# mavmap/mavmap

Hardware: AMD Instinct MI355X
Metric: global-BA LM iterations/sec (higher is better)
Workload: dtype f64; 1 GPU; C3: 500 images / 200000 points / 2000000 obs global BA, PINHOLE+OPENCV, 2 shared cameras; images=500, points=200000, observations=2000000, parallelism=single GPU, options=max_iter 200, ftol 1e-6, gtol 1e-10, ptol 1e-8, Cauchy a=1, refine intrinsics

## Files before the change

### mavmap_amd/csrc/internal.h

```cpp
#ifndef MAVBA_INTERNAL_H_
#define MAVBA_INTERNAL_H_

#include <hip/hip_runtime.h>
#include <stdint.h>

#include <utility>
#include <vector>
#include <functional>

namespace mavba {

constexpr int kPoseRec = 24;
constexpr int kIntrRec = 36;

constexpr int kImgRec = 81;
constexpr int kCamRec = 54;
constexpr int kSweepAcc = 135;

struct SweepChunk { int image; int begin; int end; };

enum { BLK_PP = 0, BLK_IP = 1, BLK_II = 2 };

struct SchurBlock {
  int kind;
  int row_ent, col_ent;
  int chunk_begin, chunk_end;
};
struct SchurChunk { int begin; int end; int slot; };
struct PartialReduce { int kind, src_begin, src_end, dst; };
struct PartialRide { int n = 0; const PartialReduce* tasks = nullptr; double* pp = nullptr; double* ip = nullptr; double* ii = nullptr; };
void launch_partial_reduce(hipStream_t st, int num_tasks, const PartialReduce* tasks, double* part_pp, double* part_ip,
                           double* part_ii);

constexpr int kClImagesMax = 16, kClCamsMax = 3;
constexpr int kClCamRow0 = 6 * kClImagesMax, kClHRow = kClCamRow0 + 9 * kClCamsMax, kClRows = (kClHRow + 16) / 16 * 16;
constexpr int kClTabPP = 0, kClTabIP = kClImagesMax * (kClImagesMax + 1) / 2, kClTabII = kClTabIP + kClCamsMax * kClImagesMax,
              kClTab = kClTabII + kClCamsMax * (kClCamsMax + 1) / 2;
constexpr int kClBatch = 32;
constexpr int kTailObs = 16;
constexpr int kClMaxBatches = 64;
struct SchurCluster { int p0, p1; };

#if defined(__HIPCC__)
__host__ __device__
#endif
inline unsigned image_set_mix(unsigned x) {
  x ^= x >> 16; x *= 0x7feb352du; x ^= x >> 15; x *= 0x846ca68bu; x ^= x >> 16;
  return x;
}

constexpr int kRowsBatch = 16;
constexpr int kRowsMaxPoints = 256;
constexpr int kRowsClasses = 3;
constexpr int kRowsClassNT[kRowsClasses] = {5, 6, 8};
struct SchurRowsCluster { int p0, p1, ni, nc, emit_off, emit_n[2], flags; };
constexpr int kRowsUnplaced = 1;
#if defined(__HIPCC__)
__host__ __device__
#endif
inline int rows_cam_off(int flags, int lc) { return lc <= 0 ? 0 : lc >= 3 ? (flags >> 24) & 255 : (flags >> (8 * lc)) & 255; }
#if defined(__HIPCC__)
__host__ __device__
#endif
inline int rows_cam_rows(int flags) { return (flags >> 24) & 255; }
inline int rows_pack_flags(bool unplaced, const int* k, int nc) {
  int off[4] = {0, 0, 0, 0};
  for (int c = 0; c < 3; ++c) off[c + 1] = off[c] + (c < nc ? k[c] : 0);
  return (unplaced ? kRowsUnplaced : 0) | off[1] << 8 | off[2] << 16 | off[3] << 24;
}
constexpr unsigned kRowsEmitZero = 8191u;
constexpr unsigned rows_emit_entry(int src, int o, int tab_index) { return (unsigned)src | (unsigned)o << 13 | (unsigned)tab_index << 20; }
constexpr int kRowsListsCam = kClImagesMax, kRowsListsCams = 2 * kClImagesMax, kRowsLists = 2 * kClImagesMax + kClCamsMax + 1;
constexpr int kRowsPassSplit = 96;
#if defined(__HIPCC__)
__host__ __device__
#endif
inline int rows_class_of_rows(int rows) { return rows <= 16 * kRowsClassNT[0] ? 0 : rows <= 16 * kRowsClassNT[1] ? 1 : 2; }
#if defined(__HIPCC__)
__host__ __device__
#endif
inline int rows_count(int ni, int cam_rows) { return 6 * ni + cam_rows + 1; }

enum {
  SC_COST = 0,
  SC_XNORM2,
  SC_GRAD_MAX,
  SC_NEW_COST,
  SC_STEP_NORM2,
  SC_MODEL_CHANGE,
  SC_CAND_XNORM2,
  SC_FAIL,
  SC_FAIL_FRONT,
  SC_CAND_END,
  SC_EVAL_COUNT = SC_GRAD_MAX + 1,
  SC_CAND_BEGIN = SC_NEW_COST,
  SC_CAND_COUNT = SC_CAND_END - SC_CAND_BEGIN,
  SC_COUNT = 16
};

enum { LM_REJECTED = 0, LM_ACCEPTED = 1, LM_INVALID = 2, LM_TERM_PTOL = 3, LM_TERM_FTOL = 4, LM_TERM_GTOL = 5 };
struct LmSpec {
  const double* dec;
  const double* scal;
  double radius, decrease_factor;
  double ptol, ftol, min_rel_dec, max_radius, abs_gtol;
  int pending_eval;
};
struct LmDecision {
  int code;
  double radius, decrease_factor;
  double rel, step_norm, cost_change;
};
#if defined(__HIPCC__)
__host__ __device__
#endif
inline LmSpec lm_spec_off() { LmSpec s{}; s.dec = nullptr; s.scal = nullptr; return s; }

struct SweepArgs {
  int N, Nstride, NI, NC, KMAX;
  const double2* uv; const int* obs_img; const int* obs_pt;
  const double* camrec; const double* intr; const int* img_cam; const int* cam_model;
  const double* points;
  const unsigned char* pt_active;
  double loss_b, loss_inv_b;
  double* R; double* Jp; double* Jc; double* Jk;
  double* cost_partial;
};
int jacobian_sweep_grid(int N);
void launch_cam_prepare(hipStream_t st, int NI, const double* poses, double* camrec);
void launch_jacobian_sweep(hipStream_t st, const SweepArgs& a);
void launch_cost_only(hipStream_t st, const SweepArgs& a);
void launch_raw_residual_norm(hipStream_t st, const SweepArgs& a, double* out_norm);

void launch_point_reduce(hipStream_t st, int NP, int NPs, int Nstride, int KMAX, const int* pt_start,
                         const int* q_start, const int* q_cam, const int* obs_img, const int* img_cam,
                         const double* R, const double* Jp, const double* Jk, double* Cu, double* gu,
                         double* Wk );

constexpr int kFrontObs = 256, kFrontPts = 64, kFrontQ = 96, kFrontMaxGrid = 65536;
struct FrontTile { int p0, p1, o0, o1, q0, q1; };
struct FrontArgs {
  SweepArgs sw;
  int num_tiles, NPs;
  const FrontTile* tiles;
  const int* pt_start; const int* q_start; const int* q_cam; const int* q_pt;
  const unsigned char* pt_free;
  const double* scale_cam; const double* scale_pt;
  double radius, dmin, dmax;
  double* Cu; double* gu; double* Gi; double* h;
  double* Epose; double* Eintr;
  double* fail;
  long long* trace;
  LmSpec spec;
};
int point_front_grid(int num_tiles);
void launch_point_front(hipStream_t st, const FrontArgs& a, int kmax_intr, bool entries);

struct CamSweepArgs {
  int NI, NC;
  const SweepChunk* chunks; int num_chunks;
  const double2* im_uv; const int* im_pt;
  const double* camrec; const double* intr; const int* img_cam; const int* cam_model;
  const double* points; const unsigned char* pt_active; double loss_b, loss_inv_b;
  double* partial;
  LmSpec spec;
};
void launch_camera_sweep(hipStream_t st, const CamSweepArgs& a, int kmax, bool any_intr_free);
void launch_rot_prior(hipStream_t st, int n, const int* prior_img, const double* prior_R0, double w,
                      const double* poses, double* res, double* jac, double* cost_partial, const LmSpec& spec = lm_spec_off());

void launch_scales(hipStream_t st, int NI, int NC, int NP, int NPs, int jacobi,
                   const unsigned char* pose_free, const unsigned char* intr_free,
                   const unsigned char* pt_free, const double* img_rec, const double* cam_rec,
                   const double* Cu, double* scale_cam, double* scale_pt);

constexpr int kStateNormsCamBlocks = 64;

void launch_factor_entries_pose(hipStream_t st, int N, int Nstride, int NPs, const int* obs_img, const int* obs_pt,
                                const unsigned char* pt_free, const double* Jc, const double* Jp, const double* scale_cam,
                                const double* scale_pt, double* Gi, double* h, double* Epose, const int* pt_start,
                                const double* Cu, const double* gu, double radius, double dmin, double dmax, double* fail);
void launch_entries_intr(hipStream_t st, int Q, int NI, int NPs, const int* q_pt, const int* q_cam,
                         const double* Wk, const double* scale_cam, const double* scale_pt,
                         const double* Gi, const double* h, double* Eintr);

void launch_schur_chunks(hipStream_t st, int kind, int num_chunks, const SchurChunk* chunks,
                         const int2* terms, const double* Epose, const double* Eintr,
                         double* partial);
#if defined(__HIPCC__)
__host__ __device__
#endif
constexpr int schur_partial_stride(int kind) { return kind == BLK_PP ? 42 : kind == BLK_IP ? 54 : 90; }
void launch_schur_rows(hipStream_t st, const FrontArgs& a, int kmax_intr, bool generic, int num_clusters,
                       const SchurRowsCluster* clusters, const int* tab, const int* cl_lists, const unsigned short* obs_meta,
                       const unsigned long long* lanemap, const unsigned* emit_map, double* part_pp, double* part_ip, double* part_ii,
                       const struct CamSweepArgs* with_sweep = nullptr );
void rows_emit_map(int ni, int nc, int flags, std::vector<unsigned>& pass0, std::vector<unsigned>& pass1);
constexpr unsigned long long kRowsLanesIdentity = 0xFEDCBA9876543210ull;
void launch_schur_clusters(hipStream_t st, int num_clusters, const SchurCluster* clusters, const int* tab,
                           const int* pt_start, const int* q_start, const unsigned short* obs_meta,
                           const unsigned short* q_meta, const unsigned char* pt_clustered, const double* Epose,
                           const double* Eintr, const double* h, int NPs, double* part_pp, double* part_ip,
                           double* part_ii);
void launch_schur_finalize(hipStream_t st, int num_blocks, const SchurBlock* blocks,
                           const double* part_pp, const double* part_ip, const double* part_ii,
                           int NI, int NC, const int* slot, int nb, bool add_base, double radius, double dmin,
                           double dmax, const int* img_cam, const double* img_rec,
                           const double* cam_rec, const double* scale_cam, const int* off_img, const int* off_cam,
                           double* S);
void launch_tiles_copy(hipStream_t st, int num_tiles, const int* tiles, const int* slot, int nb, double* M, double* buf, bool to_buf);
void launch_fix_diag(hipStream_t st, int n_mat, const int* slot, bool add_one, const int* col_var,
                     const double* scale_cam, double* S);

int backsub_points_grid(int NP);
void launch_backsub_points_jvp(hipStream_t st, int NP, int NPs, int NI, double radius, double dmin, double dmax,
                               const SweepArgs& a, const int* pt_start, const double* delta_cam,
                               const unsigned char* pt_free, const double* Gi, const double* h, const double* Cu,
                               const double* gu, const double* scale_pt, double* cand_points, double* delta_points,
                               double* partial , const double* cand_camrec = nullptr, const double* cand_intr = nullptr,
                               double* cost_partial = nullptr);
struct BsTile { int p0, np, o0, no; };
constexpr int kBsTileObs = 64, kBsTilePts = 64;
std::vector<BsTile> build_backsub_tiles(const int* pt_start, int NP);
int backsub_tiles_grid(int num_tiles);
void launch_backsub_points_tiles(hipStream_t st, int num_tiles, const BsTile* tiles, int NPs, int NI, double radius, double dmin,
                                 double dmax, const SweepArgs& a, const int* pt_start, const double* delta_cam,
                                 const unsigned char* pt_free, const double* Gi, const double* h, const double* Cu,
                                 const double* gu, const double* scale_pt, double* cand_points, double* delta_points,
                                 double* partial , const double* cand_camrec, const double* cand_intr,
                                 double* cost_partial);
struct CamUpdateArgs {
  int NI, NC, cam_part; double radius, dmin, dmax;
  const double* scale_cam; const double* img_rec; const double* cam_rec; const double* poses; const double* intr;
  double* cand_poses; double* cand_intr; double* delta_cam; double* partial3 ; double* cand_camrec;
};
int update_cameras_groups(int NI);
void launch_update_cameras(hipStream_t st, const CamUpdateArgs& u, const double* y);

struct ReduceTask { const double* src; int rows, stride, is_max; const double* src2; int rows2; double* out; };
struct ReduceTasks { ReduceTask t[6]; };
void launch_reduce_tasks(hipStream_t st, const ReduceTasks& tasks, int n, const LmSpec& spec = lm_spec_off());
constexpr int kLmPubDoubles = SC_COUNT + 8;
void launch_lm_snapshot(hipStream_t st, const LmSpec& spec, double* dec, double* host_pub, double seq, double* fail_slots );
void launch_lm_decide_cases(hipStream_t st, int n, const double* in, double* out);
void launch_lm_tail(hipStream_t st, const ReduceTasks& tasks, int n, const LmSpec& spec, double* dec, double* host_pub, double seq, double* fail_slots);
void state_norms_grid(int NI, int NC, int NP, int* gp, int* gc);
struct EvalTailArgs {
  int NI, NC, NP, NPs, with_cams, cam_part, gp, gc, num_tasks;
  int first_group = 0;
  const int* img_chunk_start; const double* cam_partial; const int* prior_start; const double* prior_res; const double* prior_jac;
  const int* cam_img_start; const int* cam_imgs; double* img_rec; double* cam_rec; double* img_intr_tmp;
  const unsigned char* pose_free; const unsigned char* intr_free; const unsigned char* pt_free;
  const double* poses; const double* intr; const double* points; const double* gu; double* norm_partial;
  ReduceTasks T; LmSpec spec;
  PartialRide ride;
};
void launch_camera_reduce(hipStream_t st, const EvalTailArgs& a);
void launch_state_norms(hipStream_t st, const EvalTailArgs& a);
void launch_eval_small(hipStream_t st, const EvalTailArgs& a);
void launch_eval_head_tail(hipStream_t st, const EvalTailArgs& a);

void launch_points_to_caller(hipStream_t st, int NP, int width, const int* orig, const double* in, double* out);
void launch_point_errors(hipStream_t st, int NP, const int* pt_start, const double* rnorm,
                         const int* pt_count, double* perr);

hipError_t device_alloc(void** p, size_t bytes);
void device_free(void* p);
hipError_t copy_h2d_staged(void* dst, const void* src, size_t bytes, hipStream_t st);
hipError_t copy_d2h_staged_sync(void* dst, const void* src, size_t bytes, hipStream_t st);
void release_staged(hipStream_t st);
bool upload_batch_begin(hipStream_t st);
hipError_t upload_batch_end(bool emit);
hipError_t zero_async(void* p, size_t bytes, hipStream_t st);
void upload_batch_debug_arena(size_t bytes);
int host_threads();
void host_run(int T, const std::function<void(int)>& body);

struct CholFront {
  int k;
  int na;
  int act_off;
  int factor_next;
  int sh_begin;
  long long sh_off;
};
struct CholStep { int kind, front_off, nf, nf0, max_na, merge_begin, init_off, tasks; };
struct CholMerge { int sh_begin; long long sh_off; };
struct CholNode { int begin, end, parent; };
enum { CHOL_TASK_TILE = 0, CHOL_TASK_PRE_DIAG = 1, CHOL_TASK_PRE_SUB = 2, CHOL_TASK_CHAIN = 3 };
struct CholTask { int kind, i, j, ub, ue; };
struct CholStructure {
  int nb = 0, nseg = 1;
  std::vector<CholNode> nodes;
  std::vector<int> seg_of_tile;
  std::vector<int> seg_first;
  std::vector<CholFront> fronts;
  std::vector<CholMerge> merges;
  std::vector<CholStep> steps;
  std::vector<int> init_tiles;
  int num_leaf_init = 0;
  int chain_steps = 0;
  int num_fronts_max = 0;
  long long envelope_tiles = 0;
  double factor_flops = 0.0;
  size_t shadow_doubles = 0;
  int* d_ints = nullptr;
  int *d_rows = nullptr, *d_seg_of_tile = nullptr, *d_seg_first = nullptr, *d_init = nullptr;
  unsigned* d_flags = nullptr;
  CholFront* d_fronts = nullptr;
  CholMerge* d_merges = nullptr;
  mutable double* d_shadow = nullptr;
  std::vector<int> tile_slot;
  int* d_tile_slot = nullptr;
  long long num_tiles = 0;
  size_t store_doubles() const { return (size_t)std::max<long long>(num_tiles, 1) * 4096; }
  int active_tiles = 0;
  bool persist_ok = false;
  double predicted_forward_us = 0.0;
  int persist_grid = 0;
  int persist_chain_wgs = 0;
  long long persist_tiles = 0;
  long long persist_updates = 0;
  CholTask* d_tasks = nullptr;
  int* d_pints = nullptr;
  int *d_wg_begin = nullptr, *d_upd = nullptr, *d_tile_id = nullptr, *d_chain_info = nullptr;
  unsigned* d_pflags = nullptr;
  double* d_pre = nullptr;
  unsigned long long* d_trace = nullptr;
  std::vector<CholTask> h_tasks;
  std::vector<int> h_wg_begin, h_upd, h_chain_info;
  bool host_only = false;
  int host_only_cus = 256;
  double lpp_estimate_us = 0.0;
  mutable unsigned epoch = 0;
  CholStructure() {}
  CholStructure(const CholStructure&) = delete;
  CholStructure& operator=(const CholStructure&) = delete;
  ~CholStructure();
  void release();
  hipError_t build(int nb, const std::vector<std::pair<int, int>>& tile_pairs, const std::vector<CholNode>& tree,
                   hipStream_t st);
  hipError_t build_dense(int nb);
  hipError_t build_persistent(const std::vector<std::vector<int>>& col_rows, const std::vector<int>& col_step,
                              const std::vector<int>& height, hipStream_t st);
};
bool dense_spd_solve_is_small(int n_pad, const CholStructure& cs);
bool dense_spd_solve_device(hipStream_t st, double* M, int n_pad, double* y, double* fail,
                            double* diag_ws, double* L, const CholStructure& cs,
                            const int* y_scatter = nullptr, double* y_nat = nullptr, bool allow_persistent = true,
                            hipEvent_t after_factor = nullptr ,
                            const CamUpdateArgs* upd = nullptr);

}
#endif
```

### mavmap_amd/csrc/kernels.hip

```cpp
#include "internal.h"
#include <cstdlib>
#include <type_traits>
#include "ba_math.h"
#include "dev_reduce.h"
#include "lm_decide.h"
#include "lm_bodies.h"
#include "sweep_body.h"
#include "launch_dispatch.h"

namespace mavba {

__global__ void k_cam_prepare(int NI, const double* __restrict__ poses, double* __restrict__ camrec) {
  const int i = blockIdx.x * blockDim.x + threadIdx.x;
  if (i >= NI) return;
  double rec[9];
  cam_prepare(poses + 6 * i, rec);
#pragma unroll
  for (int k = 0; k < 9; ++k) camrec[9 * i + k] = rec[k];
}
void launch_cam_prepare(hipStream_t st, int NI, const double* poses, double* camrec) {
  if (NI <= 0) return;
  hipLaunchKernelGGL(k_cam_prepare, dim3((NI + 127) / 128), dim3(128), 0, st, NI, poses, camrec);
}

// ... 370 lines not shown
    const int np = T.p1 - T.p0;
    const int o0 = T.o0, o1 = T.o1;
    const int q0 = T.q0, nq = KMAX > 0 ? T.q1 - T.q0 : 0;
    int im = im_n, lp = 0, pt0 = pt_n;
    double2 m0 = m_n;
    bool act = act_n;
    const bool own_free = own_free_n;
    const double own_sp[3] = {own_sp_n[0], own_sp_n[1], own_sp_n[2]};
    for (int j = tid; j <= np; j += 256) s_pb[j] = a.pt_start[T.p0 + j];
    for (int i = tid; i < np * 9; i += 256) s_sum[i] = 0.0;
    if constexpr (KMAX > 0) {
      for (int q = tid; q < nq; q += 256) { s_qcam[q] = a.q_cam[q0 + q]; s_qpt[q] = a.q_pt[q0 + q] - T.p0; }
      for (int i = tid; i < nq * SH::K3; i += 256) s_q[i] = 0.0;
    }
    const bool single = o1 - o0 <= kFrontObs;
    double jc[12], jp[6];
    auto eval_obs = [&](int imv, int pt, double2 m, double (&rr)[2], double (&jk)[18], int& cam) -> double {
      im = imv;
      lp = pt - T.p0;
      cam = w.img_cam[imv];
      const int model = w.cam_model[cam];
      double rec[9], kin[9], X[3];
#pragma unroll
      for (int k = 0; k < 9; ++k) rec[k] = w.camrec[9 * imv + k];
#pragma unroll
      for (int k = 0; k < 9; ++k) kin[k] = w.intr[9 * cam + k];
      X[0] = w.points[3 * (long long)pt]; X[1] = w.points[3 * (long long)pt + 1]; X[2] = w.points[3 * (long long)pt + 2];
      double r[2], Jc[12], Jp[6], Jk[18];
      obs_jacobian(model, rec, kin, X, m.x, m.y, r, Jc, Jp, Jk);
      double wgt, half_rho;
      cauchy_weight(r[0] * r[0] + r[1] * r[1], w.loss_b, w.loss_inv_b, wgt, half_rho);
      if constexpr (MASK) { if (!w.pt_active[pt]) { wgt = 0.0; half_rho = 0.0; } }
      rr[0] = wgt * r[0]; rr[1] = wgt * r[1];
#pragma unroll
      for (int e = 0; e < 12; ++e) jc[e] = wgt * Jc[e];
#pragma unroll
      for (int e = 0; e < 6; ++e) jp[e] = wgt * Jp[e];
#pragma unroll
      for (int e = 0; e < 18; ++e) jk[e] = wgt * Jk[e];
      return half_rho;
    };
    for (int base = o0; base < o1; base += kFrontObs) {
      const int o = base + tid;
      if (base != o0) {
        act = o < o1;
        if (act) { im = w.obs_img[o]; pt0 = w.obs_pt[o]; m0 = w.uv[o]; }
      }
      double prod[SH::NROWS];
      int cam = -1;
      if (act) {
        double rr[2], jk[18];
        cost += eval_obs(im, pt0, m0, rr, jk, cam);
        prod[0] = jp[0] * jp[0] + jp[3] * jp[3]; prod[1] = jp[0] * jp[1] + jp[3] * jp[4]; prod[2] = jp[0] * jp[2] + jp[3] * jp[5];
        prod[3] = jp[1] * jp[1] + jp[4] * jp[4]; prod[4] = jp[1] * jp[2] + jp[4] * jp[5]; prod[5] = jp[2] * jp[2] + jp[5] * jp[5];
        prod[6] = jp[0] * rr[0] + jp[3] * rr[1]; prod[7] = jp[1] * rr[0] + jp[4] * rr[1]; prod[8] = jp[2] * rr[0] + jp[5] * rr[1];
#pragma unroll
        for (int k = 0; k < KMAX; ++k)
#pragma unroll
          for (int t = 0; t < 3; ++t) prod[9 + 3 * k + t] = jk[k] * jp[t] + jk[9 + k] * jp[3 + t];
      }
      auto round = [&](auto rc) {
        constexpr int R = decltype(rc)::value;
        constexpr int lo = R * SH::NR, hi = (lo + SH::NR < SH::NROWS) ? lo + SH::NR : SH::NROWS;
        constexpr int PR = R == 0 ? 9 : 0;
        constexpr int wlo = (lo > 9 ? lo : 9) - 9, WR = hi - 9 - wlo;
        if (R > 0) lds_barrier();
        if (act) {
          if (R == 0) s_cam[tid] = cam;
#pragma unroll
          for (int v = lo; v < hi; ++v) s_park[(v - lo) * kFrPitch + tid] = prod[v];
        }
        lds_barrier();
        const int nit = np * PR + nq * WR;
        for (int it = tid; it < nit; it += 256) {
          const bool is_pt = it < np * PR;
          int j, slot, c = -1;
          const double* row;
          double* dst;
          if (is_pt) {
            j = it / 9;
            slot = it - 9 * j;
            row = s_park + slot * kFrPitch - base;
            dst = s_sum + it;
          } else {
            const int t2 = it - np * PR;
            const int wr = WR > 0 ? WR : 1;
            const int q = t2 / wr, vv = wlo + (t2 - q * wr);
            j = s_qpt[q]; c = s_qcam[q];
            row = s_park + (vv + 9 - lo) * kFrPitch - base;
            dst = s_q + q * SH::K3 + vv;
          }
          const int b = max(s_pb[j], base), e = min(s_pb[j + 1], base + kFrontObs);
          const int* camv = s_cam - base;
          double acc = *dst;
          for (int i0 = b; i0 < e; i0 += 4) {
            const int i1 = min(i0 + 1, e - 1), i2 = min(i0 + 2, e - 1), i3 = min(i0 + 3, e - 1);
            double x0 = row[i0], x1 = row[i1], x2 = row[i2], x3 = row[i3];
            if (WR > 0 && !is_pt) {
              x0 = camv[i0] == c ? x0 : 0.0; x1 = camv[i1] == c ? x1 : 0.0; x2 = camv[i2] == c ? x2 : 0.0; x3 = camv[i3] == c ? x3 : 0.0;
            }
            acc += x0;
            acc += i0 + 1 < e ? x1 : 0.0;
            acc += i0 + 2 < e ? x2 : 0.0;
            acc += i0 + 3 < e ? x3 : 0.0;
          }
          *dst = acc;
        }
      };
      round(std::integral_constant<int, 0>{});
      if constexpr (SH::ROUNDS > 1) round(std::integral_constant<int, 1>{});
      lds_barrier();
    }
    if (tile + 1 < t_end) request_tile(tile + 1);
    if (tid < np) {
      const int p = T.p0 + tid;
      double C6[6], g3[3];
#pragma unroll
      for (int k = 0; k < 6; ++k) C6[k] = s_sum[tid * 9 + k];
#pragma unroll
      for (int k = 0; k < 3; ++k) g3[k] = s_sum[tid * 9 + 6 + k];
#pragma unroll
      for (int k = 0; k < 6; ++k) a.Cu[(size_t)k * NPs + p] = C6[k];
#pragma unroll
      for (int k = 0; k < 3; ++k) a.gu[(size_t)k * NPs + p] = g3[k];
      if constexpr (ENTRIES) {
        double G[6] = {0, 0, 0, 0, 0, 0}, hh[3] = {0, 0, 0}, sp[3] = {0, 0, 0};
        if (own_free) {
#pragma unroll
          for (int k = 0; k < 3; ++k) sp[k] = own_sp[k];
          double C[6];
          C[0] = sp[0] * sp[0] * C6[0]; C[1] = sp[0] * sp[1] * C6[1]; C[2] = sp[0] * sp[2] * C6[2];
          C[3] = sp[1] * sp[1] * C6[3]; C[4] = sp[1] * sp[2] * C6[4]; C[5] = sp[2] * sp[2] * C6[5];
          const double inv_radius = 1.0 / a.radius;
          C[0] = __builtin_fma(clampd(C[0], a.dmin, a.dmax), inv_radius, C[0]);
          C[3] = __builtin_fma(clampd(C[3], a.dmin, a.dmax), inv_radius, C[3]);
          C[5] = __builtin_fma(clampd(C[5], a.dmin, a.dmax), inv_radius, C[5]);
          bool fin = chol3_inv_fast(C, G);
          const double gs[3] = {sp[0] * g3[0], sp[1] * g3[1], sp[2] * g3[2]};
          gi_mul(G, gs, hh);
#pragma unroll
          for (int k = 0; k < 6; ++k) fin = fin && isfinite(G[k]);
          if (!fin) atomicAdd(a.fail, 1.0);
        }
        if (s_pb[tid + 1] > s_pb[tid]) {
#pragma unroll
          for (int k = 0; k < 6; ++k) a.Gi[(size_t)k * NPs + p] = G[k];
#pragma unroll
          for (int k = 0; k < 3; ++k) a.h[(size_t)k * NPs + p] = hh[k];
        }
#pragma unroll
        for (int k = 0; k < 6; ++k) s_g[tid * 12 + k] = G[k];
#pragma unroll
        for (int k = 0; k < 3; ++k) { s_g[tid * 12 + 6 + k] = hh[k]; s_g[tid * 12 + 9 + k] = sp[k]; }
      }
    }
    if constexpr (ENTRIES) {
      lds_barrier();
      if constexpr (KMAX > 0) {
        for (int it = tid; it < nq * 9; it += 256) {
          const int q = it / 9, k = it - 9 * q;
          const double* g = s_g + s_qpt[q] * 12;
          double w0 = 0.0, w1 = 0.0, w2 = 0.0;
          if (k < KMAX) {
            const double sk = a.scale_cam[6 * w.NI + 9 * s_qcam[q] + k];
            const double* W = s_q + q * SH::K3 + 3 * k;
            w0 = W[0] * sk * g[9]; w1 = W[1] * sk * g[10]; w2 = W[2] * sk * g[11];
          }
          const double u0 = w0 * g[0];
          const double u1 = w0 * g[1] + w1 * g[2];
          const double u2 = w0 * g[3] + w1 * g[4] + w2 * g[5];
          double* out = a.Eintr + (size_t)(q0 + q) * kIntrRec;
          out[3 * k] = u0; out[3 * k + 1] = u1; out[3 * k + 2] = u2;
          out[27 + k] = u0 * g[6] + u1 * g[7] + u2 * g[8];
        }
        lds_barrier();
      }
      for (int base = o0; base < o1; base += kFrontObs) {
        const int o = base + tid;
        if (!single) {
          act = o < o1;
          if (act) { double rr[2], jk[18]; int cam; (void)eval_obs(w.obs_img[o], w.obs_pt[o], w.uv[o], rr, jk, cam); }
        }
        double rec[kPoseRec];
#pragma unroll
        for (int k = 0; k < kPoseRec; ++k) rec[k] = 0.0;
        if (act && a.pt_free[T.p0 + lp]) {
          const double* g = s_g + lp * 12;
          double jps[6];
#pragma unroll
          for (int row = 0; row < 2; ++row)
#pragma unroll
            for (int k = 0; k < 3; ++k) jps[row * 3 + k] = jp[row * 3 + k] * g[9 + k];
#pragma unroll
          for (int e = 0; e < 6; ++e) {
            const double sc = a.scale_cam[6 * im + e];
            const double j0 = jc[e] * sc, j1 = jc[6 + e] * sc;
            const double w0 = j0 * jps[0] + j1 * jps[3], w1 = j0 * jps[1] + j1 * jps[4], w2 = j0 * jps[2] + j1 * jps[5];
            const double u0 = w0 * g[0];
            const double u1 = w0 * g[1] + w1 * g[2];
            const double u2 = w0 * g[3] + w1 * g[4] + w2 * g[5];
            rec[3 * e] = u0; rec[3 * e + 1] = u1; rec[3 * e + 2] = u2;
            rec[18 + e] = u0 * g[6] + u1 * g[7] + u2 * g[8];
          }
        }
        const long long lim = (long long)o1 * kPoseRec;
        constexpr int kStage = SH::A >= 256 * 25 ? 256 : 128;
#pragma unroll
        for (int part = 0; part < 256 / kStage; ++part) {
          if (tid / kStage == part) {
#pragma unroll
            for (int k = 0; k < kPoseRec; ++k) s_rec[(tid % kStage) * 25 + k] = rec[k];
          }
          lds_barrier();
          const long long gbase = ((long long)base + part * kStage) * kPoseRec;
#pragma unroll 4
          for (int i = tid; i < kStage * kPoseRec; i += 256) {
            const int t = i / kPoseRec, k = i - t * kPoseRec;
            if (gbase + i < lim) a.Epose[gbase + i] = s_rec[t * 25 + k];
          }
          lds_barrier();
        }
      }
    } else {
      lds_barrier();
    }
  }
  const double tot = block_sum_256(cost, s_red);
  if (tid == 0) w.cost_partial[blockIdx.x] = tot;
}

int point_front_grid(int num_tiles) {
  static const int cap = [] { const char* e = std::getenv("MAVBA_FRONT_GRID"); const int v = e ? std::atoi(e) : 0; return v > 0 && v < kFrontMaxGrid ? v : kFrontMaxGrid; }();
  return num_tiles < 1 ? 0 : (num_tiles > cap ? cap : num_tiles);
}
void launch_point_front(hipStream_t st, const FrontArgs& a, int kmax_intr, bool entries) {
  const int grid = point_front_grid(a.num_tiles);
  if (grid <= 0) return;
  const bool mask = a.sw.pt_active != nullptr;
  int dev = 0;
  (void)hipGetDevice(&dev);
  with_width_or_none(kmax_intr, [&](auto k) {
    with_bool(entries, [&](auto e) {
      with_bool(mask, [&](auto m) {
        const auto kernel = &k_point_front<decltype(k)::value, decltype(e)::value, decltype(m)::value>;
        constexpr size_t bytes = FrontShape<decltype(k)::value>::BYTES;
        static bool configured[64] = {};
        if (dev >= 0 && dev < 64 && !configured[dev]) {
          (void)hipFuncSetAttribute(reinterpret_cast<const void*>(kernel), hipFuncAttributeMaxDynamicSharedMemorySize, (int)bytes);
          configured[dev] = true;
        }
        hipLaunchKernelGGL(kernel, dim3(grid), dim3(256), bytes, st, a);
      });
    });
  });
}

__global__ void __launch_bounds__(256) k_camera_sweep(CamSweepArgs a) {
  if (!lm_spec_go(a.spec, nullptr)) return;
  __shared__ double s_red[4 * kSweepAcc];
  camera_sweep_body(a, blockIdx.x, s_red);
}

template <int K>
__global__ void __launch_bounds__(256, 2) k_camera_sweep_gram(CamSweepArgs a) {
  if (!lm_spec_go(a.spec, nullptr)) return;
  __shared__ __attribute__((aligned(16))) double s_rows[kCsLdsDoubles];
  camera_sweep_gram_body<K>(a, blockIdx.x, s_rows);
}
void launch_camera_sweep(hipStream_t st, const CamSweepArgs& a, int kmax, bool any_intr_free) {
  if (a.num_chunks <= 0) return;
  const dim3 g(a.num_chunks), b(256);
  if (!any_intr_free) hipLaunchKernelGGL(k_camera_sweep, g, b, 0, st, a);
  else with_width(kmax, [&](auto k) { hipLaunchKernelGGL((k_camera_sweep_gram<decltype(k)::value>), g, b, 0, st, a); });
}

__global__ void k_rot_prior(int n, const int* __restrict__ prior_img, const double* __restrict__ R0,
                            double w, const double* __restrict__ poses, double* __restrict__ res,
                            double* __restrict__ jac, double* __restrict__ cost_partial, LmSpec spec) {
  if (!lm_spec_go(spec, nullptr)) return;
  const int q = blockIdx.x * blockDim.x + threadIdx.x;
  if (q >= n) return;
  double r, j[3];
  rot_prior_eval(poses + 6 * prior_img[q], R0 + 9 * q, w, r, j);
  res[q] = r; jac[3 * q] = j[0]; jac[3 * q + 1] = j[1]; jac[3 * q + 2] = j[2];
  cost_partial[q] = 0.5 * r * r;
}
void launch_rot_prior(hipStream_t st, int n, const int* prior_img, const double* prior_R0, double w,
                      const double* poses, double* res, double* jac, double* cost_partial, const LmSpec& spec) {
  if (n <= 0) return;
  hipLaunchKernelGGL(k_rot_prior, dim3((n + 127) / 128), dim3(128), 0, st, n, prior_img, prior_R0, w, poses, res, jac, cost_partial, spec);
}

__device__ void partial_reduce_task(const PartialReduce T, int lane, double* part_pp, double* part_ip, double* part_ii);
__global__ void __launch_bounds__(64) k_camera_reduce_img(
    int NI, const int* __restrict__ img_chunk_start, const double* __restrict__ partial,
    const int* __restrict__ prior_start, const double* __restrict__ prior_res,
    const double* __restrict__ prior_jac, double* __restrict__ img_rec, double* __restrict__ img_intr_tmp, LmSpec spec, PartialRide ride) {
  if (!lm_spec_go(spec, nullptr)) return;
  if ((int)blockIdx.x >= NI) { partial_reduce_task(ride.tasks[blockIdx.x - NI], threadIdx.x, ride.pp, ride.ip, ride.ii); return; }
  camera_reduce_img_body(blockIdx.x, threadIdx.x, img_chunk_start, partial, prior_start, prior_res, prior_jac, img_rec, img_intr_tmp);
}
__global__ void __launch_bounds__(1024) k_camera_reduce_cam(
    const int* __restrict__ cam_img_start, const int* __restrict__ cam_imgs,
    const double* __restrict__ img_intr_tmp, double* __restrict__ cam_rec, LmSpec spec) {
  __shared__ double s_part[16][64];
  if (!lm_spec_go(spec, nullptr)) return;
  const int c = blockIdx.x;
  const int e = threadIdx.x & 63, part = threadIdx.x >> 6;
  double s = 0.0;
  if (e < kCamRec) {
    const int t1 = cam_img_start[c + 1];
    for (int t = cam_img_start[c] + part; t < t1; t += 64) {
      const int i0 = cam_imgs[t], i1 = cam_imgs[min(t + 16, t1 - 1)], i2 = cam_imgs[min(t + 32, t1 - 1)], i3 = cam_imgs[min(t + 48, t1 - 1)];
      const double x0 = img_intr_tmp[(size_t)i0 * kCamRec + e], x1 = img_intr_tmp[(size_t)i1 * kCamRec + e];
      const double x2 = img_intr_tmp[(size_t)i2 * kCamRec + e], x3 = img_intr_tmp[(size_t)i3 * kCamRec + e];
      s += x0;
      if (t + 16 < t1) s += x1;
      if (t + 32 < t1) s += x2;
      if (t + 48 < t1) s += x3;
    }
  }
  s_part[part][e] = s;
  __syncthreads();
  if (part == 0 && e < kCamRec) {
    double tot = 0.0;
#pragma unroll
    for (int k = 0; k < 16; ++k) tot += s_part[k][e];
    cam_rec[(size_t)c * kCamRec + e] = tot;
  }
}
void launch_camera_reduce(hipStream_t st, const EvalTailArgs& a) {
  if (a.NI > 0 || a.ride.n > 0)
    hipLaunchKernelGGL(k_camera_reduce_img, dim3(a.NI + a.ride.n), dim3(64), 0, st, a.NI, a.img_chunk_start, a.cam_partial,
                       a.prior_start, a.prior_res, a.prior_jac, a.img_rec, a.img_intr_tmp, a.spec, a.ride);
  if (a.NC > 0 && a.with_cams)
    hipLaunchKernelGGL(k_camera_reduce_cam, dim3(a.NC), dim3(1024), 0, st, a.cam_img_start, a.cam_imgs, a.img_intr_tmp, a.cam_rec, a.spec);
}

__global__ void k_scales(int NI, int NC, int NP, int NPs, int jacobi,
                         const unsigned char* __restrict__ pose_free,
                         const unsigned char* __restrict__ intr_free,
                         const unsigned char* __restrict__ pt_free, const double* __restrict__ img_rec,
                         const double* __restrict__ cam_rec, const double* __restrict__ Cu,
                         double* __restrict__ scale_cam, double* __restrict__ scale_pt) {
  const int t = blockIdx.x * blockDim.x + threadIdx.x;
  const int ncam = 6 * NI + 9 * NC;
  if (t < ncam) {
    double n2; bool fr;
    if (t < 6 * NI) {
      const int i = t / 6, e = t % 6;
      n2 = img_rec[(size_t)i * kImgRec + sym_idx(e, e, 6)];
      fr = pose_free[t] != 0;
    } else {
      const int c = (t - 6 * NI) / 9, k = (t - 6 * NI) % 9;
      n2 = cam_rec[(size_t)c * kCamRec + sym_idx(k, k, 9)];
      fr = intr_free[9 * c + k] != 0;
    }
    scale_cam[t] = fr ? (jacobi ? 1.0 / (1.0 + sqrt(n2)) : 1.0) : 0.0;
  }
  if (t < NP) {
    const bool fr = pt_free[t] != 0;
    const int d[3] = {0, 3, 5};
#pragma unroll
    for (int k = 0; k < 3; ++k)
      scale_pt[k * NPs + t] = fr ? (jacobi ? 1.0 / (1.0 + sqrt(Cu[d[k] * NPs + t])) : 1.0) : 0.0;
  }
}
void launch_scales(hipStream_t st, int NI, int NC, int NP, int NPs, int jacobi,
                   const unsigned char* pose_free, const unsigned char* intr_free,
                   const unsigned char* pt_free, const double* img_rec, const double* cam_rec,
                   const double* Cu, double* scale_cam, double* scale_pt) {
  const int n = max(6 * NI + 9 * NC, NP);
  if (n <= 0) return;
  hipLaunchKernelGGL(k_scales, dim3((n + 255) / 256), dim3(256), 0, st, NI, NC, NP, NPs, jacobi, pose_free,
                     intr_free, pt_free, img_rec, cam_rec, Cu, scale_cam, scale_pt);
}

__global__ void __launch_bounds__(256) k_state_norms(
    int NI, int NC, int NP, int NPs, int gp, int cam_part, const unsigned char* __restrict__ pose_free,
    const unsigned char* __restrict__ intr_free, const unsigned char* __restrict__ pt_free,
    const double* __restrict__ poses, const double* __restrict__ intr, const double* __restrict__ points,
    const double* __restrict__ img_rec, const double* __restrict__ cam_rec, const double* __restrict__ gu,
    double* __restrict__ partial, LmSpec spec) {
  __shared__ double s_red[4];
  if (!lm_spec_go(spec, nullptr)) return;
  state_norms_body(blockIdx.x, gp, gridDim.x - gp, NI, NC, NP, NPs, cam_part, pose_free, intr_free, pt_free, poses, intr, points,
                   img_rec, cam_rec, gu, partial, s_red);
}
void state_norms_grid(int NI, int NC, int NP, int* gp, int* gc) {
  *gp = std::min(512, (NP + 255) / 256);
  *gc = std::max(1, std::min(kStateNormsCamBlocks, (6 * NI + 9 * NC + 255) / 256));
}
void launch_state_norms(hipStream_t st, const EvalTailArgs& a) {
  hipLaunchKernelGGL(k_state_norms, dim3(a.gp + a.gc), dim3(256), 0, st, a.NI, a.NC, a.NP, a.NPs, a.gp, a.cam_part, a.pose_free,
                     a.intr_free, a.pt_free, a.poses, a.intr, a.points, a.img_rec, a.cam_rec, a.gu, a.norm_partial, a.spec);
}


__global__ void __launch_bounds__(256) k_entries_pose(
    int N, int Nstride, int NPs, const int* __restrict__ obs_img, const int* __restrict__ obs_pt,
    const unsigned char* __restrict__ pt_free, const double* __restrict__ Jc, const double* __restrict__ Jp,
    const double* __restrict__ scale_cam, const double* __restrict__ scale_pt, double* __restrict__ Gi,
    double* __restrict__ h, double* __restrict__ Epose, const int* __restrict__ pt_start, const double* __restrict__ Cu,
    const double* __restrict__ gu, double radius, double dmin, double dmax, double* __restrict__ fail) {
  __shared__ double s_rec[256 * 25];
  const long long S = Nstride;
  const long long o = (long long)blockIdx.x * 256 + threadIdx.x;
  double rec[kPoseRec];
#pragma unroll
  for (int k = 0; k < kPoseRec; ++k) rec[k] = 0.0;
  if (o < N) {
    const int p = obs_pt[o];
    const bool fr = pt_free[p] != 0;
    if (!fr && o == pt_start[p]) {
#pragma unroll
      for (int k = 0; k < 6; ++k) Gi[k * NPs + p] = 0.0;
#pragma unroll
      for (int k = 0; k < 3; ++k) h[k * NPs + p] = 0.0;
    }
    if (fr) {
      const int im = obs_img[o];
      double sp[3], G[6], hh[3], jp[6];
#pragma unroll
      for (int k = 0; k < 3; ++k) sp[k] = scale_pt[k * NPs + p];
      double C[6];
      C[0] = sp[0] * sp[0] * Cu[p];           C[1] = sp[0] * sp[1] * Cu[NPs + p];     C[2] = sp[0] * sp[2] * Cu[2 * NPs + p];
      C[3] = sp[1] * sp[1] * Cu[3 * NPs + p]; C[4] = sp[1] * sp[2] * Cu[4 * NPs + p]; C[5] = sp[2] * sp[2] * Cu[5 * NPs + p];
      C[0] += clampd(C[0], dmin, dmax) / radius;
      C[3] += clampd(C[3], dmin, dmax) / radius;
      C[5] += clampd(C[5], dmin, dmax) / radius;
      const bool ok = chol3_inv(C, G);
      const double gs[3] = {sp[0] * gu[p], sp[1] * gu[NPs + p], sp[2] * gu[2 * NPs + p]};
      gi_mul(G, gs, hh);
      if (o == pt_start[p]) {
        bool fin = ok;
#pragma unroll
        for (int k = 0; k < 6; ++k) fin = fin && isfinite(G[k]);
        if (!fin) atomicAdd(fail, 1.0);
#pragma unroll
        for (int k = 0; k < 6; ++k) Gi[k * NPs + p] = G[k];
#pragma unroll
        for (int k = 0; k < 3; ++k) h[k * NPs + p] = hh[k];
      }
#pragma unroll
      for (int row = 0; row < 2; ++row)
#pragma unroll
        for (int k = 0; k < 3; ++k) jp[row * 3 + k] = Jp[(row * 3 + k) * S + o] * sp[k];
#pragma unroll
      for (int e = 0; e < 6; ++e) {
        const double sc = scale_cam[6 * im + e];
        const double j0 = Jc[e * S + o] * sc, j1 = Jc[(6 + e) * S + o] * sc;
        const double w0 = j0 * jp[0] + j1 * jp[3], w1 = j0 * jp[1] + j1 * jp[4], w2 = j0 * jp[2] + j1 * jp[5];
        const double u0 = w0 * G[0];
        const double u1 = w0 * G[1] + w1 * G[2];
        const double u2 = w0 * G[3] + w1 * G[4] + w2 * G[5];
        rec[3 * e] = u0; rec[3 * e + 1] = u1; rec[3 * e + 2] = u2;
        rec[18 + e] = u0 * hh[0] + u1 * hh[1] + u2 * hh[2];
      }
    }
  }
#pragma unroll
  for (int k = 0; k < kPoseRec; ++k) s_rec[threadIdx.x * 25 + k] = rec[k];
  __syncthreads();
  const long long base = (long long)blockIdx.x * 256 * kPoseRec;
  const long long lim = (long long)N * kPoseRec;
  for (int i = threadIdx.x; i < 256 * kPoseRec; i += 256) {
    const int t = i / kPoseRec, k = i - t * kPoseRec;
    if (base + i < lim) Epose[base + i] = s_rec[t * 25 + k];
  }
}
void launch_factor_entries_pose(hipStream_t st, int N, int Nstride, int NPs, const int* obs_img, const int* obs_pt,
                                const unsigned char* pt_free, const double* Jc, const double* Jp, const double* scale_cam,
                                const double* scale_pt, double* Gi, double* h, double* Epose, const int* pt_start,
                                const double* Cu, const double* gu, double radius, double dmin, double dmax, double* fail) {
  if (N <= 0) return;
  hipLaunchKernelGGL(k_entries_pose, dim3((N + 255) / 256), dim3(256), 0, st, N, Nstride, NPs, obs_img, obs_pt,
                     pt_free, Jc, Jp, scale_cam, scale_pt, Gi, h, Epose, pt_start, Cu, gu, radius, dmin, dmax, fail);
}

__global__ void __launch_bounds__(256) k_entries_intr(
    int Q, int NI, int NPs, const int* __restrict__ q_pt, const int* __restrict__ q_cam,
    const double* __restrict__ Wk, const double* __restrict__ scale_cam, const double* __restrict__ scale_pt,
    const double* __restrict__ Gi, const double* __restrict__ h, double* __restrict__ Eintr) {
  const long long t = (long long)blockIdx.x * 256 + threadIdx.x;
  const int q = (int)(t / 9), k = (int)(t - 9ll * q);
  if (q >= Q) return;
  const int p = q_pt[q], c = q_cam[q];
  const double* W = Wk + (size_t)q * 27 + 3 * k;
  const double sk = scale_cam[6 * NI + 9 * c + k];
  const double w0 = W[0] * sk * scale_pt[p], w1 = W[1] * sk * scale_pt[NPs + p], w2 = W[2] * sk * scale_pt[2 * NPs + p];
  const double u0 = w0 * Gi[p];
  const double u1 = w0 * Gi[NPs + p] + w1 * Gi[2 * NPs + p];
  const double u2 = w0 * Gi[3 * (size_t)NPs + p] + w1 * Gi[4 * (size_t)NPs + p] + w2 * Gi[5 * (size_t)NPs + p];
  double* out = Eintr + (size_t)q * kIntrRec;
  out[3 * k] = u0; out[3 * k + 1] = u1; out[3 * k + 2] = u2;
  out[27 + k] = u0 * h[p] + u1 * h[NPs + p] + u2 * h[2 * NPs + p];
}
void launch_entries_intr(hipStream_t st, int Q, int NI, int NPs, const int* q_pt, const int* q_cam,
                         const double* Wk, const double* scale_cam, const double* scale_pt,
                         const double* Gi, const double* h, double* Eintr) {
  if (Q <= 0) return;
  hipLaunchKernelGGL(k_entries_intr, dim3((unsigned)((9ll * Q + 255) / 256)), dim3(256), 0, st, Q, NI, NPs, q_pt, q_cam, Wk, scale_cam,
                     scale_pt, Gi, h, Eintr);
}

template <int RX, int RY, int SX, int SY, bool DIAG>
__global__ void __launch_bounds__(256) k_schur_chunks(int num_chunks, const SchurChunk* __restrict__ chunks,
                                                      const int2* __restrict__ terms,
                                                      const double* __restrict__ EX,
                                                      const double* __restrict__ EY,
                                                      double* __restrict__ partial) {
  const int wv = threadIdx.x >> 6, lane = threadIdx.x & 63;
  const int per_xcd = (gridDim.x + 7) >> 3;
  const int wg = (blockIdx.x & 7) * per_xcd + (blockIdx.x >> 3);
  const int cid = wg * 4 + wv;
  if (cid >= num_chunks) return;
  const SchurChunk ch = chunks[cid];
  constexpr int NA = RX * RY;
  constexpr int PS = NA + (DIAG ? RX : 0);
  double acc[NA], ev[RX];
#pragma unroll
  for (int i = 0; i < NA; ++i) acc[i] = 0.0;
#pragma unroll
  for (int i = 0; i < RX; ++i) ev[i] = 0.0;
  for (int t = ch.begin + lane; t < ch.end; t += 64) {
    const int2 xy = terms[t];
    const double* px = EX + (size_t)xy.x * SX;
    const double* py = EY + (size_t)xy.y * SY;
    double ux[RX * 3], uy[RY * 3];
#pragma unroll
    for (int i = 0; i < RX * 3; i += 2) {
      if (i + 1 < RX * 3) { const double2 v = *reinterpret_cast<const double2*>(px + i); ux[i] = v.x; ux[i + 1] = v.y; }
      else ux[i] = px[i];
    }
#pragma unroll
    for (int i = 0; i < RY * 3; i += 2) {
      if (i + 1 < RY * 3) { const double2 v = *reinterpret_cast<const double2*>(py + i); uy[i] = v.x; uy[i + 1] = v.y; }
      else uy[i] = py[i];
    }
#pragma unroll
    for (int r = 0; r < RX; ++r)
#pragma unroll
      for (int c = 0; c < RY; ++c)
        acc[r * RY + c] += ux[3 * r] * uy[3 * c] + ux[3 * r + 1] * uy[3 * c + 1] + ux[3 * r + 2] * uy[3 * c + 2];
    if (DIAG && xy.x == xy.y) {
#pragma unroll
      for (int r = 0; r < RX; ++r) ev[r] += px[RX * 3 + r];
    }
  }
  double* out = partial + (size_t)ch.slot * PS;
#pragma unroll
  for (int i = 0; i < NA; ++i) { const double v = wave_sum(acc[i]); if (lane == 0) out[i] = v; }
  if (DIAG) {
#pragma unroll
    for (int r = 0; r < RX; ++r) { const double v = wave_sum(ev[r]); if (lane == 0) out[NA + r] = v; }
  }
}

namespace {
typedef double cl_d4 __attribute__((ext_vector_type(4)));
constexpr int kClK = 3 * kClBatch, kClPitch = kClK + 2;
constexpr int kClThreads = 512, kClWaves = kClThreads / 64;
struct ClShape {
  static constexpr int images = kClImagesMax, cam_row0 = kClCamRow0, hrow = kClHRow, rows = kClRows;
  static constexpr int NT = rows / 16, tiles = NT * (NT + 1) / 2, acc = (tiles + kClWaves - 1) / kClWaves;
  static constexpr int tab_ip = kClTabIP, tab_ii = kClTabII, tab = kClTab;
};
constexpr bool kClPipelined = kClBatch >= 32;
template <int NT>
constexpr bool cluster_row_used(int W, int row) {
  int t = 0;
  for (int i = 0; i < NT; ++i)
    for (int j = 0; j <= i; ++j) {
      if (t % kClWaves == W && (i == row || j == row)) return true;
      ++t;
    }
  return false;
}
template <class SH, int W>
__device__ __forceinline__ void cluster_mfma(const double* __restrict__ E, int lane, cl_d4 (&acc)[SH::acc]) {
  constexpr int NT = SH::NT;
  const int li = lane & 15, lk = lane >> 4;
  const double* base = E + li * kClPitch + lk;
  auto load = [&](double (&x)[NT], int kk) {
#pragma unroll
    for (int i = 0; i < NT; ++i)
      if (cluster_row_used<NT>(W, i)) x[i] = base[16 * i * kClPitch + kk];
  };
  auto mma = [&](const double (&x)[NT]) {
    int t = 0;
#pragma unroll
    for (int i = 0; i < NT; ++i)
#pragma unroll
      for (int j = 0; j <= i; ++j) {
        if (t % kClWaves == W) acc[t / kClWaves] = __builtin_amdgcn_mfma_f64_16x16x4f64(x[i], x[j], acc[t / kClWaves], 0, 0, 0);
        ++t;
      }
  };
  if constexpr (!kClPipelined) {
    double a[NT];
#pragma unroll 1
    for (int kk = 0; kk < kClK; kk += 4) { load(a, kk); mma(a); }
  } else {
    static_assert(kClK % 8 == 0, "two k-steps per trip");
    double a[NT], b[NT];
    load(a, 0);
#pragma unroll 1
    for (int kk = 0; kk < kClK; kk += 8) {
      load(b, kk + 4);
      __builtin_amdgcn_sched_barrier(0);
      mma(a);
      __builtin_amdgcn_sched_barrier(0);
      if (kk + 8 < kClK) load(a, kk + 8);
      __builtin_amdgcn_sched_barrier(0);
      mma(b);
      __builtin_amdgcn_sched_barrier(0);
    }
  }
}
template <class SH>
__device__ __forceinline__ void cluster_store(int R, int C, double v, const int* __restrict__ tab,
                                              double* __restrict__ part_pp, double* __restrict__ part_ip,
                                              double* __restrict__ part_ii) {
  constexpr int P0 = SH::cam_row0, H = SH::hrow;
  if (R < P0) {
    const int la = R / 6, r = R - 6 * la, lb = C / 6, c = C - 6 * lb;
    if (la == lb && r < c) return;
    const int slot = tab[la * (la + 1) / 2 + lb];
    if (slot >= 0) part_pp[(size_t)slot * 42 + r * 6 + c] = v;
  } else if (R < H) {
    const int lc = (R - P0) / 9, r = (R - P0) - 9 * lc;
    if (C < P0) {
      const int la = C / 6, c = C - 6 * la;
      const int slot = tab[SH::tab_ip + lc * SH::images + la];
      if (slot >= 0) part_ip[(size_t)slot * 54 + r * 6 + c] = v;
    } else {
      const int lc2 = (C - P0) / 9, c = (C - P0) - 9 * lc2;
      if (lc == lc2 && r < c) return;
      const int slot = tab[SH::tab_ii + lc * (lc + 1) / 2 + lc2];
      if (slot >= 0) part_ii[(size_t)slot * 90 + r * 9 + c] = v;
    }
  } else if (R == H) {
    if (C < P0) {
      const int la = C / 6, r = C - 6 * la;
      const int slot = tab[la * (la + 1) / 2 + la];
      if (slot >= 0) part_pp[(size_t)slot * 42 + 36 + r] = v;
    } else if (C < H) {
      const int lc = (C - P0) / 9, r = (C - P0) - 9 * lc;
      const int slot = tab[SH::tab_ii + lc * (lc + 1) / 2 + lc];
      if (slot >= 0) part_ii[(size_t)slot * 90 + 81 + r] = v;
    }
  }
}
template <class SH, int W>
__device__ __forceinline__ void cluster_emit(int lane, const cl_d4 (&acc)[SH::acc], const int* __restrict__ tab,
                                             double* __restrict__ part_pp, double* __restrict__ part_ip,
                                             double* __restrict__ part_ii) {
  const int li = lane & 15, lk = lane >> 4;
  int t = 0;
#pragma unroll
  for (int i = 0; i < SH::NT; ++i)
#pragma unroll
    for (int j = 0; j <= i; ++j) {
      if (t % kClWaves == W) {
#pragma unroll
        for (int r = 0; r < 4; ++r) {
          const int R = 16 * i + lk + 4 * r, C = 16 * j + li;
          if (R >= C) cluster_store<SH>(R, C, acc[t / kClWaves][r], tab, part_pp, part_ip, part_ii);
        }
      }
      ++t;
    }
}
}

namespace {
constexpr int kClChunk = (kClImagesMax * kClBatch * 2 / 3 * 9 + kClThreads - 1) / kClThreads, kClQChunk = (2 * kClBatch * 14 + kClThreads - 1) / kClThreads + 1;
template <int REC, int USED, int NU>
struct ClusterRegs { double2 v[NU]; unsigned meta[NU]; };
template <int REC, int USED, int NU>
struct ClusterPlan {
  static constexpr int D2 = (USED + 1) / 2;
  int src[NU];
  int rec_no[NU];
  unsigned dst[NU];
  __device__ __forceinline__ void init(int tid) {
#pragma unroll
    for (int u = 0; u < NU; ++u) {
      const int f = u * kClThreads + tid, oo = f / D2, e2 = (f - oo * D2) * 2;
      rec_no[u] = oo;
      src[u] = oo * REC + e2;
      dst[u] = (unsigned)((e2 / 3) * kClPitch + e2 % 3) | (e2 % 3 == 2 ? 0x8000u : 0u) | (e2 + 1 < USED ? 0x4000u : 0u);
    }
  }
};
template <int REC, int USED, int NU>
__device__ __forceinline__ void cluster_fetch(ClusterRegs<REC, USED, NU>& R, const ClusterPlan<REC, USED, NU>& P, int first,
                                              int count, const unsigned short* __restrict__ rec_meta,
                                              const double* __restrict__ rec) {
  if (count <= 0) return;
  const double* base = rec + (size_t)first * REC;
  const unsigned short* mbase = rec_meta + first;
  const int last = count - 1;
#pragma unroll
  for (int u = 0; u < NU; ++u) {
    const int over = max(P.rec_no[u] - last, 0);
    R.v[u] = *reinterpret_cast<const double2*>(base + (P.src[u] - over * REC));
    R.meta[u] = mbase[P.rec_no[u] - over];
  }
}
template <int REC, int USED, int NU>
__device__ __forceinline__ void cluster_scatter(const ClusterRegs<REC, USED, NU>& R, const ClusterPlan<REC, USED, NU>& P,
                                                double* __restrict__ E, int row0, int row_step, int count) {
#pragma unroll
  for (int u = 0; u < NU; ++u)
    if (P.rec_no[u] < count && R.meta[u] != 0xFFFFu) {
      const int at = (row0 + row_step * (int)(R.meta[u] >> 8)) * kClPitch + 3 * (int)(R.meta[u] & 255u) + (int)(P.dst[u] & 0x3FFFu);
      E[at] = R.v[u].x;
      if (P.dst[u] & 0x4000u) E[at + ((P.dst[u] & 0x8000u) ? kClPitch - 2 : 1)] = R.v[u].y;
    }
}
template <int REC, int USED, int NU>
__device__ __forceinline__ void cluster_fetch_any(ClusterRegs<REC, USED, NU>& R, int tid, int u0, int first, int count,
                                                  const unsigned short* __restrict__ rec_meta, const double* __restrict__ rec) {
  constexpr int D2 = (USED + 1) / 2;
  const int ntot = count * D2;
#pragma unroll
  for (int u = 0; u < NU; ++u) {
    const int f = (u0 + u) * kClThreads + tid;
    R.meta[u] = 0xFFFFu;
    if (f < ntot) {
      const int oo = f / D2, e2 = (f - oo * D2) * 2, o = first + oo;
      R.v[u] = *reinterpret_cast<const double2*>(rec + (size_t)o * REC + e2);
      R.meta[u] = rec_meta[o];
    }
  }
}
template <int REC, int USED, int NU>
__device__ __forceinline__ void cluster_scatter_any(const ClusterRegs<REC, USED, NU>& R, double* __restrict__ E, int tid, int u0,
                                                    int row0, int row_step) {
  constexpr int D2 = (USED + 1) / 2;
#pragma unroll
  for (int u = 0; u < NU; ++u)
    if (R.meta[u] != 0xFFFFu) {
      const int f = (u0 + u) * kClThreads + tid, e2 = (f % D2) * 2;
      const int at = (row0 + row_step * (int)(R.meta[u] >> 8) + e2 / 3) * kClPitch + 3 * (int)(R.meta[u] & 255u) + e2 % 3;
      E[at] = R.v[u].x;
      if (e2 + 1 < USED) E[at + ((e2 % 3 == 2) ? kClPitch - 2 : 1)] = R.v[u].y;
    }
}
template <int REC, int USED, int NU>
__device__ __forceinline__ void cluster_overflow(double* __restrict__ E, int tid, int first, int count, int row0,
                                                 int row_step, const unsigned short* __restrict__ rec_meta,
                                                 const double* __restrict__ rec) {
  const int u_end = (count * ((USED + 1) / 2) + kClThreads - 1) / kClThreads;
  for (int uc = NU; uc < u_end; uc += NU) {
    ClusterRegs<REC, USED, NU> R;
    cluster_fetch_any(R, tid, uc, first, count, rec_meta, rec);
    cluster_scatter_any(R, E, tid, uc, row0, row_step);
  }
}
}

__global__ void __launch_bounds__(kClThreads, kClPipelined ? 1 : 2) k_schur_clusters(
    const SchurCluster* __restrict__ clusters, const int* __restrict__ tabs, const int* __restrict__ pt_start,
    const int* __restrict__ q_start, const unsigned short* __restrict__ obs_meta,
    const unsigned short* __restrict__ q_meta, const unsigned char* __restrict__ pt_clustered,
    const double* __restrict__ Epose, const double* __restrict__ Eintr, const double* __restrict__ h, int NPs,
    double* __restrict__ part_pp, double* __restrict__ part_ip, double* __restrict__ part_ii) {
  using SH = ClShape;
  __shared__ __attribute__((aligned(16))) double E[SH::rows * kClPitch];
  __shared__ int s_bounds[2][kClMaxBatches + 1];
  __shared__ int s_tab[SH::tab];
  const int tid = threadIdx.x, wv = tid >> 6, lane = tid & 63;
  const SchurCluster cl = clusters[blockIdx.x];
  const int nbatch = (cl.p1 - cl.p0 + kClBatch - 1) / kClBatch;
  for (int i = tid; i <= nbatch; i += kClThreads) {
    const int p = min(cl.p0 + i * kClBatch, cl.p1);
    s_bounds[0][i] = pt_start[p];
    s_bounds[1][i] = q_start[p];
  }
  for (int i = tid; i < SH::tab; i += kClThreads) s_tab[i] = tabs[(size_t)blockIdx.x * SH::tab + i];
  cl_d4 acc[SH::acc];
#pragma unroll
  for (int i = 0; i < SH::acc; ++i) acc[i] = (cl_d4){0.0, 0.0, 0.0, 0.0};
  __syncthreads();
  ClusterRegs<kPoseRec, 18, kClChunk> RP;
  ClusterRegs<kIntrRec, 27, kClQChunk> RQ;
  ClusterPlan<kPoseRec, 18, kClChunk> PP;
  ClusterPlan<kIntrRec, 27, kClQChunk> PQ;
  PP.init(tid);
  PQ.init(tid);
  double hv = 0.0;
  unsigned char hon = 0;
  auto fetch = [&](int bi) {
    const int b0 = cl.p0 + bi * kClBatch, b1 = min(b0 + kClBatch, cl.p1);
    cluster_fetch(RP, PP, s_bounds[0][bi], s_bounds[0][bi + 1] - s_bounds[0][bi], obs_meta, Epose);
    cluster_fetch(RQ, PQ, s_bounds[1][bi], s_bounds[1][bi + 1] - s_bounds[1][bi], q_meta, Eintr);
    hon = 0;
    if (tid < (b1 - b0) * 3) {
      const int pp = tid / 3, t = tid - 3 * pp;
      hon = pt_clustered[b0 + pp];
      hv = h[(size_t)t * NPs + b0 + pp];
    }
  };
  if constexpr (kClPipelined) fetch(0);
  for (int bi = 0; bi < nbatch; ++bi) {
    if constexpr (!kClPipelined) fetch(bi);
    for (int i = tid; i < SH::rows * kClPitch / 2; i += kClThreads) reinterpret_cast<double2*>(E)[i] = make_double2(0.0, 0.0);
    __syncthreads();
    cluster_scatter(RP, PP, E, 0, 6, s_bounds[0][bi + 1] - s_bounds[0][bi]);
    cluster_scatter(RQ, PQ, E, SH::cam_row0, 9, s_bounds[1][bi + 1] - s_bounds[1][bi]);
    if (hon) E[SH::hrow * kClPitch + tid] = hv;
    cluster_overflow<kPoseRec, 18, kClChunk>(E, tid, s_bounds[0][bi], s_bounds[0][bi + 1] - s_bounds[0][bi], 0, 6, obs_meta, Epose);
    cluster_overflow<kIntrRec, 27, kClQChunk>(E, tid, s_bounds[1][bi], s_bounds[1][bi + 1] - s_bounds[1][bi], SH::cam_row0, 9, q_meta, Eintr);
    __syncthreads();
    if constexpr (kClPipelined) {
      if (bi + 1 < nbatch) fetch(bi + 1);
      __builtin_amdgcn_sched_barrier(0);
    }
    switch (wv) {
      case 0: cluster_mfma<SH, 0>(E, lane, acc); break;
      case 1: cluster_mfma<SH, 1>(E, lane, acc); break;
      case 2: cluster_mfma<SH, 2>(E, lane, acc); break;
      case 3: cluster_mfma<SH, 3>(E, lane, acc); break;
      case 4: cluster_mfma<SH, 4>(E, lane, acc); break;
      case 5: cluster_mfma<SH, 5>(E, lane, acc); break;
      case 6: cluster_mfma<SH, 6>(E, lane, acc); break;
      default: cluster_mfma<SH, 7>(E, lane, acc); break;
    }
    __syncthreads();
  }
  const int* tab = s_tab;
  switch (wv) {
    case 0: cluster_emit<SH, 0>(lane, acc, tab, part_pp, part_ip, part_ii); break;
    case 1: cluster_emit<SH, 1>(lane, acc, tab, part_pp, part_ip, part_ii); break;
    case 2: cluster_emit<SH, 2>(lane, acc, tab, part_pp, part_ip, part_ii); break;
    case 3: cluster_emit<SH, 3>(lane, acc, tab, part_pp, part_ip, part_ii); break;
    case 4: cluster_emit<SH, 4>(lane, acc, tab, part_pp, part_ip, part_ii); break;
    case 5: cluster_emit<SH, 5>(lane, acc, tab, part_pp, part_ip, part_ii); break;
    case 6: cluster_emit<SH, 6>(lane, acc, tab, part_pp, part_ip, part_ii); break;
    default: cluster_emit<SH, 7>(lane, acc, tab, part_pp, part_ip, part_ii); break;
  }
}
void launch_schur_clusters(hipStream_t st, int num_clusters, const SchurCluster* clusters, const int* tab,
                           const int* pt_start, const int* q_start, const unsigned short* obs_meta,
                           const unsigned short* q_meta, const unsigned char* pt_clustered, const double* Epose,
                           const double* Eintr, const double* h, int NPs, double* part_pp, double* part_ip,
                           double* part_ii) {
  if (num_clusters <= 0) return;
  hipLaunchKernelGGL(k_schur_clusters, dim3(num_clusters), dim3(kClThreads), 0, st, clusters, tab, pt_start, q_start, obs_meta,
                     q_meta, pt_clustered, Epose, Eintr, h, NPs, part_pp, part_ip, part_ii);
}

void launch_schur_chunks(hipStream_t st, int kind, int num_chunks, const SchurChunk* chunks,
                         const int2* terms, const double* Epose, const double* Eintr, double* partial) {
  if (num_chunks <= 0) return;
  const dim3 g((((num_chunks + 3) / 4) + 7) / 8 * 8), b(256);
  if (kind == BLK_PP)
    hipLaunchKernelGGL((k_schur_chunks<6, 6, kPoseRec, kPoseRec, true>), g, b, 0, st, num_chunks, chunks, terms, Epose, Epose, partial);
  else if (kind == BLK_IP)
    hipLaunchKernelGGL((k_schur_chunks<9, 6, kIntrRec, kPoseRec, false>), g, b, 0, st, num_chunks, chunks, terms, Eintr, Epose, partial);
  else
    hipLaunchKernelGGL((k_schur_chunks<9, 9, kIntrRec, kIntrRec, true>), g, b, 0, st, num_chunks, chunks, terms, Eintr, Eintr, partial);
}

__device__ __forceinline__ double strided_sum16(const double* __restrict__ part, int PS, int idx, int begin, int end) {
  double s[16];
#pragma unroll
  for (int u = 0; u < 16; ++u) s[u] = 0.0;
  for (int c = begin; c < end; c += 16) {
    double x[16];
#pragma unroll
    for (int u = 0; u < 16; ++u) x[u] = part[(size_t)min(c + u, end - 1) * PS + idx];
#pragma unroll
    for (int u = 0; u < 16; ++u) s[u] += (c + u < end) ? x[u] : 0.0;
  }
  return (((s[0] + s[1]) + (s[2] + s[3])) + ((s[4] + s[5]) + (s[6] + s[7]))) + (((s[8] + s[9]) + (s[10] + s[11])) + ((s[12] + s[13]) + (s[14] + s[15])));
}
__device__ void partial_reduce_task(const PartialReduce T, int lane, double* part_pp, double* part_ip, double* part_ii) {
  double* part = T.kind == BLK_PP ? part_pp : T.kind == BLK_IP ? part_ip : part_ii;
  const int PS = schur_partial_stride(T.kind);
  for (int idx = lane; idx < PS; idx += 64) part[(size_t)T.dst * PS + idx] = strided_sum16(part, PS, idx, T.src_begin, T.src_end);
}
__global__ void __launch_bounds__(256) k_partial_reduce(int num_tasks, const PartialReduce* __restrict__ tasks,
                                                        double* __restrict__ part_pp, double* __restrict__ part_ip,
                                                        double* __restrict__ part_ii) {
  const int task = blockIdx.x * 4 + (threadIdx.x >> 6), lane = threadIdx.x & 63;
  if (task >= num_tasks) return;
  partial_reduce_task(tasks[task], lane, part_pp, part_ip, part_ii);
}
void launch_partial_reduce(hipStream_t st, int num_tasks, const PartialReduce* tasks, double* part_pp, double* part_ip,
                           double* part_ii) {
  if (num_tasks <= 0) return;
  hipLaunchKernelGGL(k_partial_reduce, dim3((num_tasks + 3) / 4), dim3(256), 0, st, num_tasks, tasks, part_pp, part_ip, part_ii);
}

__global__ void __launch_bounds__(256) k_schur_finalize(
    int num_blocks, const SchurBlock* __restrict__ blocks, const double* __restrict__ part_pp,
    const double* __restrict__ part_ip, const double* __restrict__ part_ii, int NI, int NC, const int* __restrict__ slot, int nb,
    int add_base, double radius, double dmin, double dmax, const int* __restrict__ img_cam,
    const double* __restrict__ img_rec, const double* __restrict__ cam_rec,
    const double* __restrict__ scale_cam, const int* __restrict__ off_img, const int* __restrict__ off_cam,
    double* __restrict__ S) {
  const int wv = threadIdx.x >> 6, lane = threadIdx.x & 63;
  const int bid = blockIdx.x * 4 + wv;
  if (bid >= num_blocks) return;
  const SchurBlock B = blocks[bid];
  const int RX = B.kind == BLK_PP ? 6 : 9, RY = B.kind == BLK_II ? 9 : 6;
  const int NA = RX * RY;
  const bool diag_kind = B.kind != BLK_IP;
  const int PS = NA + (diag_kind ? RX : 0);
  const double* part = B.kind == BLK_PP ? part_pp : B.kind == BLK_IP ? part_ip : part_ii;
  const int row0 = B.kind == BLK_PP ? 6 * B.row_ent : 6 * NI + 9 * B.row_ent;
  const int col0 = B.kind == BLK_II ? 6 * NI + 9 * B.col_ent : 6 * B.col_ent;
  const int prow0 = B.kind == BLK_PP ? off_img[B.row_ent] : off_cam[B.row_ent];
  const int pcol0 = B.kind == BLK_II ? off_cam[B.col_ent] : off_img[B.col_ent];
  const bool is_diag = diag_kind && B.row_ent == B.col_ent;
  auto apply = [&](int idx, double s) {
    if (idx < NA) {
      const int r = idx / RY, c = idx - r * RY;
      const int gr = row0 + r, gc = col0 + c;
      double base = 0.0;
      if (add_base) {
        const double sr = scale_cam[gr], sc = scale_cam[gc];
        if (B.kind == BLK_PP && is_diag) {
          const int x = r < c ? r : c, y = r < c ? c : r;
          base = sr * sc * img_rec[(size_t)B.row_ent * kImgRec + sym_idx(x, y, 6)];
          if (r == c && sr != 0.0) base += clampd(base, dmin, dmax) / radius;
        } else if (B.kind == BLK_IP && img_cam[B.col_ent] == B.row_ent) {
          base = sr * sc * img_rec[(size_t)B.col_ent * kImgRec + 27 + c * 9 + r];
        } else if (B.kind == BLK_II && is_diag) {
          const int x = r < c ? r : c, y = r < c ? c : r;
          base = sr * sc * cam_rec[(size_t)B.row_ent * kCamRec + sym_idx(x, y, 9)];
          if (r == c && sr != 0.0) base += clampd(base, dmin, dmax) / radius;
        }
      }
      double val = base - s;
      if (is_diag && r == c && scale_cam[gr] == 0.0) val = add_base ? 1.0 : 0.0;
      if (!is_diag || r >= c) {
        const int R = prow0 + r, C = pcol0 + c;
        if ((R >> 6) >= (C >> 6)) S[((size_t)slot[(R >> 6) * nb + (C >> 6)] << 12) + (R & 63) * 64 + (C & 63)] = val;
        if ((C >> 6) >= (R >> 6)) S[((size_t)slot[(C >> 6) * nb + (R >> 6)] << 12) + (C & 63) * 64 + (R & 63)] = val;
      }
    } else if (is_diag) {
      const int r = idx - NA;
      const int gr = row0 + r;
      double base = 0.0;
      if (add_base) {
        const double g = B.kind == BLK_PP ? img_rec[(size_t)B.row_ent * kImgRec + 21 + r]
                                          : cam_rec[(size_t)B.row_ent * kCamRec + 45 + r];
        base = scale_cam[gr] * g;
      }
      const int C = prow0 + r;
      S[((size_t)slot[nb * nb + (C >> 6)] << 12) + (C & 63)] = base - s;
    }
  };
  for (int idx = lane; idx < PS; idx += 64) apply(idx, strided_sum16(part, PS, idx, B.chunk_begin, B.chunk_end));
}
void launch_schur_finalize(hipStream_t st, int num_blocks, const SchurBlock* blocks,
                           const double* part_pp, const double* part_ip, const double* part_ii,
                           int NI, int NC, const int* slot, int nb, bool add_base, double radius, double dmin,
                           double dmax, const int* img_cam, const double* img_rec,
                           const double* cam_rec, const double* scale_cam, const int* off_img, const int* off_cam,
                           double* S) {
  if (num_blocks <= 0) return;
  hipLaunchKernelGGL(k_schur_finalize, dim3((num_blocks + 3) / 4), dim3(256), 0, st, num_blocks, blocks, part_pp,
                     part_ip, part_ii, NI, NC, slot, nb, add_base ? 1 : 0, radius, dmin, dmax, img_cam, img_rec, cam_rec,
                     scale_cam, off_img, off_cam, S);
}
__global__ void __launch_bounds__(256) k_tiles_copy(int num_tiles, const int* __restrict__ tiles, const int* __restrict__ slot, int nb,
                                                    double* __restrict__ M, double* __restrict__ buf, int to_buf) {
  const int t = blockIdx.x;
  if (t < num_tiles) {
    double2* a = reinterpret_cast<double2*>(M + ((size_t)tiles[t] << 12));
    double2* b = reinterpret_cast<double2*>(buf + ((size_t)t << 12));
    for (int e = threadIdx.x; e < 2048; e += 256) { if (to_buf) b[e] = a[e]; else a[e] = b[e]; }
  } else {
    double* rhs = buf + ((size_t)num_tiles << 12);
    for (int c = (t - num_tiles) * 256 + threadIdx.x; c < nb * 64; c += (gridDim.x - num_tiles) * 256) {
      double* a = M + ((size_t)slot[nb * nb + (c >> 6)] << 12) + (c & 63);
      if (to_buf) rhs[c] = *a; else *a = rhs[c];
    }
  }
}
void launch_tiles_copy(hipStream_t st, int num_tiles, const int* tiles, const int* slot, int nb, double* M, double* buf, bool to_buf) {
  const int extra = std::max(1, std::min(16, (nb * 64 + 1023) / 1024));
  hipLaunchKernelGGL(k_tiles_copy, dim3(num_tiles + extra), dim3(256), 0, st, num_tiles, tiles, slot, nb, M, buf, to_buf ? 1 : 0);
}

__global__ void k_fix_diag(int n_mat, const int* __restrict__ slot, int add_one, const int* __restrict__ col_var,
                           const double* __restrict__ scale_cam, double* __restrict__ S) {
  const int t = blockIdx.x * blockDim.x + threadIdx.x;
  if (t >= n_mat) return;
  const int j = col_var[t];
  if (j < 0 || scale_cam[j] == 0.0) S[((size_t)slot[(t >> 6) * (n_mat >> 6) + (t >> 6)] << 12) + (t & 63) * 65] = add_one ? 1.0 : 0.0;
}
void launch_fix_diag(hipStream_t st, int n_mat, const int* slot, bool add_one, const int* col_var, const double* scale_cam, double* S) {
  hipLaunchKernelGGL(k_fix_diag, dim3((n_mat + 255) / 256), dim3(256), 0, st, n_mat, slot, add_one ? 1 : 0, col_var, scale_cam, S);
}

constexpr int kBsCamsLds = 16;
__global__ void __launch_bounds__(256) k_backsub_points_packed(
    int NP, int NPs, int NI, int NC, int N, int ppb, int nblocks, double radius, double dmin, double dmax, double loss_b, double loss_inv_b,
    const int* __restrict__ pt_start, const int* __restrict__ obs_img, const int* __restrict__ obs_pt,
    const double2* __restrict__ uv, const int* __restrict__ img_cam, const int* __restrict__ cam_model,
    const double* __restrict__ camrec, const double* __restrict__ intr, const double* __restrict__ delta_cam,
    const unsigned char* __restrict__ pt_free, const double* __restrict__ Gi, const double* __restrict__ h,
    const double* __restrict__ Cu, const double* __restrict__ gu, const double* __restrict__ scale_pt,
    const double* __restrict__ points, double* __restrict__ cand_points, double* __restrict__ delta_points,
    double* __restrict__ partial, const double* __restrict__ cand_camrec, const double* __restrict__ cand_intr,
    const unsigned char* __restrict__ pt_active, double* __restrict__ cost_partial) {
  __shared__ double s_t[3][256];
  __shared__ double s_new[3][128];
  __shared__ double s_red[4];
  __shared__ double s_kin[kBsCamsLds][9], s_dk[kBsCamsLds][9];
  __shared__ int s_model[kBsCamsLds];
  const int tid = threadIdx.x;
  const bool cams_lds = NC <= kBsCamsLds;
  double a_step = 0.0, a_model = 0.0, a_x2 = 0.0, a_cost = 0.0;
  const int G = (int)gridDim.x;
  struct Obs { int pt, im; double2 m; };
  auto load_obs = [&](int o) {
    Obs r{0, 0, make_double2(0.0, 0.0)};
    if (N <= 0) return r;
    const int oc = min(o, N - 1);
    r.pt = obs_pt[oc]; r.im = obs_img[oc]; r.m = uv[oc];
    return r;
  };
  auto obs_term = [&](const Obs& q, bool valid, double (&t)[3]) {
    t[0] = t[1] = t[2] = 0.0;
    if (!valid || !pt_free[q.pt]) return;
    const int cam = img_cam[q.im];
    const double X[3] = {points[3 * (size_t)q.pt], points[3 * (size_t)q.pt + 1], points[3 * (size_t)q.pt + 2]};
    double rec[9], kin[9], dc[6], dk[9];
#pragma unroll
    for (int k = 0; k < 9; ++k) rec[k] = camrec[9 * q.im + k];
#pragma unroll
    for (int k = 0; k < 6; ++k) dc[k] = delta_cam[6 * q.im + k];
    int model;
    if (cams_lds) {
      model = s_model[cam];
#pragma unroll
      for (int k = 0; k < 9; ++k) { kin[k] = s_kin[cam][k]; dk[k] = s_dk[cam][k]; }
    } else {
      model = cam_model[cam];
#pragma unroll
      for (int k = 0; k < 9; ++k) { kin[k] = intr[9 * cam + k]; dk[k] = delta_cam[6 * NI + 9 * cam + k]; }
    }
    double r[2], tt[3];
#ifndef MAVBA_BS_SKIP
#define MAVBA_BS_SKIP 0
#endif
    if (MAVBA_BS_SKIP & 1) { r[0] = rec[0] + kin[0] + dc[0] + dk[0]; r[1] = X[0] + q.m.x; tt[0] = rec[3]; tt[1] = X[1]; tt[2] = q.m.y; }
    else
    obs_backsub_term(model, rec, kin, X, q.m.x, q.m.y, dc, dk, r, tt);
    double w, half_rho;
    cauchy_weight(r[0] * r[0] + r[1] * r[1], loss_b, loss_inv_b, w, half_rho);
    const double w2 = w * w;
    t[0] = w2 * tt[0]; t[1] = w2 * tt[1]; t[2] = w2 * tt[2];
  };
  int o0 = 0, o1 = 0, o0n = 0, o1n = 0;
  Obs cur{0, 0, make_double2(0.0, 0.0)};
  if ((int)blockIdx.x < nblocks) {
    const int b0 = (int)blockIdx.x;
    o0 = pt_start[b0 * ppb]; o1 = pt_start[min(b0 * ppb + ppb, NP)];
    if (b0 + G < nblocks) { o0n = pt_start[(b0 + G) * ppb]; o1n = pt_start[min((b0 + G) * ppb + ppb, NP)]; }
    cur = load_obs(o0 + tid);
  }
  if (cams_lds) {
    for (int e = tid; e < 9 * NC; e += 256) { s_kin[e / 9][e % 9] = intr[e]; s_dk[e / 9][e % 9] = delta_cam[6 * NI + e]; }
    for (int c = tid; c < NC; c += 256) s_model[c] = cam_model[c];
    __syncthreads();
  }
  for (int blk = blockIdx.x; blk < nblocks; blk += G) {
    const int p0 = blk * ppb, p1 = min(p0 + ppb, NP);
    const int p = p0 + tid;
    const bool owner = p < p1;
    int o0nn = 0, o1nn = 0;
    Obs nxt = cur;
    if (blk + G < nblocks) {
      nxt = load_obs(o0n + tid);
      if (blk + 2 * G < nblocks) { o0nn = pt_start[(blk + 2 * G) * ppb]; o1nn = pt_start[min((blk + 2 * G) * ppb + ppb, NP)]; }
    }
    int mb = 0, me = 0;
    bool fr = false;
    double G[6] = {0, 0, 0, 0, 0, 0}, sp[3] = {0, 0, 0}, hh[3] = {0, 0, 0}, cu[3] = {0, 0, 0}, gg[3] = {0, 0, 0}, Xo[3] = {0, 0, 0};
    if (owner) {
      mb = pt_start[p]; me = pt_start[p + 1];
      fr = pt_free[p] != 0;
#pragma unroll
      for (int k = 0; k < 3; ++k) Xo[k] = points[3 * (size_t)p + k];
      if (fr) {
        const int dg[3] = {0, 3, 5};
#pragma unroll
        for (int k = 0; k < 6; ++k) G[k] = Gi[k * NPs + p];
#pragma unroll
        for (int k = 0; k < 3; ++k) { sp[k] = scale_pt[k * NPs + p]; hh[k] = h[k * NPs + p]; cu[k] = Cu[dg[k] * NPs + p]; gg[k] = gu[k * NPs + p]; }
      }
    }
    double T[3] = {0.0, 0.0, 0.0};
    for (int base = o0; base < o1; base += 256) {
      const int o = base + tid;
      const Obs q = base == o0 ? cur : load_obs(o);
      double t[3];
      obs_term(q, o < o1, t);
      s_t[0][tid] = t[0]; s_t[1][tid] = t[1]; s_t[2][tid] = t[2];
      __syncthreads();
      if (owner) {
        const int b = max(mb, base), e = (MAVBA_BS_SKIP & 2) ? min(me, max(mb, base) + 1) : min(me, base + 256);
        for (int i = b; i < e; ++i) { T[0] += s_t[0][i - base]; T[1] += s_t[1][i - base]; T[2] += s_t[2][i - base]; }
      }
      __syncthreads();
    }
    if (owner) {
      double d[3] = {0, 0, 0};
      if (fr) {
        const double q0 = -sp[0] * T[0], q1 = -sp[1] * T[1], q2 = -sp[2] * T[2];
        const double z[3] = {q0 * G[0], q0 * G[1] + q1 * G[2], q0 * G[3] + q1 * G[4] + q2 * G[5]};
        const double tt[3] = {hh[0] - z[0], hh[1] - z[1], hh[2] - z[2]};
        double yp[3];
        git_mul(G, tt, yp);
#pragma unroll
        for (int k = 0; k < 3; ++k) {
          const double s = sp[k];
          const double D2 = clampd(s * s * cu[k], dmin, dmax) / radius;
          const double gs = s * gg[k];
          a_model += 0.5 * yp[k] * (gs + D2 * yp[k]);
          d[k] = -yp[k] * s;
          a_step += d[k] * d[k];
        }
      }
#pragma unroll
      for (int k = 0; k < 3; ++k) {
        const double xn = Xo[k] + d[k];
        cand_points[3 * (size_t)p + k] = xn;
        delta_points[3 * (size_t)p + k] = d[k];
        if (fr) a_x2 += xn * xn;
        if (cost_partial) s_new[k][tid] = xn;
      }
    }
    if (cost_partial) {
      __syncthreads();
      for (int base = o0; base < o1; base += 256) {
        const int o = base + tid;
        if (o < o1) {
          const int pt = obs_pt[o], im = obs_img[o];
          const double2 m = uv[o];
          const int cam = img_cam[im];
          double rec[9], kin[9], r[2];
#pragma unroll
          for (int k = 0; k < 9; ++k) rec[k] = cand_camrec[9 * im + k];
#pragma unroll
          for (int k = 0; k < 9; ++k) kin[k] = cand_intr[9 * cam + k];
          const double Xn[3] = {s_new[0][pt - p0], s_new[1][pt - p0], s_new[2][pt - p0]};
          obs_residual(cam_model[cam], rec, kin, Xn, m.x, m.y, r);
          double w, half_rho;
          cauchy_weight(r[0] * r[0] + r[1] * r[1], loss_b, loss_inv_b, w, half_rho);
          if (pt_active && !pt_active[pt]) half_rho = 0.0;
          a_cost += half_rho;
        }
      }
      __syncthreads();
    }
    o0 = o0n; o1 = o1n; o0n = o0nn; o1n = o1nn; cur = nxt;
  }
  const double s0 = block_sum_256(a_step, s_red);
  const double s1 = block_sum_256(a_model, s_red);
  const double s2 = block_sum_256(a_x2, s_red);
  if (threadIdx.x == 0) { partial[3 * blockIdx.x] = s0; partial[3 * blockIdx.x + 1] = s1; partial[3 * blockIdx.x + 2] = s2; }
  if (cost_partial) {
    const double s3 = block_sum_256(a_cost, s_red);
    if (threadIdx.x == 0) cost_partial[blockIdx.x] = s3;
  }
}
int backsub_points_grid(int NP) {
  int gp = (NP + 15) / 16;
  if (gp > 1024) gp = 1024;
  return gp < 1 ? 1 : gp;
}
void launch_backsub_points_jvp(hipStream_t st, int NP, int NPs, int NI, double radius, double dmin, double dmax,
                               const SweepArgs& a, const int* pt_start, const double* delta_cam,
                               const unsigned char* pt_free, const double* Gi, const double* h, const double* Cu,
                               const double* gu, const double* scale_pt, double* cand_points, double* delta_points,
                               double* partial, const double* cand_camrec, const double* cand_intr, double* cost_partial) {
  const int gp = backsub_points_grid(NP);
  const double track = NP > 0 ? (double)a.N / NP : 1.0;
  const int ppb = std::max(1, std::min(128, (int)(224.0 / std::max(track, 1.0))));
  const int nblocks = (NP + ppb - 1) / ppb;
  hipLaunchKernelGGL(k_backsub_points_packed, dim3(gp), dim3(256), 0, st, NP, NPs, NI, a.NC, a.N, ppb, nblocks, radius, dmin, dmax, a.loss_b,
                     a.loss_inv_b, pt_start, a.obs_img, a.obs_pt, a.uv, a.img_cam, a.cam_model, a.camrec, a.intr, delta_cam, pt_free,
                     Gi, h, Cu, gu, scale_pt, a.points, cand_points, delta_points, partial, cand_camrec, cand_intr, a.pt_active,
                     cost_partial);
}

__device__ __forceinline__ void wave_lds_sync() {
  __builtin_amdgcn_fence(__ATOMIC_RELEASE, "wavefront");
  __builtin_amdgcn_wave_barrier();
  __builtin_amdgcn_fence(__ATOMIC_ACQUIRE, "wavefront");
}
template <bool COST>
__global__ void __launch_bounds__(256) k_backsub_points_tiles(
    int num_tiles, const BsTile* __restrict__ tiles, int NPs, int NI, int NC, int N, double radius, double dmin, double dmax,
    double loss_b, double loss_inv_b, const int* __restrict__ pt_start, const int* __restrict__ obs_img,
    const int* __restrict__ obs_pt, const double2* __restrict__ uv, const int* __restrict__ img_cam,
    const int* __restrict__ cam_model, const double* __restrict__ camrec, const double* __restrict__ intr,
    const double* __restrict__ delta_cam, const unsigned char* __restrict__ pt_free, const double* __restrict__ Gi,
    const double* __restrict__ h, const double* __restrict__ Cu, const double* __restrict__ gu,
    const double* __restrict__ scale_pt, const double* __restrict__ points, double* __restrict__ cand_points,
    double* __restrict__ delta_points, double* __restrict__ partial, const double* __restrict__ cand_camrec,
    const double* __restrict__ cand_intr, const unsigned char* __restrict__ pt_active, double* __restrict__ cost_partial) {
  __shared__ double s_t[4][3][kBsTileObs];
  __shared__ double s_new[4][3][kBsTilePts];
  __shared__ double s_red[4];
  __shared__ double s_acc[4][256];
  __shared__ double s_kin[kBsCamsLds][9], s_dk[kBsCamsLds][9], s_ckin[kBsCamsLds][9];
  __shared__ int s_model[kBsCamsLds];
  const int tid = threadIdx.x, lane = tid & 63;
  const int wv = __builtin_amdgcn_readfirstlane(tid >> 6);
  const bool cams_lds = NC <= kBsCamsLds;
  const int stride = 4 * (int)gridDim.x;
  s_acc[0][tid] = 0.0; s_acc[1][tid] = 0.0; s_acc[2][tid] = 0.0; s_acc[3][tid] = 0.0;
  struct Obs { int pt, im; double2 m; };
  auto load_obs = [&](int o) {
    Obs r{0, 0, make_double2(0.0, 0.0)};
    if (N <= 0) return r;
    const int oc = min(o, N - 1);
    r.pt = obs_pt[oc]; r.im = obs_img[oc]; r.m = uv[oc];
    return r;
  };
  auto load_tile = [&](int t) {
    const int4 v = *reinterpret_cast<const int4*>(tiles + t);
    return BsTile{v.x, v.y, v.z, v.w};
  };
  auto obs_term = [&](const Obs& q, bool valid, double (&t)[3]) {
    t[0] = t[1] = t[2] = 0.0;
    if (!valid || !pt_free[q.pt]) return;
    const int cam = img_cam[q.im];
    const double X[3] = {points[3 * (size_t)q.pt], points[3 * (size_t)q.pt + 1], points[3 * (size_t)q.pt + 2]};
    double rec[9], kin[9], dc[6], dk[9];
#pragma unroll
    for (int k = 0; k < 9; ++k) rec[k] = camrec[9 * q.im + k];
#pragma unroll
    for (int k = 0; k < 6; ++k) dc[k] = delta_cam[6 * q.im + k];
    int model;
    if (cams_lds) {
      model = s_model[cam];
#pragma unroll
      for (int k = 0; k < 9; ++k) { kin[k] = s_kin[cam][k]; dk[k] = s_dk[cam][k]; }
    } else {
      model = cam_model[cam];
#pragma unroll
      for (int k = 0; k < 9; ++k) { kin[k] = intr[9 * cam + k]; dk[k] = delta_cam[6 * NI + 9 * cam + k]; }
    }
    double r[2], tt[3];
    obs_backsub_term(model, rec, kin, X, q.m.x, q.m.y, dc, dk, r, tt);
    double w, half_rho;
    cauchy_weight(r[0] * r[0] + r[1] * r[1], loss_b, loss_inv_b, w, half_rho);
    const double w2 = w * w;
    t[0] = w2 * tt[0]; t[1] = w2 * tt[1]; t[2] = w2 * tt[2];
  };
  int t = 4 * (int)blockIdx.x + wv;
  BsTile T{0, 0, 0, 0}, Tn{0, 0, 0, 0};
  Obs cur{0, 0, make_double2(0.0, 0.0)};
  if (t < num_tiles) {
    T = load_tile(t);
    if (t + stride < num_tiles) Tn = load_tile(t + stride);
    cur = load_obs(T.o0 + lane);
  }
  if (cams_lds) {
    for (int e = tid; e < 9 * NC; e += 256) {
      s_kin[e / 9][e % 9] = intr[e]; s_dk[e / 9][e % 9] = delta_cam[6 * NI + e];
      if constexpr (COST) s_ckin[e / 9][e % 9] = cand_intr[e];
    }
    for (int c = tid; c < NC; c += 256) s_model[c] = cam_model[c];
    __syncthreads();
  }
  for (; t < num_tiles; t += stride) {
    Obs nxt = cur;
    BsTile Tnn{0, 0, 0, 0};
    if (t + stride < num_tiles) {
      nxt = load_obs(Tn.o0 + lane);
      if (t + 2 * stride < num_tiles) Tnn = load_tile(t + 2 * stride);
    }
    const int p = T.p0 + lane;
    const bool owner = lane < T.np;
    int mb = 0, me = 0;
    if (owner) { mb = pt_start[p] - T.o0; me = pt_start[p + 1] - T.o0; }
    double Ts[3] = {0.0, 0.0, 0.0};
    for (int base = 0; base < T.no; base += kBsTileObs) {
      const Obs q = base == 0 ? cur : load_obs(T.o0 + base + lane);
      double tt[3];
      obs_term(q, base + lane < T.no, tt);
      s_t[wv][0][lane] = tt[0]; s_t[wv][1][lane] = tt[1]; s_t[wv][2][lane] = tt[2];
      wave_lds_sync();
      if (owner) {
        const int b = max(mb, base), e = min(me, base + kBsTileObs);
        for (int i = b; i < e; ++i) { Ts[0] += s_t[wv][0][i - base]; Ts[1] += s_t[wv][1][i - base]; Ts[2] += s_t[wv][2][i - base]; }
      }
      wave_lds_sync();
    }
    if (owner) {
      const bool fr = pt_free[p] != 0;
      double a_step = 0.0, a_model = 0.0, a_x2 = 0.0;
      double d[3] = {0, 0, 0}, Xo[3];
#pragma unroll
      for (int k = 0; k < 3; ++k) Xo[k] = points[3 * (size_t)p + k];
      if (fr) {
        const int dg[3] = {0, 3, 5};
        double G[6], sp[3], hh[3], cu[3], gg[3];
#pragma unroll
        for (int k = 0; k < 6; ++k) G[k] = Gi[k * NPs + p];
#pragma unroll
        for (int k = 0; k < 3; ++k) { sp[k] = scale_pt[k * NPs + p]; hh[k] = h[k * NPs + p]; cu[k] = Cu[dg[k] * NPs + p]; gg[k] = gu[k * NPs + p]; }
        const double q0 = -sp[0] * Ts[0], q1 = -sp[1] * Ts[1], q2 = -sp[2] * Ts[2];
        const double z[3] = {q0 * G[0], q0 * G[1] + q1 * G[2], q0 * G[3] + q1 * G[4] + q2 * G[5]};
        const double tt[3] = {hh[0] - z[0], hh[1] - z[1], hh[2] - z[2]};
        double yp[3];
        git_mul(G, tt, yp);
#pragma unroll
        for (int k = 0; k < 3; ++k) {
          const double s = sp[k];
          const double D2 = clampd(s * s * cu[k], dmin, dmax) / radius;
          const double gs = s * gg[k];
          a_model += 0.5 * yp[k] * (gs + D2 * yp[k]);
          d[k] = -yp[k] * s;
          a_step += d[k] * d[k];
        }
      }
#pragma unroll
      for (int k = 0; k < 3; ++k) {
        const double xn = Xo[k] + d[k];
        cand_points[3 * (size_t)p + k] = xn;
        delta_points[3 * (size_t)p + k] = d[k];
        if (fr) a_x2 += xn * xn;
        if constexpr (COST) s_new[wv][k][lane] = xn;
      }
      if (fr) { s_acc[0][tid] += a_step; s_acc[1][tid] += a_model; s_acc[2][tid] += a_x2; }
    }
    if constexpr (COST) {
      wave_lds_sync();
      for (int base = 0; base < T.no; base += kBsTileObs) {
        const Obs q = T.no <= kBsTileObs ? cur : load_obs(T.o0 + base + lane);
        if (base + lane < T.no) {
          const int cam = img_cam[q.im];
          double rec[9], kin[9], r[2];
#pragma unroll
          for (int k = 0; k < 9; ++k) rec[k] = cand_camrec[9 * q.im + k];
          int model;
          if (cams_lds) {
            model = s_model[cam];
#pragma unroll
            for (int k = 0; k < 9; ++k) kin[k] = s_ckin[cam][k];
          } else {
            model = cam_model[cam];
#pragma unroll
            for (int k = 0; k < 9; ++k) kin[k] = cand_intr[9 * cam + k];
          }
          const int j = q.pt - T.p0;
          const double Xn[3] = {s_new[wv][0][j], s_new[wv][1][j], s_new[wv][2][j]};
          obs_residual(model, rec, kin, Xn, q.m.x, q.m.y, r);
          double w, half_rho;
          cauchy_weight(r[0] * r[0] + r[1] * r[1], loss_b, loss_inv_b, w, half_rho);
          if (pt_active && !pt_active[q.pt]) half_rho = 0.0;
          s_acc[3][tid] += half_rho;
        }
      }
      wave_lds_sync();
    }
    T = Tn; Tn = Tnn; cur = nxt;
  }
  const double s0 = block_sum_256(s_acc[0][tid], s_red);
  const double s1 = block_sum_256(s_acc[1][tid], s_red);
  const double s2 = block_sum_256(s_acc[2][tid], s_red);
  if (tid == 0) { partial[3 * blockIdx.x] = s0; partial[3 * blockIdx.x + 1] = s1; partial[3 * blockIdx.x + 2] = s2; }
  if constexpr (COST) {
    const double s3 = block_sum_256(s_acc[3][tid], s_red);
    if (tid == 0) cost_partial[blockIdx.x] = s3;
  }
}
int backsub_tiles_grid(int num_tiles) { return std::max(1, std::min(768, (num_tiles + 3) / 4)); }
void launch_backsub_points_tiles(hipStream_t st, int num_tiles, const BsTile* tiles, int NPs, int NI, double radius, double dmin,
                                 double dmax, const SweepArgs& a, const int* pt_start, const double* delta_cam,
                                 const unsigned char* pt_free, const double* Gi, const double* h, const double* Cu,
                                 const double* gu, const double* scale_pt, double* cand_points, double* delta_points,
                                 double* partial, const double* cand_camrec, const double* cand_intr, double* cost_partial) {
  with_bool(cost_partial != nullptr, [&](auto cost) {
    hipLaunchKernelGGL((k_backsub_points_tiles<decltype(cost)::value>), dim3(backsub_tiles_grid(num_tiles)), dim3(256), 0, st, num_tiles,
                       tiles, NPs, NI, a.NC, a.N, radius, dmin, dmax, a.loss_b, a.loss_inv_b, pt_start, a.obs_img, a.obs_pt, a.uv, a.img_cam,
                       a.cam_model, a.camrec, a.intr, delta_cam, pt_free, Gi, h, Cu, gu, scale_pt, a.points, cand_points, delta_points,
                       partial, cand_camrec, cand_intr, a.pt_active, cost_partial);
  });
}

int update_cameras_groups(int NI) { return std::max(1, (NI + kUpdImagesPerGroup - 1) / kUpdImagesPerGroup); }
__global__ void __launch_bounds__(256) k_update_cameras(
    int NI, int NC, int cam_part, double radius, double dmin, double dmax, const double* __restrict__ y,
    const double* __restrict__ scale_cam, const double* __restrict__ img_rec, const double* __restrict__ cam_rec,
    const double* __restrict__ poses, const double* __restrict__ intr, double* cand_poses,
    double* __restrict__ cand_intr, double* __restrict__ delta_cam, double* __restrict__ partial3,
    double* __restrict__ cand_camrec) {
  __shared__ double s_red[4];
  update_cameras_body(blockIdx.x, NI, NC, cam_part, radius, dmin, dmax, y, scale_cam, img_rec, cam_rec, poses, intr, cand_poses, cand_intr,
                      delta_cam, partial3, cand_camrec, s_red);
}
void launch_update_cameras(hipStream_t st, const CamUpdateArgs& u, const double* y) {
  hipLaunchKernelGGL(k_update_cameras, dim3(update_cameras_groups(u.NI)), dim3(256), 0, st, u.NI, u.NC, u.cam_part, u.radius, u.dmin,
                     u.dmax, y, u.scale_cam, u.img_rec, u.cam_rec, u.poses, u.intr, u.cand_poses, u.cand_intr, u.delta_cam, u.partial3,
                     u.cand_camrec);
}

__global__ void __launch_bounds__(256) k_reduce_tasks(ReduceTasks T, LmSpec spec) {
  __shared__ double s_red[4];
  if (!lm_spec_go(spec, nullptr)) return;
  reduce_task_body(T.t[blockIdx.x], s_red);
}
__global__ void __launch_bounds__(64) k_lm_snapshot(LmSpec spec, double* dec, double* host_pub, double seq, double* fail_slots) {
  lm_snapshot_body(threadIdx.x, spec, dec, host_pub, seq, fail_slots);
}
__global__ void __launch_bounds__(1024) k_lm_tail(ReduceTasks T, int n, LmSpec spec, double* dec, double* host_pub, double seq, double* fail_slots) {
  __shared__ double s_t[4][2][4];
  reduce_tasks_grouped(T, n, s_t);
  if (threadIdx.x < 64) lm_snapshot_body(threadIdx.x, spec, dec, host_pub, seq, fail_slots);
}
__global__ void __launch_bounds__(1024) k_eval_small(EvalTailArgs a) {
  if (!lm_spec_go(a.spec, nullptr)) return;
  eval_tail_body<true>(a);
}
void launch_eval_small(hipStream_t st, const EvalTailArgs& a) { hipLaunchKernelGGL(k_eval_small, dim3(1), dim3(1024), 0, st, a); }
__global__ void __launch_bounds__(256) k_eval_head(EvalTailArgs a, int img_blocks) {
  __shared__ double s_red[4];
  if (!lm_spec_go(a.spec, nullptr)) return;
  if ((int)blockIdx.x < img_blocks) {
    const int i = 4 * blockIdx.x + (threadIdx.x >> 6);
    if (i < a.NI) camera_reduce_img_body(i, threadIdx.x & 63, a.img_chunk_start, a.cam_partial, a.prior_start, a.prior_res, a.prior_jac, a.img_rec, a.img_intr_tmp);
    return;
  }
  if ((int)blockIdx.x >= img_blocks + a.gp) {
    const int task = 4 * ((int)blockIdx.x - img_blocks - a.gp) + (threadIdx.x >> 6);
    if (task < a.ride.n) partial_reduce_task(a.ride.tasks[task], threadIdx.x & 63, a.ride.pp, a.ride.ip, a.ride.ii);
    return;
  }
  state_norms_body(blockIdx.x - img_blocks, a.gp, a.gc, a.NI, a.NC, a.NP, a.NPs, a.cam_part, a.pose_free, a.intr_free, a.pt_free, a.poses, a.intr,
                   a.points, a.img_rec, a.cam_rec, a.gu, a.norm_partial, s_red);
}
__global__ void __launch_bounds__(1024) k_eval_tail(EvalTailArgs a) {
  if (!lm_spec_go(a.spec, nullptr)) return;
  eval_tail_body<false>(a);
}
void launch_eval_head_tail(hipStream_t st, const EvalTailArgs& a) {
  const int img_blocks = (a.NI + 3) / 4;
  hipLaunchKernelGGL(k_eval_head, dim3(img_blocks + a.gp + (a.ride.n + 3) / 4), dim3(256), 0, st, a, img_blocks);
  EvalTailArgs b = a;
  b.first_group = a.gp;
  hipLaunchKernelGGL(k_eval_tail, dim3(1), dim3(1024), 0, st, b);
}
void launch_lm_tail(hipStream_t st, const ReduceTasks& T, int n, const LmSpec& spec, double* dec, double* host_pub, double seq, double* fail_slots) {
  if (n > 4) {
    launch_reduce_tasks(st, T, n);
    launch_lm_snapshot(st, spec, dec, host_pub, seq, fail_slots);
    return;
  }
  hipLaunchKernelGGL(k_lm_tail, dim3(1), dim3(1024), 0, st, T, n, spec, dec, host_pub, seq, fail_slots);
}
__global__ void k_lm_decide_cases(int n, const double* __restrict__ in, double* __restrict__ out) {
  const int c = blockIdx.x * blockDim.x + threadIdx.x;
  if (c >= n) return;
  const double* q = in + (size_t)c * (SC_COUNT + 8);
  LmSpec sp = lm_spec_off();
  sp.radius = q[SC_COUNT]; sp.decrease_factor = q[SC_COUNT + 1]; sp.ptol = q[SC_COUNT + 2]; sp.ftol = q[SC_COUNT + 3];
  sp.min_rel_dec = q[SC_COUNT + 4]; sp.max_radius = q[SC_COUNT + 5]; sp.abs_gtol = q[SC_COUNT + 6]; sp.pending_eval = q[SC_COUNT + 7] != 0.0;
  const LmDecision d = lm_decide(q, sp);
  double* o = out + (size_t)c * 6;
  o[0] = (double)d.code; o[1] = d.radius; o[2] = d.decrease_factor; o[3] = d.rel; o[4] = d.step_norm; o[5] = d.cost_change;
}
void launch_lm_decide_cases(hipStream_t st, int n, const double* in, double* out) {
  if (n > 0) hipLaunchKernelGGL(k_lm_decide_cases, dim3((n + 255) / 256), dim3(256), 0, st, n, in, out);
}
void launch_lm_snapshot(hipStream_t st, const LmSpec& spec, double* dec, double* host_pub, double seq, double* fail_slots) {
  hipLaunchKernelGGL(k_lm_snapshot, dim3(1), dim3(64), 0, st, spec, dec, host_pub, seq, fail_slots);
}
void launch_reduce_tasks(hipStream_t st, const ReduceTasks& T, int n, const LmSpec& spec) {
  if (n > 0) hipLaunchKernelGGL(k_reduce_tasks, dim3(n), dim3(256), 0, st, T, spec);
}

__global__ void k_points_to_caller(int NP, int width, const int* __restrict__ orig, const double* __restrict__ in, double* __restrict__ out) {
  const int t = blockIdx.x * blockDim.x + threadIdx.x;
  if (t >= NP * width) return;
  const int q = t / width, e = t - q * width;
  out[(size_t)orig[q] * width + e] = in[t];
}
void launch_points_to_caller(hipStream_t st, int NP, int width, const int* orig, const double* in, double* out) {
  if (NP <= 0) return;
  hipLaunchKernelGGL(k_points_to_caller, dim3((NP * width + 255) / 256), dim3(256), 0, st, NP, width, orig, in, out);
}

__global__ void k_point_errors(int NP, const int* __restrict__ pt_start, const double* __restrict__ rnorm,
                               const int* __restrict__ pt_count, double* __restrict__ perr) {
  const int p = blockIdx.x * blockDim.x + threadIdx.x;
  if (p >= NP) return;
  const double cnt = (double)pt_count[p];
  double s = 0.0;
  for (int o = pt_start[p]; o < pt_start[p + 1]; ++o) s += rnorm[o] / cnt;
  perr[p] = s;
}
void launch_point_errors(hipStream_t st, int NP, const int* pt_start, const double* rnorm,
                         const int* pt_count, double* perr) {
  if (NP <= 0) return;
  hipLaunchKernelGGL(k_point_errors, dim3((NP + 255) / 256), dim3(256), 0, st, NP, pt_start, rnorm, pt_count, perr);
}

}
```

### mavmap_amd/csrc/lm_bodies.h

```cpp
#ifndef MAVBA_LM_BODIES_H_
#define MAVBA_LM_BODIES_H_
#include "internal.h"
#include "ba_math.h"
#include "dev_reduce.h"
#include "lm_decide.h"

namespace mavba {

__device__ __forceinline__ void camera_reduce_img_elem(int i, int e, const int* img_chunk_start, const double* partial,
                                                        const int* prior_start, const double* prior_res, const double* prior_jac,
                                                        double* img_rec, double* img_intr_tmp) {
  const int c0 = img_chunk_start[i], c1 = img_chunk_start[i + 1];
  double s = 0.0;
  int c = c0;
  for (; c + 4 <= c1; c += 4) {
    const double x0 = partial[(size_t)c * kSweepAcc + e], x1 = partial[(size_t)(c + 1) * kSweepAcc + e];
    const double x2 = partial[(size_t)(c + 2) * kSweepAcc + e], x3 = partial[(size_t)(c + 3) * kSweepAcc + e];
    s += x0; s += x1; s += x2; s += x3;
  }
  for (; c < c1; ++c) s += partial[(size_t)c * kSweepAcc + e];
  if (e < 27 && prior_start) {
    for (int q = prior_start[i]; q < prior_start[i + 1]; ++q) {
      const double* j = prior_jac + 3 * q;
      if (e < 21) {
        int x = 0, rem = e;
        while (rem >= 6 - x) { rem -= 6 - x; ++x; }
        const int y = x + rem;
        if (y < 3) s += j[x] * j[y];
      } else if (e - 21 < 3) {
        s += j[e - 21] * prior_res[q];
      }
    }
  }
  if (e < kImgRec) img_rec[(size_t)i * kImgRec + e] = s;
  else img_intr_tmp[(size_t)i * kCamRec + (e - kImgRec)] = s;
}
__device__ __forceinline__ void camera_reduce_img_body(int i, int lane, const int* img_chunk_start, const double* partial,
                                                       const int* prior_start, const double* prior_res, const double* prior_jac,
                                                       double* img_rec, double* img_intr_tmp) {
  for (int e = lane; e < kSweepAcc; e += 64)
    camera_reduce_img_elem(i, e, img_chunk_start, partial, prior_start, prior_res, prior_jac, img_rec, img_intr_tmp);
}

__device__ __forceinline__ double camera_reduce_cam_part(int c, int part, int e, const int* cam_img_start, const int* cam_imgs,
                                                         const double* img_intr_tmp) {
  double s = 0.0;
  const int t1 = cam_img_start[c + 1];
  for (int t = cam_img_start[c] + part; t < t1; t += 16) s += img_intr_tmp[(size_t)cam_imgs[t] * kCamRec + e];
  return s;
}

__device__ __forceinline__ void state_norms_local(int vb, int lt, int gp, int gc, int NI, int NC, int NP, int NPs, int cam_part,
                                                  const unsigned char* pose_free, const unsigned char* intr_free,
                                                  const unsigned char* pt_free, const double* poses, const double* intr,
                                                  const double* points, const double* img_rec, const double* cam_rec,
                                                  const double* gu, double& gmax, double& x2) {
  gmax = 0.0; x2 = 0.0;
  if (vb < gp) {
    for (int p = vb * 256 + lt; p < NP; p += gp * 256) {
      if (!pt_free[p]) continue;
#pragma unroll
      for (int k = 0; k < 3; ++k) {
        gmax = fmax(gmax, fabs(gu[k * NPs + p]));
        const double x = points[3 * (size_t)p + k];
        x2 += x * x;
      }
    }
  } else {
    const int ncam = 6 * NI + 9 * NC;
    for (int t = (vb - gp) * 256 + lt; t < ncam; t += gc * 256) {
      double g, x; bool fr;
      if (t < 6 * NI) {
        fr = pose_free[t] != 0; g = img_rec[(size_t)(t / 6) * kImgRec + 21 + t % 6]; x = poses[t];
      } else {
        const int c = (t - 6 * NI) / 9, k = (t - 6 * NI) % 9;
        fr = intr_free[9 * c + k] != 0; g = cam_rec[(size_t)c * kCamRec + 45 + k]; x = intr[9 * c + k];
      }
      if (!fr) continue;
      gmax = fmax(gmax, fabs(g));
      if (cam_part) x2 += x * x;
    }
  }
}
__device__ __forceinline__ void state_norms_body(int vb, int gp, int gc, int NI, int NC, int NP, int NPs, int cam_part,
                                                 const unsigned char* pose_free, const unsigned char* intr_free,
                                                 const unsigned char* pt_free, const double* poses, const double* intr,
                                                 const double* points, const double* img_rec, const double* cam_rec,
                                                 const double* gu, double* partial, double* s_red) {
  double gmax, x2;
  state_norms_local(vb, threadIdx.x, gp, gc, NI, NC, NP, NPs, cam_part, pose_free, intr_free, pt_free, poses, intr, points, img_rec, cam_rec,
                    gu, gmax, x2);
  const double m = block_max_256(gmax, s_red);
  const double s = block_sum_256(x2, s_red);
  if (threadIdx.x == 0) { partial[2 * vb] = m; partial[2 * vb + 1] = s; }
}

__device__ __forceinline__ double group4_sum(const double* w) { return (w[0] + w[1]) + (w[2] + w[3]); }
__device__ __forceinline__ double group4_max(const double* w) { return fmax(fmax(w[0], w[1]), fmax(w[2], w[3])); }

__device__ __forceinline__ void reduce_task_body(const ReduceTask& t, double* s_red) {
  double v = 0.0;
  for (int r = threadIdx.x; r < t.rows; r += 256) {
    const double x = t.src[(size_t)r * t.stride];
    v = t.is_max ? fmax(v, x) : v + x;
  }
  double total = t.is_max ? block_max_256(v, s_red) : block_sum_256(v, s_red);
  if (t.rows2 > 0) {
    __syncthreads();
    double w = 0.0;
    for (int r = threadIdx.x; r < t.rows2; r += 256) w += t.src2[r];
    total += block_sum_256(w, s_red);
  }
  if (threadIdx.x == 0) *t.out = total;
}

__device__ __forceinline__ void reduce_tasks_grouped(const ReduceTasks& T, int n, double (*s_t)[2][4]) {
  const int tid = threadIdx.x, g = tid >> 8, lt = tid & 255, wv = (tid >> 6) & 3, lane = tid & 63;
  if (g < n) {
    const ReduceTask t = T.t[g];
    double v = 0.0;
    for (int r = lt; r < t.rows; r += 256) {
      const double x = t.src[(size_t)r * t.stride];
      v = t.is_max ? fmax(v, x) : v + x;
    }
    const double red = t.is_max ? wave_max(v) : wave_sum(v);
    double w = 0.0;
    for (int r = lt; r < t.rows2; r += 256) w += t.src2[r];
    const double red2 = wave_sum(w);
    if (lane == 0) { s_t[g][0][wv] = red; s_t[g][1][wv] = red2; }
  }
  __syncthreads();
  if (tid < n) {
    const ReduceTask t = T.t[tid];
    double total = t.is_max ? group4_max(s_t[tid][0]) : group4_sum(s_t[tid][0]);
    if (t.rows2 > 0) total += group4_sum(s_t[tid][1]);
    *t.out = total;
  }
  __syncthreads();
}

template <bool IMAGES>
__device__ __forceinline__ void eval_tail_body(const EvalTailArgs& a) {
  __shared__ double s_part[16][64];
  __shared__ double s_w[kStateNormsCamBlocks][2][4];
  __shared__ double s_t[4][2][4];
  const int tid = threadIdx.x, g = tid >> 8, lt = tid & 255, wv = (tid >> 6) & 3, lane = tid & 63;
  if constexpr (IMAGES) {
    for (int q = tid; q < a.NI * kSweepAcc; q += 1024)
      camera_reduce_img_elem(q / kSweepAcc, q % kSweepAcc, a.img_chunk_start, a.cam_partial, a.prior_start, a.prior_res, a.prior_jac, a.img_rec,
                             a.img_intr_tmp);
    __syncthreads();
  }
  if (a.with_cams) {
    for (int c = 0; c < a.NC; ++c) {
      if (lane < kCamRec) s_part[tid >> 6][lane] = camera_reduce_cam_part(c, tid >> 6, lane, a.cam_img_start, a.cam_imgs, a.img_intr_tmp);
      __syncthreads();
      if (tid < kCamRec) {
        double tot = 0.0;
#pragma unroll
        for (int k = 0; k < 16; ++k) tot += s_part[k][tid];
        a.cam_rec[(size_t)c * kCamRec + tid] = tot;
      }
      __syncthreads();
    }
  }
  const int nvb = a.gp + a.gc;
  for (int vb0 = a.first_group; vb0 < nvb; vb0 += 4) {
    const int vb = vb0 + g;
    if (vb < nvb) {
      double gmax, x2;
      state_norms_local(vb, lt, a.gp, a.gc, a.NI, a.NC, a.NP, a.NPs, a.cam_part, a.pose_free, a.intr_free, a.pt_free, a.poses, a.intr, a.points,
                        a.img_rec, a.cam_rec, a.gu, gmax, x2);
      const double m = wave_max(gmax), sum = wave_sum(x2);
      if (lane == 0) { s_w[vb - a.first_group][0][wv] = m; s_w[vb - a.first_group][1][wv] = sum; }
    }
  }
  __syncthreads();
  if (tid < nvb - a.first_group) {
    a.norm_partial[2 * (a.first_group + tid)] = group4_max(s_w[tid][0]);
    a.norm_partial[2 * (a.first_group + tid) + 1] = group4_sum(s_w[tid][1]);
  }
  __syncthreads();
  reduce_tasks_grouped(a.T, a.num_tasks, s_t);
}

constexpr int kUpdImagesPerGroup = 42;
__device__ __forceinline__ void update_cameras_body(int vb, int NI, int NC, int cam_part, double radius, double dmin, double dmax,
                                                    const double* y, const double* scale_cam, const double* img_rec,
                                                    const double* cam_rec, const double* poses, const double* intr,
                                                    double* cand_poses, double* cand_intr, double* delta_cam, double* partial3,
                                                    double* cand_camrec, double* s_red) {
  const int i0 = vb * kUpdImagesPerGroup, i1 = min(i0 + kUpdImagesPerGroup, NI);
  double a_step = 0.0, a_model = 0.0, a_x2 = 0.0;
  auto one = [&](int t) {
    const double s = scale_cam[t];
    double n2, g, x;
    if (t < 6 * NI) {
      const int i = t / 6, e = t % 6;
      n2 = img_rec[(size_t)i * kImgRec + sym_idx(e, e, 6)]; g = img_rec[(size_t)i * kImgRec + 21 + e]; x = poses[t];
    } else {
      const int c = (t - 6 * NI) / 9, k = (t - 6 * NI) % 9;
      n2 = cam_rec[(size_t)c * kCamRec + sym_idx(k, k, 9)]; g = cam_rec[(size_t)c * kCamRec + 45 + k]; x = intr[9 * c + k];
    }
    double d = 0.0;
    if (s != 0.0) {
      const double yy = y[t];
      const double D2 = clampd(s * s * n2, dmin, dmax) / radius;
      d = -yy * s;
      if (cam_part) { a_model += 0.5 * yy * (s * g + D2 * yy); a_step += d * d; }
    }
    const double xn = x + d;
    if (s != 0.0 && cam_part) a_x2 += xn * xn;
    delta_cam[t] = d;
    if (t < 6 * NI) cand_poses[t] = xn; else cand_intr[t - 6 * NI] = xn;
  };
  for (int t = 6 * i0 + threadIdx.x; t < 6 * i1; t += 256) one(t);
  if (vb == 0)
    for (int t = 6 * NI + threadIdx.x; t < 6 * NI + 9 * NC; t += 256) one(t);
  const double s0 = block_sum_256(a_step, s_red);
  const double s1 = block_sum_256(a_model, s_red);
  const double s2 = block_sum_256(a_x2, s_red);
  if (threadIdx.x == 0) { partial3[3 * vb] = s0; partial3[3 * vb + 1] = s1; partial3[3 * vb + 2] = s2; }
  if (cand_camrec) {
    __syncthreads();
    for (int i = i0 + threadIdx.x; i < i1; i += 256) {
      double rec[9];
      cam_prepare(cand_poses + 6 * i, rec);
#pragma unroll
      for (int k = 0; k < 9; ++k) cand_camrec[9 * i + k] = rec[k];
    }
  }
}

__device__ __forceinline__ void lm_snapshot_body(int lane, const LmSpec& spec, double* dec, double* host_pub, double seq, double* fail_slots) {
  const LmDecision d = lm_decide(spec.scal, spec);
  if (lane == 0) { dec[0] = (double)d.code; dec[1] = d.radius; }
  volatile double* out = host_pub;
  double v = 0.0;
  if (lane < SC_COUNT) v = spec.scal[lane];
  else if (lane == SC_COUNT) v = (double)d.code;
  else if (lane == SC_COUNT + 1) v = d.radius;
  else if (lane == SC_COUNT + 2) v = d.decrease_factor;
  else if (lane == SC_COUNT + 3) v = d.rel;
  else if (lane == SC_COUNT + 4) v = d.step_norm;
  else if (lane == SC_COUNT + 5) v = d.cost_change;
  if (lane < SC_COUNT + 6) out[lane] = v;
  __threadfence_system();
  __builtin_amdgcn_wave_barrier();
  if (lane == 0) out[SC_COUNT + 7] = seq;
  if (lane < 2 && fail_slots) fail_slots[lane] = 0.0;
}

}
#endif
```

### mavmap_amd/csrc/session.h

```cpp
#ifndef MAVBA_SESSION_H_
#define MAVBA_SESSION_H_
#include <algorithm>
#include <chrono>
#include <cmath>
#include <cstdio>
#include <cstdlib>
#include <cstring>
#include <condition_variable>
#include <functional>
#include <limits>
#include <map>
#include <memory>
#include <mutex>
#include <shared_mutex>
#include <stdexcept>
#include <string>
#include <thread>
#include <unordered_map>
#include <vector>

#include "../../include/mavba.h"
#include "../../include/mavba_triangulate.h"
#include "../../include/mavba_backsub_tiles.h"
#include "../../include/mavba_absolute_pose.h"
// ... 127 lines not shown

template <typename T>
struct PinnedBuf {
  T* p = nullptr;
  size_t n = 0;
  bool pinned = true;
  explicit PinnedBuf(size_t count) : n(count) {
    void* q = nullptr;
    const size_t bytes = std::max<size_t>(count, 1) * sizeof(T);
    if (pinned_alloc(&q, bytes) != hipSuccess) {
      (void)hipGetLastError();
      pinned = false;
      q = host_scratch_alloc(bytes);
    }
    p = static_cast<T*>(q);
  }
  PinnedBuf(const PinnedBuf&) = delete;
  PinnedBuf& operator=(const PinnedBuf&) = delete;
  ~PinnedBuf() { if (pinned) pinned_free(p); else host_scratch_free(p, std::max<size_t>(n, 1) * sizeof(T)); }
  T& operator[](size_t i) { return p[i]; }
  const T& operator[](size_t i) const { return p[i]; }
  T* data() { return p; }
};

template <typename KeyFn, typename EmitFn>
static void counting_sort_parallel(long long n, int nkeys, KeyFn key, std::vector<int>& start, EmitFn emit) {
  int T = n >= 200000 ? host_threads() : 1;
  while (T > 1 && (size_t)T * nkeys > ((size_t)64 << 20)) T /= 2;
  HostBuf<int> hist_store((size_t)T * nkeys);
  std::vector<int*> hist(T);
  for (int t = 0; t < T; ++t) hist[t] = hist_store.data() + (size_t)t * nkeys;
  auto run = [&](const std::function<void(int)>& body) { host_run(T, body); };
  run([&](int t) {
    std::memset(hist[t], 0, (size_t)nkeys * sizeof(int));
    for (long long i = n * t / T; i < n * (t + 1) / T; ++i) hist[t][key(i)]++;
  });
  start.assign((size_t)nkeys + 1, 0);
  std::vector<long long> range_sum((size_t)T + 1, 0);
  run([&](int r) {
    long long sum = 0;
    for (long long k = (long long)nkeys * r / T; k < (long long)nkeys * (r + 1) / T; ++k) {
      int within = 0;
      for (int t = 0; t < T; ++t) { const int c = hist[t][k]; hist[t][k] = within; within += c; }
      start[k] = within;
      sum += within;
    }
    range_sum[r + 1] = sum;
  });
  for (int r = 0; r < T; ++r) range_sum[r + 1] += range_sum[r];
  run([&](int r) {
    int pos = (int)range_sum[r];
    for (long long k = (long long)nkeys * r / T; k < (long long)nkeys * (r + 1) / T; ++k) {
      const int tot = start[k];
      start[k] = pos;
      for (int t = 0; t < T; ++t) hist[t][k] += pos;
      pos += tot;
    }
  });
  start[nkeys] = (int)range_sum[T];
  run([&](int t) {
    for (long long i = n * t / T; i < n * (t + 1) / T; ++i) emit(i, hist[t][key(i)]++);
  });
}

static inline int model_k(int m) { return m == MAVBA_MODEL_PINHOLE ? 4 : m == MAVBA_MODEL_OPENCV ? 8 : 9; }
static inline int round_up(int x, int m) { return (x + m - 1) / m * m; }
static inline double now_s() {
  return std::chrono::duration<double>(std::chrono::steady_clock::now().time_since_epoch()).count();
}

struct KernelTimer { std::string name; long long launches = 0; double total_ms = 0.0; };

template <typename F>
static void parallel_ranges(long long n, F&& body, long long min_parallel = 200000) {
  int T = (int)std::min<long long>(host_threads(), std::max<long long>(n, 1));
  if (n < min_parallel) T = 1;
  if (T == 1) { body(0ll, n); return; }
  host_run(T, [&](int t) { body(n * t / T, n * (t + 1) / T); });
}

}

using namespace mavba;

struct mavba_session {
  mavba_options opt;
  int device = 0;
  hipStream_t st = nullptr;
  int NI = 0, NC = 0, NP = 0, N = 0, Nstride = 32, NPs = 32, KMAX = 4, n_full = 0, n_pad = 64, Q = 0;
  long long NO_all = 0;
  bool any_intr_free = false;
  std::vector<double> h_poses0, h_intr0, h_points0;
  std::vector<int> h_cam_model, h_img_cam, h_pt_start, h_oimg;
  std::vector<long long> perm;
  std::vector<int> h_pt_count_all;
  std::vector<double> h_dropped_rnorm;
  std::vector<double> h_dropped_cost;
  double fixed_cost_priors = 0.0;
  int num_priors_all = 0;
  std::vector<unsigned char> h_pt_removed;
  DevBuf<unsigned char> d_pt_active;
  std::vector<int> h_pt_orig;
  std::vector<unsigned char> h_pose_const, h_intr_const_in, h_pt_const_in;
  std::vector<unsigned char> h_img_used, h_cam_used, h_pt_used;
  std::vector<unsigned char> h_prior_on_img;
  std::vector<unsigned char> h_pose_free, h_intr_free, h_pt_free;
  double fixed_cost = 0.0;
  long long num_residuals = 0, num_residuals_reduced = 0, num_parameters_reduced = 0;
  int num_priors = 0;
  double prior_weight = 0.0;
  double setup_seconds = 0.0, solve_seconds = 0.0;

  DevBuf<double2> d_uv, d_im_uv;
  DevBuf<int> d_obs_img, d_obs_pt, d_pt_start, d_im_pt, d_img_cam, d_cam_model, d_img_chunk_start,
      d_cam_img_start, d_cam_imgs, d_prior_img, d_prior_start, d_q_pt, d_q_cam, d_q_start, d_pt_count;
  DevBuf<FrontTile> d_front_tiles;
  int num_front_tiles = 0;
  DevBuf<FrontTile> d_tail_tiles;
  int num_tail_tiles = 0, tail_begin = 0;
  bool front_ok = false;
  bool fused_ok = false;
  int eval_rows = 0;
  bool front_valid = false;
  double front_radius = 0.0;
  bool fail_slot_clean = false;
  bool planes_ready = false;
  DevBuf<BsTile> d_bs_tiles;
  int num_bs_tiles = 0;
  int backsub_blocks = -1;
  void read_backsub_switch();
  bool backsub_on_tiles() const { return backsub_blocks < 0 ? !small_window() : backsub_blocks == 0; }
  int backsub_rows() const { return backsub_on_tiles() ? backsub_tiles_grid(num_bs_tiles) : backsub_points_grid(NP); }
  DevBuf<SweepChunk> d_sweep_chunks;
  int num_sweep_chunks = 0;
  DevBuf<unsigned char> d_pose_free, d_intr_free, d_pt_free;
  DevBuf<double> d_prior_R0;
  DevBuf<SchurBlock> d_blocks;
  DevBuf<SchurChunk> d_chunks[3];
  DevBuf<SchurCluster> d_clusters;
  DevBuf<SchurRowsCluster> d_rows_clusters;
  DevBuf<int> d_rows_lists;
  DevBuf<unsigned> d_rows_emit;
  DevBuf<unsigned long long> d_rows_lanes;
  int rows_class_count[kRowsClasses] = {};
  bool rows_ok = false;
  bool rows_generic = false;
  DevBuf<PartialReduce> d_reduce_tasks;
  int num_reduce_tasks = 0;
  DevBuf<int> d_cl_tab, d_cl_lists;
  DevBuf<unsigned short> d_obs_meta, d_q_meta;
  DevBuf<unsigned char> d_pt_clustered;
  int num_clusters = 0, num_slots[3] = {0, 0, 0};
  long long clustered_points = 0, cluster_partials = 0;
  double cluster_flops = 0.0;
  DevBuf<int2> d_terms[3];
  int num_blocks = 0, num_chunks[3] = {0, 0, 0};
  long long num_terms[3] = {0, 0, 0};
  DevBuf<double> d_poses, d_intr, d_points, d_cposes, d_cintr, d_cpoints, d_poses0, d_intr0, d_points0;
  DevBuf<double> d_camrec, d_ccamrec;
  bool camrec_current = false;
  DevBuf<double> d_R, d_Jp, d_Jc, d_Jk, d_Cu, d_gu, d_Gi, d_h, d_scale_cam, d_scale_pt;
  DevBuf<double> d_sweep_partial, d_camsum , d_img_intr_tmp, d_cam_partial;
  DevBuf<double> d_prior_res, d_prior_jac, d_prior_cost;
  DevBuf<double> d_Epose, d_Eintr, d_Wk, d_part[3];
  DevBuf<double> d_M, d_L, d_y, d_diag_ws, d_delta_cam, d_delta_pts, d_norm_partial, d_step_partial, d_scal;
  DevBuf<double> d_rnorm, d_perr;
  DevBuf<int> d_pt_orig;
  DevBuf<int> d_perm32;
  DevBuf<double> d_pts_out;
  double* d_img_rec = nullptr;
  double* d_cam_rec = nullptr;
  CholStructure chol_struct;
  bool prereduced = false;
  bool sweep_rode_along = false;
  bool setup_batched = false;
  bool M_is_clean = false;
  bool allow_persistent = true;
  bool persist_decided = false;
  bool speculate_on = true;
  void decide_persistent();
  int n_mat = 64, nd_parts = 0;
  std::vector<int> h_off_img, h_off_cam, h_col_var;
  DevBuf<int> d_off, d_col_var;
  DevBuf<double> d_ymat;
  DevBuf<int> d_ar_tiles;
  DevBuf<double> d_ar_buf;
  int num_ar_tiles = 0;

  bool evaluated = false, scales_ready = false, started = false, assembled = false;
  double radius = 1e4, decrease_factor = 2.0;
  double cost = 0.0, x_norm = 0.0, grad_max = 0.0, abs_gtol = 0.0, initial_cost = 0.0;
  int iteration = 0, invalid_steps = 0, n_success = 0, n_fail = 0;
  int termination = MAVBA_TERM_RUNNING;

  mavba_allreduce_fn ar_fn = nullptr;
  void* ar_ctx = nullptr;
  void* rccl_comm = nullptr;
  bool rccl_comm_owned = true;
  std::shared_ptr<RcclGuard> rccl_guard;
  bool sharded() const { return (ar_fn || rccl_comm) && (world > 1 || force_exchange); }
  bool force_exchange = false;
  int rank = 0, world = 1;

  std::vector<KernelTimer> timers;
  struct Pending { int idx; hipEvent_t a, b; bool own_a = true; };
  std::vector<Pending> pending;
  std::vector<hipEvent_t> ev_pool;

  ~mavba_session() {
    if (st) (void)hipStreamSynchronize(st);
    if (rccl_comm && rccl_comm_owned) rccl_comm_destroy(rccl_comm);
    if (lm_pub) lm_pub_free(lm_pub);
    HostSpare<long long>::give(perm); HostSpare<int>::give(h_oimg); HostSpare<double>::give(h_points0);
    for (auto& p : pending) { (void)hipEventDestroy(p.a); (void)hipEventDestroy(p.b); }
    for (auto& e : ev_pool) (void)hipEventDestroy(e);
    if (st) stream_release(st, device);
  }

  int timer_index(const char* name) {
    for (size_t i = 0; i < timers.size(); ++i) if (timers[i].name == name) return (int)i;
    timers.push_back(KernelTimer{name, 0, 0.0});
    return (int)timers.size() - 1;
  }
  hipEvent_t get_event() {
    if (!ev_pool.empty()) { hipEvent_t e = ev_pool.back(); ev_pool.pop_back(); return e; }
    hipEvent_t e; HIP_OK(hipEventCreate(&e)); return e;
  }
  template <typename F>
  void timed(const char* name, F&& f) {
    if (!opt.profile_kernels) { f(); return; }
    Pending p; p.idx = timer_index(name); p.a = get_event(); p.b = get_event();
    HIP_OK(hipEventRecord(p.a, st));
    f();
    HIP_OK(hipEventRecord(p.b, st));
    pending.push_back(p);
  }
  template <typename F>
  void timed_split(const char* first, const char* second, F&& f) {
    if (!opt.profile_kernels) { f(nullptr); return; }
    Pending p, q;
    p.idx = timer_index(first); q.idx = timer_index(second);
    p.a = get_event(); p.b = get_event(); q.a = p.b; q.b = get_event(); q.own_a = false;
    HIP_OK(hipEventRecord(p.a, st));
    f(p.b);
    HIP_OK(hipEventRecord(q.b, st));
    pending.push_back(p); pending.push_back(q);
  }
  void flush_timers() {
    for (auto& p : pending) {
      float ms = 0.f;
      if (hipEventElapsedTime(&ms, p.a, p.b) == hipSuccess) { timers[p.idx].launches++; timers[p.idx].total_ms += ms; }
      if (p.own_a) ev_pool.push_back(p.a);
      ev_pool.push_back(p.b);
    }
    pending.clear();
  }
  void sync() { HIP_OK(hipStreamSynchronize(st)); HIP_OK(hipGetLastError()); release_staged(st); flush_timers(); }
  void download(void* dst, const void* src, size_t bytes) { HIP_OK(copy_d2h_staged_sync(dst, src, bytes, st)); release_staged(st); }

  void allreduce(double* dptr, long long count, int op) {
    if (!sharded()) return;
    if (rccl_comm) {
      if (rccl_guard) {
        std::shared_lock<std::shared_mutex> lk(rccl_guard->m);
        if (rccl_guard->aborted) throw Failure(MAVBA_ERR_HIP, "the communicator group was aborted (another rank failed)");
        rccl_allreduce(rccl_comm, dptr, count, op, st);
      } else {
        rccl_allreduce(rccl_comm, dptr, count, op, st);
      }
      return;
    }
    sync();
    if (ar_fn(ar_ctx, dptr, count, op) != 0) throw Failure(MAVBA_ERR_HIP, "all-reduce hook failed");
  }

  SweepArgs sweep_args(const double* camrec, const double* intr, const double* points) {
    SweepArgs a;
    a.N = N; a.Nstride = Nstride; a.NI = NI; a.NC = NC; a.KMAX = KMAX;
    a.uv = d_uv.p; a.obs_img = d_obs_img.p; a.obs_pt = d_obs_pt.p;
    a.camrec = camrec; a.intr = intr; a.img_cam = d_img_cam.p; a.cam_model = d_cam_model.p;
    a.points = points;
    a.pt_active = h_pt_removed.empty() ? nullptr : d_pt_active.p;
    a.loss_b = opt.loss_scale_factor * opt.loss_scale_factor; a.loss_inv_b = 1.0 / a.loss_b;
    a.R = d_R.p; a.Jp = d_Jp.p; a.Jc = d_Jc.p; a.Jk = d_Jk.p; a.cost_partial = d_sweep_partial.p;
    return a;
  }
  void read_scalars(double* h) {
    HIP_OK(hipMemcpyAsync(h, d_scal.p, SC_COUNT * sizeof(double), hipMemcpyDeviceToHost, st));
    sync();
  }

  void build(const mavba_problem* P, const DeviceRaw* raw = nullptr);
void intr_entries_on_device(const std::vector<unsigned char>& cam_active, std::vector<int>& q_start, std::vector<int>& q_cam);
    void order_on_device(const mavba_problem* P, std::vector<int>& img_start, const DeviceRaw* raw);
  void order_on_host(const mavba_problem* P, const long long* keptp, std::vector<int>& img_start,
                     std::unique_ptr<PinnedBuf<double2>>& uv_h, std::unique_ptr<PinnedBuf<int>>& opt_h,
                     std::unique_ptr<PinnedBuf<double2>>& im_uv_h, std::unique_ptr<PinnedBuf<int>>& im_pt_h);
  void ensure_perm_host();
  void derive_free_flags();
  void finish_structure();
  void choose_elimination_order(const std::vector<SchurBlock>& blocks);
  void reset_state();
  void evaluate(double next_radius = -1.0);
  void evaluate_enqueue(double next_radius = -1.0, const LmSpec& spec = lm_spec_off());
  EvalTailArgs eval_tail_args(const LmSpec& spec);
  CamUpdateArgs cam_update_args(double r);
  void launch_front(double r, bool entries, const LmSpec& spec = lm_spec_off(), const CamSweepArgs* with_sweep = nullptr);
  DevBuf<double> d_lm_dec;
  double* lm_pub = nullptr;
  double lm_seq = 0.0;
  LmSpec lm_spec(bool pending_eval) const {
    LmSpec sp{};
    sp.dec = nullptr; sp.scal = d_scal.p;
    sp.radius = radius; sp.decrease_factor = decrease_factor;
    sp.ptol = opt.parameter_tolerance; sp.ftol = opt.function_tolerance; sp.min_rel_dec = opt.min_relative_decrease;
    sp.max_radius = opt.max_trust_region_radius; sp.abs_gtol = abs_gtol; sp.pending_eval = pending_eval ? 1 : 0;
    return sp;
  }
  bool wait_publication(double* h);
  void build_front_tiles(const std::vector<int>& q_start);
  void build_tiles(const std::vector<int>& q_start, int first, DevBuf<FrontTile>& out, int& count);
  void ensure_planes();
  bool fused_now() const { return fused_ok && rows_ok; }
  int eval_cost_rows() const { return front_ok ? eval_rows : (N > 0 ? jacobian_sweep_grid(N) : 0); }
  void take_evaluation(const double* h) { cost = h[SC_COST]; grad_max = h[SC_GRAD_MAX]; x_norm = std::sqrt(h[SC_XNORM2]); }
  void assemble(double r);
  void solve_linear(double r);
  void linear_step(double r, double* h_scal);
  void candidate(double r, double* h_scal);
  void candidate_enqueue(double r, ReduceTasks* tail = nullptr, int* tail_count = nullptr);
  bool merge_small() const;
  bool small_window() const;
  bool merge_on = true;
  long long sweep_ride_max_obs = -1;
  double pub_wait_seconds = 0.0;
  bool cameras_updated = false;
  double cameras_updated_r = 0.0;
  void start();
  int iterate(int max_iters, int* done);
  void point_errors(double* out);
  void restart();
  long long filter_points(double max_error, const unsigned char* keep, unsigned char* removed_out, double* errors_out);
  void restore_initial_params() {
    HIP_OK(hipMemcpyAsync(d_poses.p, d_poses0.p, (size_t)NI * 6 * 8, hipMemcpyDeviceToDevice, st));
    HIP_OK(hipMemcpyAsync(d_intr.p, d_intr0.p, (size_t)NC * 9 * 8, hipMemcpyDeviceToDevice, st));
    HIP_OK(hipMemcpyAsync(d_points.p, d_points0.p, (size_t)NP * 3 * 8, hipMemcpyDeviceToDevice, st));
    camrec_current = false; evaluated = false; front_valid = false;
  }
  void apply_filter_state();
  void to_caller_points(const double* internal, double* out, int width) const {
    for (int q = 0; q < NP; ++q)
      for (int e = 0; e < width; ++e) out[(size_t)h_pt_orig[q] * width + e] = internal[(size_t)q * width + e];
  }
  void fill_result(mavba_result* r);
};
#endif
```

### mavmap_amd/csrc/session_build.hip

```cpp
#include "session.h"
#include <array>
#include <map>

using namespace mavba;


void mavba_session::derive_free_flags() {
  h_pose_free.assign((size_t)NI * 6, 0);
  h_intr_free.assign((size_t)NC * 9, 0);
  h_pt_free.assign(NP, 0);
  for (int i = 0; i < NI; ++i) {
    if (!h_img_used[i]) continue;
    const unsigned m = h_pose_const[i];
    for (int e = 0; e < 6; ++e) {
      const bool c = e < 3 ? (m & MAVBA_CONST_RVEC) != 0 : (m & (MAVBA_CONST_TX << (e - 3))) != 0;
      h_pose_free[(size_t)i * 6 + e] = c ? 0 : 1;
    }
  }
  any_intr_free = false;
  for (int c = 0; c < NC; ++c) {
    if (!h_cam_used[c] || h_intr_const_in[c]) continue;
    for (int k = 0; k < model_k(h_cam_model[c]); ++k) h_intr_free[(size_t)c * 9 + k] = 1;
    any_intr_free = true;
  }
// ... 1078 lines not shown
  auto run_threads = [&](const std::function<void(int)>& body) { host_run(T, body); };
  if (generic_points > 0)
    run_threads([&](int t) {
      for (int k = 0; k < 3; ++k) tcount[t * 3 + k].assign(nkeys[k], 0);
      enumerate(range[t], range[t + 1], [&](int kind, int r, int c, int, int) { tcount[t * 3 + kind][(size_t)r * ncols[kind] + c]++; });
    });
  std::vector<int> count[3];
  std::vector<unsigned char> mandatory[3];
  long long tot[3] = {0, 0, 0};
  for (int k = 0; k < 3; ++k) {
    count[k].assign(nkeys[k], 0);
    mandatory[k].assign(nkeys[k], 0);
    if (generic_points > 0) {
      std::mutex tot_m;
      parallel_ranges((long long)nkeys[k], [&](long long b0, long long b1) {
        long long sum = 0;
        for (long long key = b0; key < b1; ++key) {
          int c = 0;
          for (int t = 0; t < T; ++t) c += tcount[t * 3 + k][(size_t)key];
          count[k][(size_t)key] = c;
          sum += c;
        }
        std::lock_guard<std::mutex> g(tot_m);
        tot[k] += sum;
      }, 1 << 18);
    }
  }
  for (int i = 0; i < NI; ++i) {
    if (!img_active[i]) continue;
    mandatory[BLK_PP][(size_t)i * NI + i] = 1;
    if (cam_active[h_img_cam[i]]) mandatory[BLK_IP][(size_t)h_img_cam[i] * NI + i] = 1;
  }
  for (int c = 0; c < NC; ++c) if (cam_active[c]) mandatory[BLK_II][(size_t)c * NC + c] = 1;
  std::vector<int> cref[3];
  for (int k = 0; k < 3; ++k) cref[k].assign(nkeys[k], 0);
  std::vector<unsigned char> slot_a(kClTab), slot_b(kClTab);
  for (int la = 0, sl = kClTabPP; la < kClImages; ++la) for (int lb = 0; lb <= la; ++lb, ++sl) { slot_a[sl] = (unsigned char)la; slot_b[sl] = (unsigned char)lb; }
  for (int sl = kClTabIP; sl < kClTabII; ++sl) { slot_a[sl] = (unsigned char)((sl - kClTabIP) / kClImages); slot_b[sl] = (unsigned char)((sl - kClTabIP) % kClImages); }
  for (int lc = 0, sl = kClTabII; lc < kClCams; ++lc) for (int ld = 0; ld <= lc; ++ld, ++sl) { slot_a[sl] = (unsigned char)lc; slot_b[sl] = (unsigned char)ld; }
  auto cluster_key = [&](long long cl, int slot, int& kind) -> size_t {
    const int* imgs = &cl_imgs[(size_t)cl * kClImages];
    const int* cams = &cl_cams[(size_t)cl * kClCams];
    if (slot < kClTabIP) { kind = BLK_PP; return (size_t)imgs[slot_a[slot]] * NI + imgs[slot_b[slot]]; }
    if (slot < kClTabII) { kind = BLK_IP; return (size_t)cams[slot_a[slot]] * NI + imgs[slot_b[slot]]; }
    kind = BLK_II;
    return (size_t)cams[slot_a[slot]] * NC + cams[slot_b[slot]];
  };
  cluster_partials = 0;
  for (long long cl = 0; cl < num_clusters; ++cl)
    for (int sl = 0; sl < kClTab; ++sl)
      if (cl_present[(size_t)cl * kClTab + sl]) { int kind; const size_t key = cluster_key(cl, sl, kind); cref[kind][key]++; ++cluster_partials; }
  lap("count terms");
  for (int k = 0; k < 3; ++k)
    if (tot[k] >= (1ll << 31) - 1) throw Failure(MAVBA_ERR_INVALID_ARGUMENT, "more than 2^31 Schur terms of one kind");
  auto block_chunk_terms = [](int cnt) {
    int nch = (cnt + 1023) / 1024;
    nch = std::max(1, std::min(nch, 256));
    return std::max(1, (cnt + nch - 1) / nch);
  };
  std::vector<SchurBlock> blocks;
  std::vector<SchurChunk> chunks[3];
  std::vector<int> cursor[3];
  int kTile = 4;
  if (const char* e = std::getenv("MAVBA_PP_TILE")) kTile = std::max(1, std::atoi(e));
  for (int k = 0; k < 3; ++k) {
    cursor[k].assign(count[k].size(), 0);
    std::vector<size_t> keys;
    {
      const long long nk = (long long)count[k].size();
      const int slices = nk >= (1 << 18) ? 64 : 1;
      std::vector<std::vector<size_t>> part(slices);
      parallel_ranges(slices, [&](long long s0, long long s1) {
        for (long long sl = s0; sl < s1; ++sl) {
          const long long b0 = nk * sl / slices, b1 = nk * (sl + 1) / slices;
          for (long long key = b0; key < b1; ++key)
            if (count[k][(size_t)key] != 0 || mandatory[k][(size_t)key] || cref[k][(size_t)key] != 0) part[sl].push_back((size_t)key);
        }
      }, 2);
      size_t total = 0;
      for (const auto& v : part) total += v.size();
      keys.reserve(total);
      for (const auto& v : part) keys.insert(keys.end(), v.begin(), v.end());
    }
    if (k == BLK_PP || k == BLK_IP) {
      const unsigned long long nc = (unsigned long long)ncols[k];
      std::vector<std::pair<unsigned long long, size_t>> ranked(keys.size());
      for (size_t q = 0; q < keys.size(); ++q) {
        const unsigned long long a = keys[q], ia = a / nc, ja = a % nc;
        ranked[q] = {k == BLK_PP ? ((ia / kTile) << 42 | (ja / kTile) << 21 | 0) : ja, q};
      }
      std::stable_sort(ranked.begin(), ranked.end(), [](const auto& x, const auto& y) { return x.first < y.first; });
      std::vector<size_t> sorted(keys.size());
      for (size_t q = 0; q < keys.size(); ++q) sorted[q] = keys[ranked[q].second];
      keys.swap(sorted);
    }
    int off = 0, slot = 0;
    for (size_t key : keys) {
      const int cnt = count[k][key];
      SchurBlock B;
      B.kind = k; B.row_ent = (int)(key / ncols[k]); B.col_ent = (int)(key % ncols[k]);
      B.chunk_begin = slot;
      const int ct = block_chunk_terms(cnt);
      for (int b0 = off; b0 < off + cnt; b0 += ct)
        chunks[k].push_back(SchurChunk{b0, std::min(b0 + ct, off + cnt), slot++});
      const int nref = cref[k][key];
      cref[k][key] = slot;
      slot += nref;
      B.chunk_end = slot;
      blocks.push_back(B);
      cursor[k][key] = off;
      off += cnt;
    }
    num_slots[k] = slot;
  }
  std::vector<PartialReduce> reduce_tasks;
  const int kPreReduceFrom = N < 200000 ? 256 : 64;
  for (SchurBlock& B : blocks) {
    const int n = B.chunk_end - B.chunk_begin;
    if (n <= kPreReduceFrom) continue;
    const int first = num_slots[B.kind];
    for (int b0 = B.chunk_begin; b0 < B.chunk_end; b0 += 32)
      reduce_tasks.push_back(PartialReduce{B.kind, b0, std::min(b0 + 32, B.chunk_end), num_slots[B.kind]++});
    B.chunk_begin = first; B.chunk_end = num_slots[B.kind];
  }
  num_reduce_tasks = (int)reduce_tasks.size();
  d_reduce_tasks.upload(reduce_tasks, st);
  std::vector<int> cl_tab((size_t)std::max(num_clusters, 1) * kClTab, -1);
  for (long long cl = 0; cl < num_clusters; ++cl)
    for (int sl = 0; sl < kClTab; ++sl)
      if (cl_present[(size_t)cl * kClTab + sl]) { int kind; const size_t key = cluster_key(cl, sl, kind); cl_tab[(size_t)cl * kClTab + sl] = cref[kind][key]++; }
  lap("order blocks + chunks");
  std::unique_ptr<int2[]> terms[3];
  for (int k = 0; k < 3; ++k) terms[k].reset(new int2[std::max<size_t>((size_t)tot[k], 1)]);
  if (generic_points > 0) {
    for (int k = 0; k < 3; ++k)
      parallel_ranges((long long)nkeys[k], [&](long long b0, long long b1) {
        for (long long key = b0; key < b1; ++key) {
          int run = cursor[k][(size_t)key];
          for (int t = 0; t < T; ++t) { const int c = tcount[t * 3 + k][(size_t)key]; tcount[t * 3 + k][(size_t)key] = run; run += c; }
        }
      }, 1 << 18);
    run_threads([&](int t) {
      enumerate(range[t], range[t + 1], [&](int kind, int r, int c, int x, int y) {
        terms[kind][(size_t)tcount[t * 3 + kind][(size_t)r * ncols[kind] + c]++] = make_int2(x, y);
      });
    });
  }
  lap("fill terms");
  choose_elimination_order(blocks);
  lap("elimination order");
  num_blocks = (int)blocks.size();
  d_blocks.upload(blocks, st);
  for (int k = 0; k < 3; ++k) {
    num_chunks[k] = (int)chunks[k].size();
    num_terms[k] = tot[k];
    d_chunks[k].upload(chunks[k], st);
    d_terms[k].alloc(std::max<size_t>((size_t)tot[k], 1));
    if (tot[k]) HIP_OK(copy_h2d_staged(d_terms[k].p, terms[k].get(), (size_t)tot[k] * sizeof(int2), st));
    d_part[k].alloc((size_t)std::max(num_slots[k], 1) * schur_partial_stride(k));
  }
  {
    std::vector<unsigned char> ptc(std::max(NP, 1), 0);
    for (int p = 0; p < NP; ++p) ptc[p] = pt_mode[p] == 1;
    std::vector<int> order(num_clusters);
    for (int c = 0; c < num_clusters; ++c) order[c] = c;
    auto row_class = [&](int c) { return rows_ok ? rows_class_of_rows(rows_count(cl_ni[c], cl_kr[c])) : 0; };
    auto weight = [&](int c) {
      const int np = clusters[c].p1 - clusters[c].p0;
      if (!rows_ok) return (long long)np;
      const int nt = kRowsClassNT[row_class(c)];
      return (long long)((np + kRowsBatch - 1) / kRowsBatch) * (60 + nt * (nt + 1) / 2);
    };
    std::stable_sort(order.begin(), order.end(), [&](int a, int b) { return weight(a) > weight(b); });
    if (rows_ok) {
      std::vector<SchurRowsCluster> rc(clusters.size());
      for (int k = 0; k < kRowsClasses; ++k) rows_class_count[k] = 0;
      rows_generic = false;
      for (int c = 0; c < num_clusters; ++c) rows_generic = rows_generic || cl_nc[c] > 2;
      d_rows_lanes.upload(rows_lanes, st);
      std::vector<unsigned> emit_all, e0, e1;
      std::map<std::pair<int, int>, std::array<int, 3>> emit_of;
      for (int c = 0; c < num_clusters; ++c) {
        const int o = order[c];
        int kslot[kClCamsMax] = {0, 0, 0};
        for (int k = 0; k < cl_nc[o] && k < kClCamsMax; ++k) kslot[k] = model_k(h_cam_model[cl_cams[(size_t)o * kClCams + k]]);
        const int flags = rows_pack_flags(cl_unplaced[o] != 0, kslot, cl_nc[o]);
        auto it = emit_of.find({cl_ni[o], flags >> 8});
        if (it == emit_of.end()) {
          rows_emit_map(cl_ni[o], cl_nc[o], flags, e0, e1);
          it = emit_of.emplace(std::make_pair(cl_ni[o], flags >> 8), std::array<int, 3>{(int)emit_all.size(), (int)e0.size(), (int)e1.size()}).first;
          emit_all.insert(emit_all.end(), e0.begin(), e0.end());
          emit_all.insert(emit_all.end(), e1.begin(), e1.end());
        }
        rc[c] = SchurRowsCluster{clusters[o].p0, clusters[o].p1, cl_ni[o], cl_nc[o], it->second[0], {it->second[1], it->second[2]}, flags};
        rows_class_count[row_class(o)]++;
      }
      d_rows_clusters.upload(rc, st);
      d_rows_emit.upload(emit_all, st);
      std::vector<int> rl((size_t)std::max(num_clusters, 1) * kRowsLists, -1);
      for (int c = 0; c < num_clusters; ++c) {
        const int o = order[c];
        int* L = &rl[(size_t)c * kRowsLists];
        for (int k = 0; k < kClImages; ++k) { const int img = cl_imgs[(size_t)o * kClImages + k]; L[k] = img; L[kRowsListsCam + k] = img >= 0 ? h_img_cam[img] : -1; }
        for (int k = 0; k < kClCams; ++k) L[kRowsListsCams + k] = cl_cams[(size_t)o * kClCams + k];
      }
      d_rows_lists.upload(rl, st);
      if (std::getenv("MAVBA_CLUSTER_STATS")) {
        long long pts[kRowsClasses] = {}, bat[kRowsClasses] = {};
        for (int c = 0; c < num_clusters; ++c) { const int k = row_class(order[c]); pts[k] += rc[c].p1 - rc[c].p0; bat[k] += (rc[c].p1 - rc[c].p0 + kRowsBatch - 1) / kRowsBatch; }
        for (int k = 0; k < kRowsClasses; ++k)
          std::fprintf(stderr, "[cluster stats] k_schur_rows class %d (%d rows): %d clusters, %lld points, %lld batches\n", k, 16 * kRowsClassNT[k], rows_class_count[k], pts[k], bat[k]);
        long long hist[kClImagesMax + 1][kClCamsMax + 1][2] = {}, unplaced = 0;
        for (int c = 0; c < num_clusters; ++c) { hist[rc[c].ni][rc[c].nc][0]++; hist[rc[c].ni][rc[c].nc][1] += (rc[c].p1 - rc[c].p0 + kRowsBatch - 1) / kRowsBatch; unplaced += (rc[c].flags & kRowsUnplaced) != 0; }
        std::fprintf(stderr, "[cluster stats] k_schur_rows clusters / batches by (images, cameras):");
        for (int i = 0; i <= kClImagesMax; ++i) for (int k = 0; k <= kClCamsMax; ++k) if (hist[i][k][0]) std::fprintf(stderr, " (%d,%d) %lld/%lld", i, k, hist[i][k][0], hist[i][k][1]);
        std::fprintf(stderr, "; clusters that keep the selects: %lld\n", unplaced);
      }
    }
    std::vector<SchurCluster> cl_sorted(clusters.size());
    std::vector<int> tab_sorted(cl_tab.size(), -1);
    std::vector<int> lists_sorted((size_t)std::max(num_clusters, 1) * (kClImages + kClCams), -1);
    for (int c = 0; c < num_clusters; ++c) {
      cl_sorted[c] = clusters[order[c]];
      std::copy(cl_tab.begin() + (size_t)order[c] * kClTab, cl_tab.begin() + (size_t)(order[c] + 1) * kClTab, tab_sorted.begin() + (size_t)c * kClTab);
    }
    for (int c = 0; c < num_clusters; ++c) {
      std::copy(cl_imgs.begin() + (size_t)order[c] * kClImages, cl_imgs.begin() + (size_t)(order[c] + 1) * kClImages, lists_sorted.begin() + (size_t)c * (kClImages + kClCams));
      std::copy(cl_cams.begin() + (size_t)order[c] * kClCams, cl_cams.begin() + (size_t)(order[c] + 1) * kClCams, lists_sorted.begin() + (size_t)c * (kClImages + kClCams) + kClImages);
    }
    d_clusters.upload(cl_sorted, st); d_cl_tab.upload(tab_sorted, st); d_cl_lists.upload(lists_sorted, st);
    d_obs_meta.upload(obs_meta, st); d_q_meta.upload(q_meta, st); d_pt_clustered.upload(ptc, st);
  }
  {
    long long head_observed = 0, head_clustered = 0;
    for (int p = 0; p < tail_begin; ++p) { head_observed += h_pt_start[p + 1] > h_pt_start[p]; head_clustered += pt_mode[p] == 1; }
    const bool no_fuse = std::getenv("MAVBA_NO_FUSE") != nullptr;
    fused_ok = front_ok && !no_fuse && num_clusters > 0 && head_clustered == head_observed &&
               clustered_points == head_clustered && num_clusters <= kFrontMaxGrid;
    num_tail_tiles = 0;
    if (fused_ok && h_pt_start[NP] > h_pt_start[tail_begin]) {
      build_tiles(q_start, tail_begin, d_tail_tiles, num_tail_tiles);
      if ((long long)num_clusters + point_front_grid(num_tail_tiles) > kFrontMaxGrid) { fused_ok = false; num_tail_tiles = 0; }
    }
    rows_ok = rows_ok && fused_ok;
  }
  if (!setup_batched) sync();
  lap("upload terms");
}

void mavba_session::build_front_tiles(const std::vector<int>& q_start) {
  const bool planes_only = std::getenv("MAVBA_FRONT_PLANES") != nullptr;
  front_ok = !planes_only;
  for (int p = 0; p < NP && front_ok; ++p)
    if (q_start[p + 1] - q_start[p] > kFrontQ) front_ok = false;
  num_front_tiles = 0;
  if (front_ok) build_tiles(q_start, 0, d_front_tiles, num_front_tiles);
  else d_front_tiles.upload(std::vector<FrontTile>(), st);
  front_valid = false;
  if (!front_ok) ensure_planes();
}
void mavba_session::build_tiles(const std::vector<int>& q_start, int first, DevBuf<FrontTile>& out, int& count) {
  std::vector<FrontTile> tiles;
  int p0 = first, obs = 0, qs = 0;
  for (int p = first; p < NP; ++p) {
    const int c = h_pt_start[p + 1] - h_pt_start[p], nq = q_start[p + 1] - q_start[p];
    if (p > p0 && (obs + c > kFrontObs || p - p0 >= kFrontPts || qs + nq > kFrontQ)) {
      tiles.push_back(FrontTile{p0, p, h_pt_start[p0], h_pt_start[p], q_start[p0], q_start[p]});
      p0 = p; obs = 0; qs = 0;
    }
    obs += c; qs += nq;
  }
  if (NP > p0) tiles.push_back(FrontTile{p0, NP, h_pt_start[p0], h_pt_start[NP], q_start[p0], q_start[NP]});
  count = (int)tiles.size();
  out.upload(tiles, st);
}

namespace mavba {
std::vector<BsTile> build_backsub_tiles(const int* pt_start, int NP) {
  std::vector<BsTile> tiles;
  int p = 0;
  while (p < NP) {
    const int p0 = p, o0 = pt_start[p];
    if (pt_start[p + 1] - o0 > kBsTileObs) { ++p; }
    else
      while (p < NP && p - p0 < kBsTilePts && pt_start[p + 1] - o0 <= kBsTileObs) ++p;
    tiles.push_back(BsTile{p0, p - p0, o0, pt_start[p] - o0});
  }
  return tiles;
}
}

void mavba_session::reset_state() {
  front_valid = false;
  if (!h_pt_removed.empty()) {
    h_pt_removed.clear();
    apply_filter_state();
    M_is_clean = false;
  }
  HIP_OK(hipMemcpyAsync(d_poses.p, d_poses0.p, (size_t)NI * 6 * 8, hipMemcpyDeviceToDevice, st));
  HIP_OK(hipMemcpyAsync(d_intr.p, d_intr0.p, (size_t)NC * 9 * 8, hipMemcpyDeviceToDevice, st));
  HIP_OK(hipMemcpyAsync(d_points.p, d_points0.p, (size_t)NP * 3 * 8, hipMemcpyDeviceToDevice, st));
  evaluated = scales_ready = started = assembled = false;
  camrec_current = false;
  radius = opt.initial_trust_region_radius; decrease_factor = 2.0;
  cost = x_norm = grad_max = abs_gtol = initial_cost = 0.0;
  iteration = invalid_steps = n_success = n_fail = 0;
  termination = MAVBA_TERM_RUNNING;
  solve_seconds = 0.0;
}
```

### mavmap_amd/csrc/session_lm.hip

```cpp
#include "session.h"
#include "lm_decide.h"
#if defined(__x86_64__) || defined(__i386__)
#include <immintrin.h>
#define MAVBA_CPU_RELAX() _mm_pause()
#else
#include <thread>
#define MAVBA_CPU_RELAX() std::this_thread::yield()
#endif

using namespace mavba;


void mavba_session::ensure_planes() {
  if (planes_ready) return;
  d_R.alloc((size_t)2 * Nstride); d_Jp.alloc((size_t)6 * Nstride); d_Jc.alloc((size_t)12 * Nstride);
  d_Jk.alloc((size_t)2 * KMAX * Nstride);
  d_Wk.alloc((size_t)std::max(Q, 1) * 27);
  planes_ready = true;
}

void mavba_session::launch_front(double r, bool entries, const LmSpec& spec, const CamSweepArgs* with_sweep) {
  sweep_rode_along = false;
  prereduced = false;
  FrontArgs f;
  f.spec = spec;
  f.sw = sweep_args(d_camrec.p, d_intr.p, d_points.p);
  f.num_tiles = num_front_tiles; f.NPs = NPs; f.tiles = d_front_tiles.p;
  f.pt_start = d_pt_start.p; f.q_start = d_q_start.p; f.q_cam = d_q_cam.p; f.q_pt = d_q_pt.p;
  f.pt_free = d_pt_free.p; f.scale_cam = d_scale_cam.p; f.scale_pt = d_scale_pt.p;
  f.radius = r; f.dmin = opt.min_lm_diagonal; f.dmax = opt.max_lm_diagonal;
  f.Cu = d_Cu.p; f.gu = d_gu.p; f.Gi = d_Gi.p; f.h = d_h.p; f.Epose = d_Epose.p; f.Eintr = d_Eintr.p;
  f.fail = d_scal.p + SC_FAIL_FRONT;
  f.trace = nullptr;
  static_assert(SC_FAIL_FRONT == SC_FAIL + 1, "the two failure slots are cleared together");
  if (entries) { if (!spec.dec) HIP_OK(hipMemsetAsync(d_scal.p + SC_FAIL, 0, 2 * sizeof(double), st)); fail_slot_clean = true; }
  if (entries && fused_now()) {
    const bool forms_agree = (Q == 0 && !any_intr_free) || (Q > 0 && any_intr_free);
    const CamSweepArgs* ride = (with_sweep && forms_agree) ? with_sweep : nullptr;
    timed("schur_fused", [&] {
      launch_schur_rows(st, f, Q > 0 ? KMAX : 0, rows_generic, num_clusters, d_rows_clusters.p, d_cl_tab.p, d_rows_lists.p, d_obs_meta.p,
                        d_rows_lanes.p, d_rows_emit.p, d_part[0].p, d_part[1].p, d_part[2].p, ride);
    });
    sweep_rode_along = ride != nullptr;
    eval_rows = num_clusters;
    if (num_tail_tiles > 0) {
      FrontArgs t = f;
      t.tiles = d_tail_tiles.p; t.num_tiles = num_tail_tiles;
      t.sw.cost_partial = f.sw.cost_partial + num_clusters;
      timed("point_front", [&] { launch_point_front(st, t, Q > 0 ? KMAX : 0, true); });
      eval_rows += point_front_grid(num_tail_tiles);
    }
  } else {
    timed(entries ? "point_front" : "point_front_sums", [&] { launch_point_front(st, f, Q > 0 ? KMAX : 0, entries); });
    eval_rows = point_front_grid(num_front_tiles);
  }
  front_valid = entries;
  front_radius = r;
}

EvalTailArgs mavba_session::eval_tail_args(const LmSpec& spec) {
  EvalTailArgs e;
  e.NI = NI; e.NC = NC; e.NP = NP; e.NPs = NPs; e.with_cams = any_intr_free ? 1 : 0; e.cam_part = rank == 0 ? 1 : 0;
  state_norms_grid(NI, NC, NP, &e.gp, &e.gc);
  e.img_chunk_start = d_img_chunk_start.p; e.cam_partial = d_cam_partial.p;
  e.prior_start = num_priors > 0 ? d_prior_start.p : nullptr; e.prior_res = d_prior_res.p; e.prior_jac = d_prior_jac.p;
  e.cam_img_start = d_cam_img_start.p; e.cam_imgs = d_cam_imgs.p; e.img_rec = d_img_rec; e.cam_rec = d_cam_rec;
  e.img_intr_tmp = d_img_intr_tmp.p;
  e.pose_free = d_pose_free.p; e.intr_free = d_intr_free.p; e.pt_free = d_pt_free.p;
  e.poses = d_poses.p; e.intr = d_intr.p; e.points = d_points.p; e.gu = d_gu.p; e.norm_partial = d_norm_partial.p;
  const int rows = e.gp + e.gc;
  e.T.t[0] = ReduceTask{d_norm_partial.p, rows, 2, 1, nullptr, 0, d_scal.p + SC_GRAD_MAX};
  e.T.t[1] = ReduceTask{d_norm_partial.p + 1, rows, 2, 0, nullptr, 0, d_scal.p + SC_XNORM2};
  e.T.t[2] = ReduceTask{d_sweep_partial.p, eval_cost_rows(), 1, 0, d_prior_cost.p, num_priors, d_scal.p + SC_COST};
  e.num_tasks = 3;
  e.spec = spec;
  return e;
}

CamUpdateArgs mavba_session::cam_update_args(double r) {
  CamUpdateArgs u;
  u.NI = NI; u.NC = NC; u.cam_part = rank == 0 ? 1 : 0; u.radius = r; u.dmin = opt.min_lm_diagonal; u.dmax = opt.max_lm_diagonal;
  u.scale_cam = d_scale_cam.p; u.img_rec = d_img_rec; u.cam_rec = d_cam_rec; u.poses = d_poses.p; u.intr = d_intr.p;
  u.cand_poses = d_cposes.p; u.cand_intr = d_cintr.p; u.delta_cam = d_delta_cam.p;
  u.partial3 = d_step_partial.p + 3 * (size_t)backsub_rows(); u.cand_camrec = d_ccamrec.p;
  return u;
}

void mavba_session::evaluate_enqueue(double next_radius, const LmSpec& spec) {
  if (!camrec_current) timed("cam_prepare", [&] { launch_cam_prepare(st, NI, d_poses.p, d_camrec.p); });
  camrec_current = true;
  SweepArgs a = sweep_args(d_camrec.p, d_intr.p, d_points.p);
  CamSweepArgs c;
  c.NI = NI; c.NC = NC; c.chunks = d_sweep_chunks.p; c.num_chunks = num_sweep_chunks;
  c.im_uv = d_im_uv.p; c.im_pt = d_im_pt.p; c.camrec = d_camrec.p; c.intr = d_intr.p;
  c.img_cam = d_img_cam.p; c.cam_model = d_cam_model.p; c.points = d_points.p;
  c.pt_active = a.pt_active;
  c.loss_b = a.loss_b; c.loss_inv_b = a.loss_inv_b; c.partial = d_cam_partial.p;
  c.spec = spec;
  sweep_rode_along = false;
  if (front_ok) {
    constexpr long long kProfiledRideMaxObs = 1000000;
    const bool size_ok = (sweep_ride_max_obs < 0 || N <= sweep_ride_max_obs) && !(opt.profile_kernels && N > kProfiledRideMaxObs);
    const bool ride = scales_ready && num_sweep_chunks > 0 && (merge_small() || (merge_on && !sharded() && size_ok));
    launch_front(next_radius, scales_ready && next_radius > 0.0, spec, ride ? &c : nullptr);
  } else {
    ensure_planes();
    front_valid = false;
    timed("jacobian_sweep", [&] { launch_jacobian_sweep(st, a); });
    timed("point_reduce", [&] {
      launch_point_reduce(st, NP, NPs, Nstride, KMAX, d_pt_start.p, d_q_start.p, d_q_cam.p, d_obs_img.p, d_img_cam.p,
                          d_R.p, d_Jp.p, d_Jk.p, d_Cu.p, d_gu.p, d_Wk.p);
    });
  }
  if (!sweep_rode_along) timed("camera_sweep", [&] { launch_camera_sweep(st, c, KMAX, any_intr_free); });
  PartialRide pride;
  static const bool pride_on = [] { const char* e = std::getenv("MAVBA_PARTIAL_RIDE"); return !e || std::atoi(e) != 0; }();
  if (pride_on && merge_on && front_ok && front_valid && fused_now() && num_reduce_tasks > 0 && num_chunks[0] + num_chunks[1] + num_chunks[2] == 0 &&
      num_tail_tiles == 0 && !sharded() && !opt.profile_kernels) {
    pride.n = num_reduce_tasks; pride.tasks = d_reduce_tasks.p; pride.pp = d_part[0].p; pride.ip = d_part[1].p; pride.ii = d_part[2].p;
  }
  if (num_priors > 0)
    timed("rot_prior", [&] {
      launch_rot_prior(st, num_priors, d_prior_img.p, d_prior_R0.p, prior_weight, d_poses.p, d_prior_res.p,
                       d_prior_jac.p, d_prior_cost.p, spec);
    });
  EvalTailArgs e = eval_tail_args(spec);
  if (scales_ready && merge_small()) {
    timed("eval_small", [&] { launch_eval_small(st, e); });
    evaluated = true; assembled = false;
    return;
  }
  e.ride = pride;
  prereduced = pride.n > 0;
  if (scales_ready && merge_on && !sharded() && NI <= 160) {
    timed("eval_tail", [&] { launch_eval_head_tail(st, e); });
    evaluated = true; assembled = false;
    return;
  }
  timed("camera_reduce", [&] { launch_camera_reduce(st, e); });
  allreduce(d_camsum.p, (long long)NI * kImgRec + (long long)NC * kCamRec, 0);
  if (!scales_ready) {
    timed("scales", [&] {
      launch_scales(st, NI, NC, NP, NPs, opt.jacobi_scaling, d_pose_free.p, d_intr_free.p, d_pt_free.p, d_img_rec,
                    d_cam_rec, d_Cu.p, d_scale_cam.p, d_scale_pt.p);
    });
    scales_ready = true;
  }
  timed("state_norms", [&] { launch_state_norms(st, e); });
  timed("reduce", [&] { launch_reduce_tasks(st, e.T, e.num_tasks, spec); });
  if (sharded()) allreduce(d_scal.p + SC_COST, SC_EVAL_COUNT, 2);
  evaluated = true; assembled = false;
}
void mavba_session::evaluate(double next_radius) {
  evaluate_enqueue(next_radius);
  double h[SC_COUNT];
  read_scalars(h);
  take_evaluation(h);
}

void mavba_session::assemble(double r) {
  const double dmin = opt.min_lm_diagonal, dmax = opt.max_lm_diagonal;
  if (front_ok) {
    if (!(front_valid && front_radius == r)) launch_front(r, true);
    else if (!fail_slot_clean) HIP_OK(hipMemsetAsync(d_scal.p + SC_FAIL, 0, sizeof(double), st));
  } else {
    HIP_OK(hipMemsetAsync(d_scal.p + SC_FAIL, 0, sizeof(double), st));
    HIP_OK(hipMemsetAsync(d_scal.p + SC_FAIL_FRONT, 0, sizeof(double), st));
    timed("entries_pose", [&] {
      launch_factor_entries_pose(st, N, Nstride, NPs, d_obs_img.p, d_obs_pt.p, d_pt_free.p, d_Jc.p, d_Jp.p, d_scale_cam.p,
                                 d_scale_pt.p, d_Gi.p, d_h.p, d_Epose.p, d_pt_start.p, d_Cu.p, d_gu.p, r, dmin, dmax,
                                 d_scal.p + SC_FAIL);
    });
    timed("entries_intr", [&] {
      launch_entries_intr(st, Q, NI, NPs, d_q_pt.p, d_q_cam.p, d_Wk.p, d_scale_cam.p, d_scale_pt.p, d_Gi.p, d_h.p,
                          d_Eintr.p);
    });
  }
  if (!M_is_clean) {
    timed("memset_S", [&] {
      HIP_OK(hipMemsetAsync(d_M.p, 0, chol_struct.store_doubles() * sizeof(double), st));
      launch_fix_diag(st, n_mat, chol_struct.d_tile_slot, rank == 0, d_col_var.p, d_scale_cam.p, d_M.p);
    });
    M_is_clean = true;
  }
  if (!(front_ok && fused_now())) timed("schur_clusters", [&] {
    launch_schur_clusters(st, num_clusters, d_clusters.p, d_cl_tab.p, d_pt_start.p, d_q_start.p, d_obs_meta.p,
                          d_q_meta.p, d_pt_clustered.p, d_Epose.p, d_Eintr.p, d_h.p, NPs, d_part[0].p, d_part[1].p,
                          d_part[2].p);
  });
  if (num_chunks[0] > 0) timed("schur_chunks_pp", [&] { launch_schur_chunks(st, BLK_PP, num_chunks[0], d_chunks[0].p, d_terms[0].p, d_Epose.p, d_Eintr.p, d_part[0].p); });
  if (num_chunks[1] > 0) timed("schur_chunks_ip", [&] { launch_schur_chunks(st, BLK_IP, num_chunks[1], d_chunks[1].p, d_terms[1].p, d_Epose.p, d_Eintr.p, d_part[1].p); });
  if (num_chunks[2] > 0) timed("schur_chunks_ii", [&] { launch_schur_chunks(st, BLK_II, num_chunks[2], d_chunks[2].p, d_terms[2].p, d_Epose.p, d_Eintr.p, d_part[2].p); });
  const int nbt = n_mat / 64;
  timed("schur_finalize", [&] {
    if (!(prereduced && front_valid && front_radius == r)) launch_partial_reduce(st, num_reduce_tasks, d_reduce_tasks.p, d_part[0].p, d_part[1].p, d_part[2].p);
    launch_schur_finalize(st, num_blocks, d_blocks.p, d_part[0].p, d_part[1].p, d_part[2].p, NI, NC, chol_struct.d_tile_slot, nbt, rank == 0,
                          r, dmin, dmax, d_img_cam.p, d_img_rec, d_cam_rec, d_scale_cam.p, d_off.p, d_off.p + NI, d_M.p);
  });
  if (sharded()) {
    launch_tiles_copy(st, num_ar_tiles, d_ar_tiles.p, chol_struct.d_tile_slot, nbt, d_M.p, d_ar_buf.p, true);
    allreduce(d_ar_buf.p, (long long)num_ar_tiles * 4096 + n_mat, 0);
    launch_tiles_copy(st, num_ar_tiles, d_ar_tiles.p, chol_struct.d_tile_slot, nbt, d_M.p, d_ar_buf.p, false);
  }
  assembled = true;
}

void mavba_session::decide_persistent() {
  if (persist_decided) return;
  if (chol_struct.persist_ok && !sharded()) allow_persistent = persistent_allowed_now();
  persist_decided = true;
}

void mavba_session::solve_linear(double r) {
  decide_persistent();
  assemble(r);
  const CamUpdateArgs u = cam_update_args(r);
  const bool with_update = merge_small();
  timed_split("chol_factor", "chol_backsolve", [&](hipEvent_t mid) {
    cameras_updated = dense_spd_solve_device(st, d_M.p, n_mat, d_ymat.p, d_scal.p + SC_FAIL, d_diag_ws.p, d_L.p, chol_struct, d_col_var.p, d_y.p,
                                             allow_persistent, mid, with_update ? &u : nullptr);
    cameras_updated_r = r;
  });
  assembled = false;
  fail_slot_clean = false;
  if (!(allow_persistent && chol_struct.persist_ok) || sharded()) M_is_clean = false;
}

void mavba_session::read_backsub_switch() {
  const char* e = std::getenv("MAVBA_BACKSUB_BLOCKS");
  backsub_blocks = e ? (std::atoi(e) != 0 ? 1 : 0) : -1;
}

void mavba_session::linear_step(double r, double* h) {
  read_backsub_switch();
  solve_linear(r);
  candidate(r, h);
  if (h[SC_FAIL] >= 1e29 && allow_persistent) {
    std::fprintf(stderr, "mavba: persistent factorisation timed out, falling back to the launch-per-panel schedule\n");
    allow_persistent = false;
    persistent_timed_out();
    solve_linear(r);
    candidate(r, h);
  }
}

void mavba_session::candidate(double r, double* h) {
  candidate_enqueue(r);
  read_scalars(h);
}
void mavba_session::candidate_enqueue(double r, ReduceTasks* tail, int* tail_count) {
  const double dmin = opt.min_lm_diagonal, dmax = opt.max_lm_diagonal;
  const bool tiles = backsub_on_tiles();
  const int rows = backsub_rows(), ugroups = update_cameras_groups(NI);
  if (!(cameras_updated && cameras_updated_r == r))
    timed("update_cameras", [&] { launch_update_cameras(st, cam_update_args(r), d_y.p); });
  cameras_updated = false;
  static const long long fuse_env = [] { const char* e = std::getenv("MAVBA_COST_FUSE_MAX_OBS"); return e ? std::atoll(e) : -1ll; }();
  const long long fuse_max_obs = fuse_env >= 0 ? fuse_env : 500000ll;
  const bool cost_separate = tiles && fuse_env < 0 ? false : (long long)N > fuse_max_obs;
  double* cost_rows = cost_separate ? nullptr : d_sweep_partial.p;
  timed("backsub_points", [&] {
    if (tiles)
      launch_backsub_points_tiles(st, num_bs_tiles, d_bs_tiles.p, NPs, NI, r, dmin, dmax, sweep_args(d_camrec.p, d_intr.p, d_points.p),
                                  d_pt_start.p, d_delta_cam.p, d_pt_free.p, d_Gi.p, d_h.p, d_Cu.p, d_gu.p, d_scale_pt.p, d_cpoints.p,
                                  d_delta_pts.p, d_step_partial.p, d_ccamrec.p, d_cintr.p, cost_rows);
    else
      launch_backsub_points_jvp(st, NP, NPs, NI, r, dmin, dmax, sweep_args(d_camrec.p, d_intr.p, d_points.p), d_pt_start.p,
                                d_delta_cam.p, d_pt_free.p, d_Gi.p, d_h.p, d_Cu.p, d_gu.p, d_scale_pt.p, d_cpoints.p,
                                d_delta_pts.p, d_step_partial.p, d_ccamrec.p, d_cintr.p, cost_rows);
  });
  SweepArgs a = sweep_args(d_ccamrec.p, d_cintr.p, d_cpoints.p);
  if (cost_separate) timed("cost_only", [&] { launch_cost_only(st, a); });
  if (num_priors > 0)
    timed("rot_prior", [&] {
      launch_rot_prior(st, num_priors, d_prior_img.p, d_prior_R0.p, prior_weight, d_cposes.p, d_prior_res.p,
                       d_prior_jac.p, d_prior_cost.p);
    });
  {
    const int nsweep = N > 0 ? (cost_separate ? jacobian_sweep_grid(N) : rows) : 0;
    ReduceTasks T;
    T.t[0] = ReduceTask{d_step_partial.p, rows + ugroups, 3, 0, nullptr, 0, d_scal.p + SC_STEP_NORM2};
    T.t[1] = ReduceTask{d_step_partial.p + 1, rows + ugroups, 3, 0, nullptr, 0, d_scal.p + SC_MODEL_CHANGE};
    T.t[2] = ReduceTask{d_step_partial.p + 2, rows + ugroups, 3, 0, nullptr, 0, d_scal.p + SC_CAND_XNORM2};
    T.t[3] = ReduceTask{d_sweep_partial.p, nsweep, 1, 0, d_prior_cost.p, num_priors, d_scal.p + SC_NEW_COST};
    if (tail) { *tail = T; *tail_count = 4; }
    else timed("reduce", [&] { launch_reduce_tasks(st, T, 4); });
  }
  if (sharded()) allreduce(d_scal.p + SC_CAND_BEGIN, SC_CAND_COUNT, 0);
}

bool mavba_session::small_window() const {
  return !sharded() && NI <= 64 && NC <= 8 && NP <= 8192 && dense_spd_solve_is_small(n_mat, chol_struct);
}
bool mavba_session::merge_small() const { return merge_on && small_window(); }

void mavba_session::start() {
  { const char* e = std::getenv("MAVBA_MERGE"); merge_on = !e || std::atoi(e) != 0; }
  { const char* e = std::getenv("MAVBA_SPECULATE"); speculate_on = !e || std::atoi(e) != 0; }
  read_backsub_switch();
  { const char* e = std::getenv("MAVBA_SWEEP_RIDE_MAX_OBS"); sweep_ride_max_obs = e ? std::max(0ll, std::atoll(e)) : -1; }
  decide_persistent();
  evaluate();
  initial_cost = cost + fixed_cost;
  const double g0 = std::max(grad_max, std::numeric_limits<double>::epsilon());
  abs_gtol = opt.gradient_tolerance * g0;
  started = true;
  if (num_residuals_reduced == 0 || num_parameters_reduced == 0) { termination = MAVBA_TERM_FUNCTION_TOLERANCE; return; }
  if (grad_max <= abs_gtol) { termination = MAVBA_TERM_GRADIENT_TOLERANCE; return; }
  if (opt.print_progress) {
    std::printf("%4s %14s %12s %10s %10s %10s %10s\n", "iter", "cost", "cost_change", "|gradient|", "|step|", "tr_ratio", "tr_radius");
    std::printf("%4d %14.6e %12.2e %10.2e %10.2e %10.2e %10.2e\n", 0, cost + fixed_cost, 0.0, grad_max, 0.0, 0.0, radius);
  }
}

bool mavba_session::wait_publication(double* h) {
  volatile double* pub = lm_pub;
  const double t_end = now_s() + 2.0;
  for (long long spin = 0;; ++spin) {
    if (pub[SC_COUNT + 7] == lm_seq) break;
    MAVBA_CPU_RELAX();
    if ((spin & 0xFFFF) == 0xFFFF && now_s() > t_end) return false;
  }
  std::atomic_thread_fence(std::memory_order_acquire);
  for (int i = 0; i < SC_COUNT; ++i) h[i] = pub[i];
  return true;
}

int mavba_session::iterate(int max_iters, int* done) {
  const double t0 = now_s();
  int n = 0;
  if (!started) start();
  const bool defer = (!sharded() || rccl_comm || std::getenv("MAVBA_DEFER_WITH_HOOK") != nullptr) && !opt.print_progress;
  const bool speculate = speculate_on && defer && !sharded() && front_ok && fused_now() && rows_ok && scales_ready;
  if (speculate && !lm_pub) { lm_pub = lm_pub_alloc(); if (lm_pub) lm_pub[SC_COUNT + 7] = -1.0; }
  if (speculate && lm_pub && !d_lm_dec.p) d_lm_dec.alloc(2);
  const bool merge_tail = merge_on;
  bool pending_eval = false;
  while (termination == MAVBA_TERM_RUNNING && n < max_iters) {
    if (iteration >= opt.max_num_iterations) { termination = MAVBA_TERM_NO_CONVERGENCE; break; }
    ++iteration; ++n;
    double h[SC_COUNT];
    const LmSpec sp = lm_spec(pending_eval);
    bool speculated = false;
    struct Books { bool evaluated, assembled, front_valid, fail_slot_clean; double front_radius; int eval_rows; bool prereduced; } books{};
    if (speculate && lm_pub) {
      solve_linear(radius);
      lm_seq += 1.0;
      if (merge_tail) {
        ReduceTasks T; int nt = 0;
        candidate_enqueue(radius, &T, &nt);
        timed("lm_tail", [&] { launch_lm_tail(st, T, nt, sp, d_lm_dec.p, lm_pub, lm_seq, d_scal.p + SC_FAIL); });
      } else {
        candidate_enqueue(radius);
        timed("lm_snapshot", [&] { launch_lm_snapshot(st, sp, d_lm_dec.p, lm_pub, lm_seq, d_scal.p + SC_FAIL); });
      }
      books = Books{evaluated, assembled, front_valid, fail_slot_clean, front_radius, eval_rows, prereduced};
      std::swap(d_poses.p, d_cposes.p); std::swap(d_intr.p, d_cintr.p); std::swap(d_points.p, d_cpoints.p);
      std::swap(d_camrec.p, d_ccamrec.p);
      LmSpec ks = sp;
      ks.dec = d_lm_dec.p;
      evaluate_enqueue(1.0 , ks);
      speculated = true;
      const double tw = now_s();
      const bool published = wait_publication(h);
      pub_wait_seconds += now_s() - tw;
      if (!published) {
        sync();
        for (int i = 0; i < SC_COUNT; ++i) h[i] = lm_pub[i];
      }
      if (opt.profile_kernels) sync();
      if (h[SC_FAIL] >= 1e29 && allow_persistent) {
        std::swap(d_poses.p, d_cposes.p); std::swap(d_intr.p, d_cintr.p); std::swap(d_points.p, d_cpoints.p);
        std::swap(d_camrec.p, d_ccamrec.p);
        evaluated = books.evaluated; assembled = books.assembled;
        front_valid = false;
        fail_slot_clean = false; front_radius = books.front_radius; eval_rows = books.eval_rows; prereduced = false;
        speculated = false;
        std::fprintf(stderr, "mavba: persistent factorisation timed out, falling back to the launch-per-panel schedule\n");
        allow_persistent = false;
        persistent_timed_out();
        solve_linear(radius);
        candidate(radius, h);
      }
    } else {
      linear_step(radius, h);
    }
    if (pending_eval) take_evaluation(h);
    const LmDecision dec = lm_decide(h, sp);
    auto forget_speculation = [&] {
      if (!speculated) return;
      std::swap(d_poses.p, d_cposes.p); std::swap(d_intr.p, d_cintr.p); std::swap(d_points.p, d_cpoints.p);
      std::swap(d_camrec.p, d_ccamrec.p);
      evaluated = books.evaluated; assembled = books.assembled; front_valid = books.front_valid;
      fail_slot_clean = false;
      front_radius = books.front_radius; eval_rows = books.eval_rows; prereduced = books.prereduced;
      speculated = false;
    };
    if (dec.code == LM_TERM_GTOL) {
      forget_speculation();
      pending_eval = false;
      termination = MAVBA_TERM_GRADIENT_TOLERANCE;
      --iteration; --n;
      break;
    }
    pending_eval = false;
    if (dec.code == LM_INVALID) {
      forget_speculation();
      if (++invalid_steps >= opt.max_num_consecutive_invalid_steps) { termination = MAVBA_TERM_NUMERICAL_FAILURE; break; }
    } else {
      invalid_steps = 0;
      if (dec.code == LM_TERM_PTOL) { forget_speculation(); termination = MAVBA_TERM_PARAMETER_TOLERANCE; break; }
      if (dec.code == LM_TERM_FTOL) { forget_speculation(); termination = MAVBA_TERM_FUNCTION_TOLERANCE; break; }
    }
    const bool successful = dec.code == LM_ACCEPTED;
    radius = dec.radius;
    decrease_factor = dec.decrease_factor;
    if (successful) {
      ++n_success;
      if (speculated) {
        front_radius = radius;
        pending_eval = true;
      } else {
        std::swap(d_poses.p, d_cposes.p); std::swap(d_intr.p, d_cintr.p); std::swap(d_points.p, d_cpoints.p);
        std::swap(d_camrec.p, d_ccamrec.p);
        if (defer) {
          evaluate_enqueue(radius);
          pending_eval = true;
        } else {
          evaluate(radius);
          if (grad_max <= abs_gtol) termination = MAVBA_TERM_GRADIENT_TOLERANCE;
        }
      }
    } else {
      forget_speculation();
      ++n_fail;
    }
    if (opt.print_progress)
      std::printf("%4d %14.6e %12.2e %10.2e %10.2e %10.2e %10.2e\n", iteration, cost + fixed_cost, successful ? dec.cost_change : 0.0,
                  grad_max, dec.step_norm, dec.rel, radius);
    if (termination == MAVBA_TERM_RUNNING && radius < opt.min_trust_region_radius) termination = MAVBA_TERM_PARAMETER_TOLERANCE;
  }
  if (pending_eval) {
    double h[SC_COUNT];
    read_scalars(h);
    take_evaluation(h);
    if (grad_max <= abs_gtol) termination = MAVBA_TERM_GRADIENT_TOLERANCE;
  }
  if (termination == MAVBA_TERM_RUNNING && iteration >= opt.max_num_iterations) termination = MAVBA_TERM_NO_CONVERGENCE;
  if (done) *done = n;
  solve_seconds += now_s() - t0;
  return MAVBA_OK;
}

void mavba_session::point_errors(double* out) {
  launch_cam_prepare(st, NI, d_poses.p, d_camrec.p);
  SweepArgs a = sweep_args(d_camrec.p, d_intr.p, d_points.p);
  launch_raw_residual_norm(st, a, d_rnorm.p);
  launch_point_errors(st, NP, d_pt_start.p, d_rnorm.p, d_pt_count.p, d_perr.p);
  std::vector<double> h(NP);
  if (NP) download(h.data(), d_perr.p, (size_t)NP * 8);
  sync();
  evaluated = false;
  for (int p = 0; p < NP; ++p)
    if (h_pt_count_all[p] > 0 && (h_pt_removed.empty() || !h_pt_removed[p])) {
      const int po = h_pt_orig[p];
      out[po] = h_dropped_rnorm.empty() ? h[p] : h[p] + h_dropped_rnorm[po] / (double)h_pt_count_all[p];
    }
}

void mavba_session::restart() {
  evaluated = scales_ready = started = assembled = false;
  front_valid = false;
  cameras_updated = false;
  M_is_clean = false;
  radius = opt.initial_trust_region_radius; decrease_factor = 2.0;
  cost = x_norm = grad_max = abs_gtol = initial_cost = 0.0;
  iteration = invalid_steps = n_success = n_fail = 0;
  termination = MAVBA_TERM_RUNNING;
  solve_seconds = 0.0;
}

long long mavba_session::filter_points(double max_error, const unsigned char* keep, unsigned char* removed_out,
                                       double* errors_out) {
  if (sharded()) throw Failure(MAVBA_ERR_INVALID_ARGUMENT, "filter_points on a sharded session is not supported");
  const double t0 = now_s();
  if (termination == MAVBA_TERM_NUMERICAL_FAILURE) restore_initial_params();
  std::vector<double> err((size_t)std::max(NP, 1), 0.0);
  std::fill(err.begin(), err.end(), std::numeric_limits<double>::quiet_NaN());
  point_errors(err.data());
  if (errors_out) std::memcpy(errors_out, err.data(), (size_t)NP * 8);
  std::vector<unsigned char> removed_now(h_pt_removed);
  if (removed_now.empty()) removed_now.assign((size_t)std::max(NP, 1), 0);
  long long removed = 0;
  for (int q = 0; q < NP; ++q) {
    const int po = h_pt_orig[q];
    const bool out = !removed_now[q] && !(keep && keep[po]) && err[po] > max_error;
    if (out) { removed_now[q] = 1; ++removed; }
  }
  if (removed > 0) {
    std::vector<int> per_img((size_t)std::max(NI, 1), 0);
    for (int q = 0; q < NP; ++q)
      if (!removed_now[q])
        for (int a = h_pt_start[q]; a < h_pt_start[q + 1]; ++a) per_img[h_oimg[a]]++;
    for (int i = 0; i < NI; ++i)
      if (per_img[i] == 1 && (h_pose_const[i] != 0 || h_intr_const_in[h_img_cam[i]]))
        throw Failure(MAVBA_ERR_NEEDS_REBUILD, "filter_points: an image with constant blocks is left with one residual block "
                                               "(the reference frees it, bundle_adjustment.cc:361): build the filtered problem afresh");
  }
  if (removed_out) for (int q = 0; q < NP; ++q) removed_out[h_pt_orig[q]] = removed_now[q];
  if (removed == 0) { restart(); return 0; }
  h_pt_removed.swap(removed_now);
  apply_filter_state();
  restart();
  setup_seconds += now_s() - t0;
  return removed;
}

void mavba_session::apply_filter_state() {
  std::vector<unsigned char> active((size_t)std::max(NP, 1), 1);
  std::fill(h_img_used.begin(), h_img_used.end(), 0);
  std::fill(h_cam_used.begin(), h_cam_used.end(), 0);
  const bool any = !h_pt_removed.empty();
  long long n_all = 0, n_kept = 0;
  fixed_cost = fixed_cost_priors;
  for (int q = 0; q < NP; ++q) {
    if (any && h_pt_removed[q]) { active[q] = 0; h_pt_used[q] = 0; continue; }
    n_all += h_pt_count_all[q];
    n_kept += h_pt_start[q + 1] - h_pt_start[q];
    h_pt_used[q] = h_pt_start[q + 1] > h_pt_start[q];
    if (!h_dropped_cost.empty()) fixed_cost += h_dropped_cost[h_pt_orig[q]];
    for (int a = h_pt_start[q]; a < h_pt_start[q + 1]; ++a) { h_img_used[h_oimg[a]] = 1; h_cam_used[h_img_cam[h_oimg[a]]] = 1; }
  }
  for (int i = 0; i < NI; ++i) if (h_prior_on_img[i]) h_img_used[i] = 1;
  num_residuals = 2 * n_all + num_priors_all;
  num_residuals_reduced = 2 * n_kept + num_priors;
  derive_free_flags();
  d_pose_free.upload(h_pose_free, st); d_intr_free.upload(h_intr_free, st); d_pt_free.upload(h_pt_free, st);
  if (any) d_pt_active.upload(active, st);
  sync();
}

void mavba_session::fill_result(mavba_result* r) {
  std::memset(r, 0, sizeof(*r));
  r->initial_cost = initial_cost;
  r->final_cost = cost + fixed_cost;
  r->fixed_cost = fixed_cost;
  r->num_residuals = num_residuals;
  r->num_residuals_reduced = num_residuals_reduced;
  r->num_parameters_reduced = num_parameters_reduced;
  r->num_successful_steps = n_success;
  r->num_unsuccessful_steps = n_fail;
  r->termination = termination;
  r->final_gradient_max_norm = grad_max;
  r->final_trust_region_radius = radius;
  r->setup_seconds = setup_seconds;
  r->solve_seconds = solve_seconds;
}
```

Measured before the change: 1340 iter/s.

## Defer state-norm and reduction kernels onto later kernels as extra blocks

In the speculative evaluation path, the point part of the state-norms computation now rides as extra blocks in the camera-reduce launch. The camera part is deferred into the Schur finalize launch, and the scalar reduction tasks are deferred into the update-cameras launch. This removes separate small kernel launches and their serialization from each LM iteration. It adds bookkeeping flags (owe_cam_norms/owe_reductions) that must be saved, restored and flushed correctly across speculation rollbacks and termination, which risks ordering or correctness bugs.

```diff
diff --git a/mavmap_amd/csrc/internal.h b/mavmap_amd/csrc/internal.h
--- a/mavmap_amd/csrc/internal.h
+++ b/mavmap_amd/csrc/internal.h
@@ -175,6 +175,13 @@
                    const double* Cu, double* scale_cam, double* scale_pt);
 
 constexpr int kStateNormsCamBlocks = 64;
+struct NormsRide {
+  int n = 0;
+  int NI, NC, NP, NPs, gp, gc, cam_part;
+  const unsigned char* pose_free; const unsigned char* intr_free; const unsigned char* pt_free;
+  const double* poses; const double* intr; const double* points; const double* img_rec; const double* cam_rec; const double* gu;
+  double* norm_partial;
+};
 
 void launch_factor_entries_pose(hipStream_t st, int N, int Nstride, int NPs, const int* obs_img, const int* obs_pt,
                                 const unsigned char* pt_free, const double* Jc, const double* Jp, const double* scale_cam,
@@ -207,7 +214,7 @@
                            int NI, int NC, const int* slot, int nb, bool add_base, double radius, double dmin,
                            double dmax, const int* img_cam, const double* img_rec,
                            const double* cam_rec, const double* scale_cam, const int* off_img, const int* off_cam,
-                           double* S);
+                           double* S, const NormsRide* cam_norms = nullptr );
 void launch_tiles_copy(hipStream_t st, int num_tiles, const int* tiles, const int* slot, int nb, double* M, double* buf, bool to_buf);
 void launch_fix_diag(hipStream_t st, int n_mat, const int* slot, bool add_one, const int* col_var,
                      const double* scale_cam, double* S);
@@ -235,7 +242,8 @@
   double* cand_poses; double* cand_intr; double* delta_cam; double* partial3 ; double* cand_camrec;
 };
 int update_cameras_groups(int NI);
-void launch_update_cameras(hipStream_t st, const CamUpdateArgs& u, const double* y);
+struct ReduceTasks;
+void launch_update_cameras(hipStream_t st, const CamUpdateArgs& u, const double* y, const ReduceTasks* ride = nullptr, int num_ride = 0);
 
 struct ReduceTask { const double* src; int rows, stride, is_max; const double* src2; int rows2; double* out; };
 struct ReduceTasks { ReduceTask t[6]; };
@@ -255,8 +263,9 @@
   ReduceTasks T; LmSpec spec;
   PartialRide ride;
 };
-void launch_camera_reduce(hipStream_t st, const EvalTailArgs& a);
-void launch_state_norms(hipStream_t st, const EvalTailArgs& a);
+NormsRide norms_ride_of(const EvalTailArgs& a);
+void launch_camera_reduce(hipStream_t st, const EvalTailArgs& a, bool point_norms = false);
+void launch_state_norms(hipStream_t st, const EvalTailArgs& a, bool cams_only = false);
 void launch_eval_small(hipStream_t st, const EvalTailArgs& a);
 void launch_eval_head_tail(hipStream_t st, const EvalTailArgs& a);
 
diff --git a/mavmap_amd/csrc/kernels.hip b/mavmap_amd/csrc/kernels.hip
--- a/mavmap_amd/csrc/kernels.hip
+++ b/mavmap_amd/csrc/kernels.hip
@@ -696,9 +696,18 @@
 }
 __global__ void __launch_bounds__(1024) k_camera_reduce_cam(
     const int* __restrict__ cam_img_start, const int* __restrict__ cam_imgs,
-    const double* __restrict__ img_intr_tmp, double* __restrict__ cam_rec, LmSpec spec) {
+    const double* __restrict__ img_intr_tmp, double* __restrict__ cam_rec, LmSpec spec, int ncam, NormsRide nr) {
   __shared__ double s_part[16][64];
   if (!lm_spec_go(spec, nullptr)) return;
+  if ((int)blockIdx.x >= ncam) {
+    __shared__ double s_w[4][2][4];
+    const int tid = threadIdx.x, g = tid >> 8;
+    const int vb0 = 4 * ((int)blockIdx.x - ncam);
+    if (vb0 + g < nr.gp) state_norms_waves(nr, vb0 + g, s_w[g]);
+    __syncthreads();
+    if (tid < 4 && vb0 + tid < nr.gp) state_norms_store(nr, vb0 + tid, s_w[tid]);
+    return;
+  }
   const int c = blockIdx.x;
   const int e = threadIdx.x & 63, part = threadIdx.x >> 6;
   double s = 0.0;
@@ -723,12 +732,23 @@
     cam_rec[(size_t)c * kCamRec + e] = tot;
   }
 }
-void launch_camera_reduce(hipStream_t st, const EvalTailArgs& a) {
+NormsRide norms_ride_of(const EvalTailArgs& a) {
+  NormsRide r;
+  r.NI = a.NI; r.NC = a.NC; r.NP = a.NP; r.NPs = a.NPs; r.gp = a.gp; r.gc = a.gc; r.cam_part = a.cam_part;
+  r.pose_free = a.pose_free; r.intr_free = a.intr_free; r.pt_free = a.pt_free; r.poses = a.poses; r.intr = a.intr; r.points = a.points;
+  r.img_rec = a.img_rec; r.cam_rec = a.cam_rec; r.gu = a.gu; r.norm_partial = a.norm_partial;
+  return r;
+}
+void launch_camera_reduce(hipStream_t st, const EvalTailArgs& a, bool point_norms) {
   if (a.NI > 0 || a.ride.n > 0)
     hipLaunchKernelGGL(k_camera_reduce_img, dim3(a.NI + a.ride.n), dim3(64), 0, st, a.NI, a.img_chunk_start, a.cam_partial,
                        a.prior_start, a.prior_res, a.prior_jac, a.img_rec, a.img_intr_tmp, a.spec, a.ride);
-  if (a.NC > 0 && a.with_cams)
-    hipLaunchKernelGGL(k_camera_reduce_cam, dim3(a.NC), dim3(1024), 0, st, a.cam_img_start, a.cam_imgs, a.img_intr_tmp, a.cam_rec, a.spec);
+  const int ncam = a.NC > 0 && a.with_cams ? a.NC : 0;
+  NormsRide nr = norms_ride_of(a);
+  nr.n = point_norms ? (a.gp + 3) / 4 : 0;
+  if (ncam + nr.n > 0)
+    hipLaunchKernelGGL(k_camera_reduce_cam, dim3(ncam + nr.n), dim3(1024), 0, st, a.cam_img_start, a.cam_imgs, a.img_intr_tmp, a.cam_rec, a.spec,
+                       ncam, nr);
 }
 
 __global__ void k_scales(int NI, int NC, int NP, int NPs, int jacobi,
@@ -775,19 +795,20 @@
     const unsigned char* __restrict__ intr_free, const unsigned char* __restrict__ pt_free,
     const double* __restrict__ poses, const double* __restrict__ intr, const double* __restrict__ points,
     const double* __restrict__ img_rec, const double* __restrict__ cam_rec, const double* __restrict__ gu,
-    double* __restrict__ partial, LmSpec spec) {
+    double* __restrict__ partial, LmSpec spec, int first_group) {
   __shared__ double s_red[4];
   if (!lm_spec_go(spec, nullptr)) return;
-  state_norms_body(blockIdx.x, gp, gridDim.x - gp, NI, NC, NP, NPs, cam_part, pose_free, intr_free, pt_free, poses, intr, points,
-                   img_rec, cam_rec, gu, partial, s_red);
+  state_norms_body(first_group + blockIdx.x, gp, first_group + gridDim.x - gp, NI, NC, NP, NPs, cam_part, pose_free, intr_free, pt_free, poses, intr,
+                   points, img_rec, cam_rec, gu, partial, s_red);
 }
 void state_norms_grid(int NI, int NC, int NP, int* gp, int* gc) {
   *gp = std::min(512, (NP + 255) / 256);
   *gc = std::max(1, std::min(kStateNormsCamBlocks, (6 * NI + 9 * NC + 255) / 256));
 }
-void launch_state_norms(hipStream_t st, const EvalTailArgs& a) {
-  hipLaunchKernelGGL(k_state_norms, dim3(a.gp + a.gc), dim3(256), 0, st, a.NI, a.NC, a.NP, a.NPs, a.gp, a.cam_part, a.pose_free,
-                     a.intr_free, a.pt_free, a.poses, a.intr, a.points, a.img_rec, a.cam_rec, a.gu, a.norm_partial, a.spec);
+void launch_state_norms(hipStream_t st, const EvalTailArgs& a, bool cams_only) {
+  const int first = cams_only ? a.gp : 0;
+  hipLaunchKernelGGL(k_state_norms, dim3(a.gp + a.gc - first), dim3(256), 0, st, a.NI, a.NC, a.NP, a.NPs, a.gp, a.cam_part, a.pose_free,
+                     a.intr_free, a.pt_free, a.poses, a.intr, a.points, a.img_rec, a.cam_rec, a.gu, a.norm_partial, a.spec, first);
 }
 
 
@@ -1296,7 +1317,13 @@
     int add_base, double radius, double dmin, double dmax, const int* __restrict__ img_cam,
     const double* __restrict__ img_rec, const double* __restrict__ cam_rec,
     const double* __restrict__ scale_cam, const int* __restrict__ off_img, const int* __restrict__ off_cam,
-    double* __restrict__ S) {
+    double* __restrict__ S, int block_groups, NormsRide nr) {
+  if ((int)blockIdx.x >= block_groups) {
+    __shared__ double s_red[4];
+    state_norms_body(nr.gp + (int)blockIdx.x - block_groups, nr.gp, nr.gc, nr.NI, nr.NC, nr.NP, nr.NPs, nr.cam_part, nr.pose_free, nr.intr_free,
+                     nr.pt_free, nr.poses, nr.intr, nr.points, nr.img_rec, nr.cam_rec, nr.gu, nr.norm_partial, s_red);
+    return;
+  }
   const int wv = threadIdx.x >> 6, lane = threadIdx.x & 63;
   const int bid = blockIdx.x * 4 + wv;
   if (bid >= num_blocks) return;
@@ -1357,11 +1384,14 @@
                            int NI, int NC, const int* slot, int nb, bool add_base, double radius, double dmin,
                            double dmax, const int* img_cam, const double* img_rec,
                            const double* cam_rec, const double* scale_cam, const int* off_img, const int* off_cam,
-                           double* S) {
-  if (num_blocks <= 0) return;
-  hipLaunchKernelGGL(k_schur_finalize, dim3((num_blocks + 3) / 4), dim3(256), 0, st, num_blocks, blocks, part_pp,
+                           double* S, const NormsRide* cam_norms) {
+  NormsRide nr{};
+  if (cam_norms) { nr = *cam_norms; nr.n = nr.gc; }
+  const int block_groups = num_blocks > 0 ? (num_blocks + 3) / 4 : 0;
+  if (block_groups + nr.n <= 0) return;
+  hipLaunchKernelGGL(k_schur_finalize, dim3(block_groups + nr.n), dim3(256), 0, st, num_blocks, blocks, part_pp,
                      part_ip, part_ii, NI, NC, slot, nb, add_base ? 1 : 0, radius, dmin, dmax, img_cam, img_rec, cam_rec,
-                     scale_cam, off_img, off_cam, S);
+                     scale_cam, off_img, off_cam, S, block_groups, nr);
 }
 __global__ void __launch_bounds__(256) k_tiles_copy(int num_tiles, const int* __restrict__ tiles, const int* __restrict__ slot, int nb,
                                                     double* __restrict__ M, double* __restrict__ buf, int to_buf) {
@@ -1793,15 +1823,19 @@
     const double* __restrict__ scale_cam, const double* __restrict__ img_rec, const double* __restrict__ cam_rec,
     const double* __restrict__ poses, const double* __restrict__ intr, double* cand_poses,
     double* __restrict__ cand_intr, double* __restrict__ delta_cam, double* __restrict__ partial3,
-    double* __restrict__ cand_camrec) {
+    double* __restrict__ cand_camrec, int ugroups, ReduceTasks ride) {
   __shared__ double s_red[4];
+  if ((int)blockIdx.x >= ugroups) { reduce_task_body(ride.t[blockIdx.x - ugroups], s_red); return; }
   update_cameras_body(blockIdx.x, NI, NC, cam_part, radius, dmin, dmax, y, scale_cam, img_rec, cam_rec, poses, intr, cand_poses, cand_intr,
                       delta_cam, partial3, cand_camrec, s_red);
 }
-void launch_update_cameras(hipStream_t st, const CamUpdateArgs& u, const double* y) {
-  hipLaunchKernelGGL(k_update_cameras, dim3(update_cameras_groups(u.NI)), dim3(256), 0, st, u.NI, u.NC, u.cam_part, u.radius, u.dmin,
+void launch_update_cameras(hipStream_t st, const CamUpdateArgs& u, const double* y, const ReduceTasks* ride, int num_ride) {
+  const int ugroups = update_cameras_groups(u.NI);
+  ReduceTasks T{};
+  if (ride && num_ride > 0) T = *ride; else num_ride = 0;
+  hipLaunchKernelGGL(k_update_cameras, dim3(ugroups + num_ride), dim3(256), 0, st, u.NI, u.NC, u.cam_part, u.radius, u.dmin,
                      u.dmax, y, u.scale_cam, u.img_rec, u.cam_rec, u.poses, u.intr, u.cand_poses, u.cand_intr, u.delta_cam, u.partial3,
-                     u.cand_camrec);
+                     u.cand_camrec, ugroups, T);
 }
 
 __global__ void __launch_bounds__(256) k_reduce_tasks(ReduceTasks T, LmSpec spec) {
diff --git a/mavmap_amd/csrc/lm_bodies.h b/mavmap_amd/csrc/lm_bodies.h
--- a/mavmap_amd/csrc/lm_bodies.h
+++ b/mavmap_amd/csrc/lm_bodies.h
@@ -98,6 +98,21 @@
 __device__ __forceinline__ double group4_sum(const double* w) { return (w[0] + w[1]) + (w[2] + w[3]); }
 __device__ __forceinline__ double group4_max(const double* w) { return fmax(fmax(w[0], w[1]), fmax(w[2], w[3])); }
 
+template <class ARGS>
+__device__ __forceinline__ void state_norms_waves(const ARGS& a, int vb, double (*w)[4]) {
+  const int tid = threadIdx.x, lt = tid & 255, wv = (tid >> 6) & 3, lane = tid & 63;
+  double gmax, x2;
+  state_norms_local(vb, lt, a.gp, a.gc, a.NI, a.NC, a.NP, a.NPs, a.cam_part, a.pose_free, a.intr_free, a.pt_free, a.poses, a.intr, a.points,
+                    a.img_rec, a.cam_rec, a.gu, gmax, x2);
+  const double m = wave_max(gmax), sum = wave_sum(x2);
+  if (lane == 0) { w[0][wv] = m; w[1][wv] = sum; }
+}
+template <class ARGS>
+__device__ __forceinline__ void state_norms_store(const ARGS& a, int vb, double (*w)[4]) {
+  a.norm_partial[2 * vb] = group4_max(w[0]);
+  a.norm_partial[2 * vb + 1] = group4_sum(w[1]);
+}
+
 __device__ __forceinline__ void reduce_task_body(const ReduceTask& t, double* s_red) {
   double v = 0.0;
   for (int r = threadIdx.x; r < t.rows; r += 256) {
@@ -144,7 +159,7 @@
   __shared__ double s_part[16][64];
   __shared__ double s_w[kStateNormsCamBlocks][2][4];
   __shared__ double s_t[4][2][4];
-  const int tid = threadIdx.x, g = tid >> 8, lt = tid & 255, wv = (tid >> 6) & 3, lane = tid & 63;
+  const int tid = threadIdx.x, g = tid >> 8, lane = tid & 63;
   if constexpr (IMAGES) {
     for (int q = tid; q < a.NI * kSweepAcc; q += 1024)
       camera_reduce_img_elem(q / kSweepAcc, q % kSweepAcc, a.img_chunk_start, a.cam_partial, a.prior_start, a.prior_res, a.prior_jac, a.img_rec,
@@ -167,19 +182,10 @@
   const int nvb = a.gp + a.gc;
   for (int vb0 = a.first_group; vb0 < nvb; vb0 += 4) {
     const int vb = vb0 + g;
-    if (vb < nvb) {
-      double gmax, x2;
-      state_norms_local(vb, lt, a.gp, a.gc, a.NI, a.NC, a.NP, a.NPs, a.cam_part, a.pose_free, a.intr_free, a.pt_free, a.poses, a.intr, a.points,
-                        a.img_rec, a.cam_rec, a.gu, gmax, x2);
-      const double m = wave_max(gmax), sum = wave_sum(x2);
-      if (lane == 0) { s_w[vb - a.first_group][0][wv] = m; s_w[vb - a.first_group][1][wv] = sum; }
-    }
-  }
-  __syncthreads();
-  if (tid < nvb - a.first_group) {
-    a.norm_partial[2 * (a.first_group + tid)] = group4_max(s_w[tid][0]);
-    a.norm_partial[2 * (a.first_group + tid) + 1] = group4_sum(s_w[tid][1]);
-  }
+    if (vb < nvb) state_norms_waves(a, vb, s_w[vb - a.first_group]);
+  }
+  __syncthreads();
+  if (tid < nvb - a.first_group) state_norms_store(a, a.first_group + tid, s_w[tid]);
   __syncthreads();
   reduce_tasks_grouped(a.T, a.num_tasks, s_t);
 }
diff --git a/mavmap_amd/csrc/session.h b/mavmap_amd/csrc/session.h
--- a/mavmap_amd/csrc/session.h
+++ b/mavmap_amd/csrc/session.h
@@ -453,7 +453,7 @@
   void choose_elimination_order(const std::vector<SchurBlock>& blocks);
   void reset_state();
   void evaluate(double next_radius = -1.0);
-  void evaluate_enqueue(double next_radius = -1.0, const LmSpec& spec = lm_spec_off());
+  void evaluate_enqueue(double next_radius = -1.0, const LmSpec& spec = lm_spec_off(), bool may_hand_over = false);
   EvalTailArgs eval_tail_args(const LmSpec& spec);
   CamUpdateArgs cam_update_args(double r);
   void launch_front(double r, bool entries, const LmSpec& spec = lm_spec_off(), const CamSweepArgs* with_sweep = nullptr);
@@ -484,6 +484,10 @@
   bool small_window() const;
   bool merge_on = true;
   long long sweep_ride_max_obs = -1;
+  int eval_chain = 6;
+  void read_chain_switch();
+  bool owe_cam_norms = false, owe_reductions = false;
+  void flush_owed(bool reductions = true);
   double pub_wait_seconds = 0.0;
   bool cameras_updated = false;
   double cameras_updated_r = 0.0;
diff --git a/mavmap_amd/csrc/session_build.hip b/mavmap_amd/csrc/session_build.hip
--- a/mavmap_amd/csrc/session_build.hip
+++ b/mavmap_amd/csrc/session_build.hip
@@ -1404,6 +1404,7 @@
   HIP_OK(hipMemcpyAsync(d_points.p, d_points0.p, (size_t)NP * 3 * 8, hipMemcpyDeviceToDevice, st));
   evaluated = scales_ready = started = assembled = false;
   camrec_current = false;
+  owe_cam_norms = owe_reductions = false;
   radius = opt.initial_trust_region_radius; decrease_factor = 2.0;
   cost = x_norm = grad_max = abs_gtol = initial_cost = 0.0;
   iteration = invalid_steps = n_success = n_fail = 0;
diff --git a/mavmap_amd/csrc/session_lm.hip b/mavmap_amd/csrc/session_lm.hip
--- a/mavmap_amd/csrc/session_lm.hip
+++ b/mavmap_amd/csrc/session_lm.hip
@@ -86,7 +86,7 @@
   return u;
 }
 
-void mavba_session::evaluate_enqueue(double next_radius, const LmSpec& spec) {
+void mavba_session::evaluate_enqueue(double next_radius, const LmSpec& spec, bool may_hand_over) {
   if (!camrec_current) timed("cam_prepare", [&] { launch_cam_prepare(st, NI, d_poses.p, d_camrec.p); });
   camrec_current = true;
   SweepArgs a = sweep_args(d_camrec.p, d_intr.p, d_points.p);
@@ -115,8 +115,9 @@
   if (!sweep_rode_along) timed("camera_sweep", [&] { launch_camera_sweep(st, c, KMAX, any_intr_free); });
   PartialRide pride;
   static const bool pride_on = [] { const char* e = std::getenv("MAVBA_PARTIAL_RIDE"); return !e || std::atoi(e) != 0; }();
-  if (pride_on && merge_on && front_ok && front_valid && fused_now() && num_reduce_tasks > 0 && num_chunks[0] + num_chunks[1] + num_chunks[2] == 0 &&
-      num_tail_tiles == 0 && !sharded() && !opt.profile_kernels) {
+  const bool ride_ok = merge_on && front_ok && front_valid && fused_now() && num_chunks[0] + num_chunks[1] + num_chunks[2] == 0 &&
+                       num_tail_tiles == 0 && !sharded() && !opt.profile_kernels;
+  if (pride_on && ride_ok && num_reduce_tasks > 0) {
     pride.n = num_reduce_tasks; pride.tasks = d_reduce_tasks.p; pride.pp = d_part[0].p; pride.ip = d_part[1].p; pride.ii = d_part[2].p;
   }
   if (num_priors > 0)
@@ -137,7 +138,9 @@
     evaluated = true; assembled = false;
     return;
   }
-  timed("camera_reduce", [&] { launch_camera_reduce(st, e); });
+  const bool chain = may_hand_over && spec.dec && scales_ready && ride_ok;
+  const bool norms_ride = chain && (eval_chain & 2), reductions_ride = chain && (eval_chain & 4);
+  timed("camera_reduce", [&] { launch_camera_reduce(st, e, norms_ride); });
   allreduce(d_camsum.p, (long long)NI * kImgRec + (long long)NC * kCamRec, 0);
   if (!scales_ready) {
     timed("scales", [&] {
@@ -146,10 +149,19 @@
     });
     scales_ready = true;
   }
-  timed("state_norms", [&] { launch_state_norms(st, e); });
-  timed("reduce", [&] { launch_reduce_tasks(st, e.T, e.num_tasks, spec); });
+  if (norms_ride) owe_cam_norms = true;
+  else timed("state_norms", [&] { launch_state_norms(st, e); });
+  if (norms_ride || reductions_ride) owe_reductions = true;
+  else timed("reduce", [&] { launch_reduce_tasks(st, e.T, e.num_tasks, spec); });
   if (sharded()) allreduce(d_scal.p + SC_COST, SC_EVAL_COUNT, 2);
   evaluated = true; assembled = false;
+}
+void mavba_session::flush_owed(bool reductions) {
+  if (!owe_cam_norms && !(reductions && owe_reductions)) return;
+  const EvalTailArgs e = eval_tail_args(lm_spec_off());
+  if (owe_cam_norms) launch_state_norms(st, e, true);
+  owe_cam_norms = false;
+  if (reductions && owe_reductions) { launch_reduce_tasks(st, e.T, e.num_tasks); owe_reductions = false; }
 }
 void mavba_session::evaluate(double next_radius) {
   evaluate_enqueue(next_radius);
@@ -194,8 +206,11 @@
   const int nbt = n_mat / 64;
   timed("schur_finalize", [&] {
     if (!(prereduced && front_valid && front_radius == r)) launch_partial_reduce(st, num_reduce_tasks, d_reduce_tasks.p, d_part[0].p, d_part[1].p, d_part[2].p);
+    NormsRide nr;
+    if (owe_cam_norms) nr = norms_ride_of(eval_tail_args(lm_spec_off()));
     launch_schur_finalize(st, num_blocks, d_blocks.p, d_part[0].p, d_part[1].p, d_part[2].p, NI, NC, chol_struct.d_tile_slot, nbt, rank == 0,
-                          r, dmin, dmax, d_img_cam.p, d_img_rec, d_cam_rec, d_scale_cam.p, d_off.p, d_off.p + NI, d_M.p);
+                          r, dmin, dmax, d_img_cam.p, d_img_rec, d_cam_rec, d_scale_cam.p, d_off.p, d_off.p + NI, d_M.p, owe_cam_norms ? &nr : nullptr);
+    owe_cam_norms = false;
   });
   if (sharded()) {
     launch_tiles_copy(st, num_ar_tiles, d_ar_tiles.p, chol_struct.d_tile_slot, nbt, d_M.p, d_ar_buf.p, true);
@@ -226,6 +241,10 @@
   if (!(allow_persistent && chol_struct.persist_ok) || sharded()) M_is_clean = false;
 }
 
+void mavba_session::read_chain_switch() {
+  const char* e = std::getenv("MAVBA_EVAL_CHAIN");
+  eval_chain = e ? std::atoi(e) & 6 : 6;
+}
 void mavba_session::read_backsub_switch() {
   const char* e = std::getenv("MAVBA_BACKSUB_BLOCKS");
   backsub_blocks = e ? (std::atoi(e) != 0 ? 1 : 0) : -1;
@@ -252,8 +271,14 @@
   const double dmin = opt.min_lm_diagonal, dmax = opt.max_lm_diagonal;
   const bool tiles = backsub_on_tiles();
   const int rows = backsub_rows(), ugroups = update_cameras_groups(NI);
-  if (!(cameras_updated && cameras_updated_r == r))
-    timed("update_cameras", [&] { launch_update_cameras(st, cam_update_args(r), d_y.p); });
+  flush_owed(false);
+  const bool update_here = !(cameras_updated && cameras_updated_r == r);
+  if (owe_reductions && !(update_here && (eval_chain & 4))) flush_owed();
+  if (update_here) {
+    ReduceTasks owed; int num_owed = 0;
+    if (owe_reductions) { const EvalTailArgs e = eval_tail_args(lm_spec_off()); owed = e.T; num_owed = e.num_tasks; owe_reductions = false; }
+    timed("update_cameras", [&] { launch_update_cameras(st, cam_update_args(r), d_y.p, num_owed ? &owed : nullptr, num_owed); });
+  }
   cameras_updated = false;
   static const long long fuse_env = [] { const char* e = std::getenv("MAVBA_COST_FUSE_MAX_OBS"); return e ? std::atoll(e) : -1ll; }();
   const long long fuse_max_obs = fuse_env >= 0 ? fuse_env : 500000ll;
@@ -297,6 +322,7 @@
 void mavba_session::start() {
   { const char* e = std::getenv("MAVBA_MERGE"); merge_on = !e || std::atoi(e) != 0; }
   { const char* e = std::getenv("MAVBA_SPECULATE"); speculate_on = !e || std::atoi(e) != 0; }
+  read_chain_switch();
   read_backsub_switch();
   { const char* e = std::getenv("MAVBA_SWEEP_RIDE_MAX_OBS"); sweep_ride_max_obs = e ? std::max(0ll, std::atoll(e)) : -1; }
   decide_persistent();
@@ -342,7 +368,7 @@
     double h[SC_COUNT];
     const LmSpec sp = lm_spec(pending_eval);
     bool speculated = false;
-    struct Books { bool evaluated, assembled, front_valid, fail_slot_clean; double front_radius; int eval_rows; bool prereduced; } books{};
+    struct Books { bool evaluated, assembled, front_valid, fail_slot_clean; double front_radius; int eval_rows; bool prereduced, owe_cam_norms, owe_reductions; } books{};
     if (speculate && lm_pub) {
       solve_linear(radius);
       lm_seq += 1.0;
@@ -354,12 +380,12 @@
         candidate_enqueue(radius);
         timed("lm_snapshot", [&] { launch_lm_snapshot(st, sp, d_lm_dec.p, lm_pub, lm_seq, d_scal.p + SC_FAIL); });
       }
-      books = Books{evaluated, assembled, front_valid, fail_slot_clean, front_radius, eval_rows, prereduced};
+      books = Books{evaluated, assembled, front_valid, fail_slot_clean, front_radius, eval_rows, prereduced, owe_cam_norms, owe_reductions};
       std::swap(d_poses.p, d_cposes.p); std::swap(d_intr.p, d_cintr.p); std::swap(d_points.p, d_cpoints.p);
       std::swap(d_camrec.p, d_ccamrec.p);
       LmSpec ks = sp;
       ks.dec = d_lm_dec.p;
-      evaluate_enqueue(1.0 , ks);
+      evaluate_enqueue(1.0 , ks, merge_tail);
       speculated = true;
       const double tw = now_s();
       const bool published = wait_publication(h);
@@ -375,6 +401,7 @@
         evaluated = books.evaluated; assembled = books.assembled;
         front_valid = false;
         fail_slot_clean = false; front_radius = books.front_radius; eval_rows = books.eval_rows; prereduced = false;
+        owe_cam_norms = books.owe_cam_norms; owe_reductions = books.owe_reductions;
         speculated = false;
         std::fprintf(stderr, "mavba: persistent factorisation timed out, falling back to the launch-per-panel schedule\n");
         allow_persistent = false;
@@ -394,6 +421,7 @@
       evaluated = books.evaluated; assembled = books.assembled; front_valid = books.front_valid;
       fail_slot_clean = false;
       front_radius = books.front_radius; eval_rows = books.eval_rows; prereduced = books.prereduced;
+      owe_cam_norms = books.owe_cam_norms; owe_reductions = books.owe_reductions;
       speculated = false;
     };
     if (dec.code == LM_TERM_GTOL) {
@@ -442,6 +470,7 @@
   }
   if (pending_eval) {
     double h[SC_COUNT];
+    flush_owed();
     read_scalars(h);
     take_evaluation(h);
     if (grad_max <= abs_gtol) termination = MAVBA_TERM_GRADIENT_TOLERANCE;
@@ -469,6 +498,7 @@
 }
 
 void mavba_session::restart() {
+  owe_cam_norms = owe_reductions = false;
   evaluated = scales_ready = started = assembled = false;
   front_valid = false;
   cameras_updated = false;
```

Measured after the change: 1351 iter/s (median of 6 runs). About the same (+0.9%).
